# xdspacelab/openvslam

Hardware: NVIDIA H100
Metric: frames/sec extract+match+local-BA @1920x960 4000kp (higher is better)
Workload: dtype u8 (extract, Hamming) + f64 (pose optimiser, local BA)

## Files before the change

openvslam_b200/csrc/ba_math.cuh:

```cuda
#pragma once
#include <math.h>
#include <stdint.h>

#if defined(__CUDACC__)
#define OVS_BA_HD __host__ __device__ __forceinline__
#else
#define OVS_BA_HD static inline
#endif

namespace ovs {

constexpr int kCamPerspective = 0;
constexpr int kCamEquirectangular = 1;
constexpr double kPi = 3.14159265358979323846;

struct CameraD {
    int model;
    double fx, fy, cx, cy, fb, cols, rows;
};

OVS_BA_HD void mat3_vec(const double* R, const double* v, double* o) {
    o[0] = R[0] * v[0] + R[1] * v[1] + R[2] * v[2];
    o[1] = R[3] * v[0] + R[4] * v[1] + R[5] * v[2];
    o[2] = R[6] * v[0] + R[7] * v[1] + R[8] * v[2];
}
OVS_BA_HD void mat3_mat3(const double* A, const double* B, double* C) {
    for (int i = 0; i < 3; ++i)
        for (int j = 0; j < 3; ++j) C[3 * i + j] = A[3 * i] * B[j] + A[3 * i + 1] * B[3 + j] + A[3 * i + 2] * B[6 + j];
}

OVS_BA_HD void pose_oplus(const double* pose, const double* u, double* out) {
    const double wx = u[0], wy = u[1], wz = u[2];
    const double theta = sqrt(wx * wx + wy * wy + wz * wz);
    const double O[9] = {0, -wz, wy, wz, 0, -wx, -wy, wx, 0};
    double O2[9];
    mat3_mat3(O, O, O2);
    double a, b, c;
    if (theta < 0.00001) { a = 1.0; b = 0.5; c = 1.0 / 6.0; }
    else {
        a = sin(theta) / theta;
        b = (1 - cos(theta)) / (theta * theta);
        c = (theta - sin(theta)) / (theta * theta * theta);
    }
    double Rd[9], V[9];
    for (int i = 0; i < 9; ++i) {
        const double I = (i == 0 || i == 4 || i == 8) ? 1.0 : 0.0;
        Rd[i] = I + a * O[i] + b * O2[i];
        V[i] = I + b * O[i] + c * O2[i];
    }
    double td[3], tn[3];
    mat3_vec(V, u + 3, td);
    mat3_mat3(Rd, pose, out);
    mat3_vec(Rd, pose + 9, tn);
    out[9] = tn[0] + td[0]; out[10] = tn[1] + td[1]; out[11] = tn[2] + td[2];
}

OVS_BA_HD int edge_eval(const CameraD& cam, const double* pose, const double* pw, const double* obs, bool stereo,
                        double* e, double* Jp, double* Jl) {
    double pc[3];
    mat3_vec(pose, pw, pc);
    pc[0] += pose[9]; pc[1] += pose[10]; pc[2] += pose[11];
    const double x = pc[0], y = pc[1], z = pc[2];
    const double* R = pose;
    if (cam.model == kCamEquirectangular) {
        const double L = sqrt(x * x + y * y + z * z);
        const double theta = atan2(x, z);
        const double phi = -asin(y / L);
        e[0] = obs[0] - cam.cols * (0.5 + theta / (2 * kPi));
        e[1] = obs[1] - cam.rows * (0.5 - phi / kPi);
        if (Jp || Jl) {
            const double dpc[3][9] = {
                {0, z, -y, 1, 0, 0, R[0], R[1], R[2]},
                {-z, 0, x, 0, 1, 0, R[3], R[4], R[5]},
                {y, -x, 0, 0, 0, 1, R[6], R[7], R[8]}};
            const double xz2 = x * x + z * z;
            const double c0 = -(cam.cols / (2 * kPi)) * (1.0 / xz2);
            const double c1 = -(cam.rows / kPi) * (1.0 / (L * sqrt(xz2)));
            for (int k = 0; k < 9; ++k) {
                const double dL = (1.0 / L) * (x * dpc[0][k] + y * dpc[1][k] + z * dpc[2][k]);
                const double j0 = c0 * (z * dpc[0][k] - x * dpc[2][k]);
                const double j1 = c1 * (L * dpc[1][k] - y * dL);
                if (k < 6) { if (Jp) { Jp[k] = j0; Jp[6 + k] = j1; } }
                else if (Jl) { Jl[k - 6] = j0; Jl[3 + k - 6] = j1; }
            }
        }
        return 2;
    }
    const double fx = cam.fx, fy = cam.fy, fb = cam.fb;
    const double z_sq = z * z;
    const double reproj_x = fx * x / z + cam.cx;
    e[0] = obs[0] - reproj_x;
    e[1] = obs[1] - (fy * y / z + cam.cy);
    if (stereo) e[2] = obs[2] - (reproj_x - fb / z);
    if (Jl) {
        for (int k = 0; k < 3; ++k) {
            Jl[k] = -fx * R[k] / z + fx * x * R[6 + k] / z_sq;
            Jl[3 + k] = -fy * R[3 + k] / z + fy * y * R[6 + k] / z_sq;
            if (stereo) Jl[6 + k] = Jl[k] - fb * R[6 + k] / z_sq;
        }
    }
    if (Jp) {
        Jp[0] = x * y / z_sq * fx; Jp[1] = -(1.0 + (x * x / z_sq)) * fx; Jp[2] = y / z * fx;
        Jp[3] = -1.0 / z * fx; Jp[4] = 0.0; Jp[5] = x / z_sq * fx;
        Jp[6] = (1.0 + y * y / z_sq) * fy; Jp[7] = -x * y / z_sq * fy; Jp[8] = -x / z * fy;
        Jp[9] = 0.0; Jp[10] = -1.0 / z * fy; Jp[11] = y / z_sq * fy;
        if (stereo) {
            Jp[12] = Jp[0] - fb * y / z_sq; Jp[13] = Jp[1] + fb * x / z_sq; Jp[14] = Jp[2];
            Jp[15] = Jp[3]; Jp[16] = 0.0; Jp[17] = Jp[5] - fb / z_sq;
        }
    }
    return stereo ? 3 : 2;
}

OVS_BA_HD void huber(double e2, double delta, double* rho0, double* rho1) {
    const double dsqr = delta * delta;
    if (e2 <= dsqr) { *rho0 = e2; *rho1 = 1.0; }
    else {
        const double sqrte = sqrt(e2);
        *rho0 = 2 * sqrte * delta - dsqr;
        *rho1 = delta / sqrte;
    }
}

OVS_BA_HD bool inv3_sym(const double* D, double* Di) {
    const double a = D[0], b = D[1], c = D[2], d = D[3], e = D[4], f = D[5];
    const double c00 = d * f - e * e, c01 = c * e - b * f, c02 = b * e - c * d;
    const double det = a * c00 + b * c01 + c * c02;
    if (det == 0.0 || !isfinite(det)) return false;
    const double id = 1.0 / det;
    Di[0] = c00 * id; Di[1] = c01 * id; Di[2] = c02 * id;
    Di[3] = (a * f - c * c) * id; Di[4] = (b * c - a * e) * id; Di[5] = (a * d - b * b) * id;
    return true;
}

OVS_BA_HD int sym3(int i, int j) { return i <= j ? (i * 3 - i * (i - 1) / 2 + (j - i)) : (j * 3 - j * (j - 1) / 2 + (i - j)); }
OVS_BA_HD int sym6(int i, int j) { return i <= j ? (i * 6 - i * (i - 1) / 2 + (j - i)) : (j * 6 - j * (j - 1) / 2 + (i - j)); }

}
```

openvslam_b200/csrc/optimize.cu:

```cuda
#include <algorithm>
#include <cfloat>
#include <cmath>
#include <cstdio>
#include <cstdlib>
#include <cstring>
#include <functional>
#include <new>
#include <sched.h>
#include <time.h>
#include <vector>


#include "ba_math.cuh"
#include "block_sum.cuh"
#include "ovs_common.h"
#include "pnp_math.cuh"
#include "sim3_math.cuh"

namespace {

using ovs::CameraD;

constexpr int kMaxReducedDimBig = 6000;
constexpr int kCholMaxDynSmem = 226 * 1024;
constexpr int kNB = 32;
constexpr int kCholThreads = 512;
constexpr int kCholCluster = 8;
constexpr int kPoseThreads = 256;
constexpr int kPoseCluster = 8;

__device__ __forceinline__ double warp_sum(double v) {
#pragma unroll
    for (int o = 16; o > 0; o >>= 1) v += __shfl_xor_sync(0xffffffffu, v, o);
    return v;
}

__device__ double block_sum(double v, double* smem ) {
    const int lane = threadIdx.x & 31, wid = threadIdx.x >> 5, nw = blockDim.x >> 5;
    v = warp_sum(v);
    __syncthreads();
    if (lane == 0) smem[wid] = v;
    __syncthreads();
    double t = 0;
    for (int k = 0; k < nw; ++k) t += smem[k];
    return t;
}

__device__ __forceinline__ void atomic_max_pos(double* addr, double v) {
    atomicMax(reinterpret_cast<unsigned long long*>(addr), (unsigned long long)__double_as_longlong(v));
}

__device__ __forceinline__ void cluster_sync_all() {
    asm volatile("barrier.cluster.arrive.release.aligned;\n" ::);
    asm volatile("barrier.cluster.wait.acquire.aligned;\n" ::);
}
__device__ __forceinline__ unsigned cluster_size() { unsigned r; asm volatile("mov.u32 %0, %%cluster_nctarank;\n" : "=r"(r)); return r; }
__device__ __forceinline__ unsigned cluster_rank() { unsigned r; asm volatile("mov.u32 %0, %%cluster_ctarank;\n" : "=r"(r)); return r; }
__device__ __forceinline__ double ld_dsmem(const double* local_ptr, unsigned rank) {
    const unsigned addr = (unsigned)__cvta_generic_to_shared(local_ptr);
    unsigned remote;
    asm volatile("mapa.shared::cluster.u32 %0, %1, %2;\n" : "=r"(remote) : "r"(addr), "r"(rank));
    double v;
    asm volatile("ld.shared::cluster.f64 %0, [%1];\n" : "=d"(v) : "r"(remote));
    return v;
}
__device__ __forceinline__ void st_dsmem(double* local_ptr, unsigned rank, double v) {
    const unsigned addr = (unsigned)__cvta_generic_to_shared(local_ptr);
    unsigned remote;
    asm volatile("mapa.shared::cluster.u32 %0, %1, %2;\n" : "=r"(remote) : "r"(addr), "r"(rank));
    asm volatile("st.shared::cluster.f64 [%0], %1;\n" :: "r"(remote), "d"(v) : "memory");
}
__device__ __forceinline__ void cluster_sync_mem() {
    asm volatile("barrier.cluster.arrive.release.aligned;\n" ::: "memory");
    asm volatile("barrier.cluster.wait.acquire.aligned;\n" ::: "memory");
}

constexpr int kSpec = 4;
constexpr int kMaxTrials = 10;
struct LmCtl {
    double lambda, ni, currentChi, rho;
    double lam[kSpec], ni_after[kSpec];
    int buf[kSpec];
    int nbatch;
    int cur;
    int err_slot;
    int it;
    int qmax;
    int active;
    int iterations;
    int use_huber;
    int stopped;
    int spec_width;
    int round_live;
    int need_more;
    int pending_nbatch;
    int num_rounds, num_iterations, num_trials, batches, solver_trials;
    int round_iterations[8];
    double lambda_init[8];
    double last_chi2, last_lambda;
};

struct BaDev {
    CameraD cam;
    int K, L, M, nfree, n;
    const double* poses; const double* points;
    const double* poses_ring; const double* points_ring;
    const int* obs_kf; const int* obs_lm; const float2* obs_xy; const float* obs_xr; const float* inv_sigma_sq;
    const unsigned char* level;
    const int* free_idx;
    const int* lm_first;
    int use_huber; double delta;
};

__global__ void __launch_bounds__(128) k_ba_linearize(BaDev P, const LmCtl* __restrict__ ctl, double* __restrict__ Hpl, double* __restrict__ Cpp,
                                                       double* __restrict__ bpo, double* __restrict__ All, double* __restrict__ blo) {
    if (!ctl->active) return;
    __shared__ __align__(16) double sm[128 * 30];
    P.poses = P.poses_ring + (size_t)ctl->cur * 12 * P.K; P.points = P.points_ring + (size_t)ctl->cur * 3 * P.L;
    P.use_huber = ctl->use_huber;
    const int base = blockIdx.x * 128, t = threadIdx.x;
    const int i = base + t;
    const int nedge = min(128, P.M - base);
    const bool live = i < P.M && !P.level[i];
    int dim = 0, fi = -1;
    double e[3] = {0, 0, 0}, Jp[18], Jl[9], ww = 0;
#pragma unroll
    for (int k = 0; k < 18; ++k) Jp[k] = 0;
#pragma unroll
    for (int k = 0; k < 9; ++k) Jl[k] = 0;
    if (live) {
        const int kf = P.obs_kf[i], lm = P.obs_lm[i];
        fi = P.free_idx[kf];
        const float xr = P.obs_xr ? P.obs_xr[i] : -1.0f;
        const bool stereo = xr >= 0.0f;
        const float2 xy = P.obs_xy[i];
        const double obs[3] = {(double)xy.x, (double)xy.y, (double)xr};
        double pose[12], pw[3];
#pragma unroll
        for (int k = 0; k < 12; ++k) pose[k] = P.poses[12 * (size_t)kf + k];
#pragma unroll
        for (int k = 0; k < 3; ++k) pw[k] = P.points[3 * (size_t)lm + k];
        dim = ovs::edge_eval(P.cam, pose, pw, obs, stereo, e, Jp, Jl);
        const double w = (double)P.inv_sigma_sq[i];
        double chi = 0;
        for (int d = 0; d < dim; ++d) chi += w * e[d] * e[d];
        double rho0 = chi, rho1 = 1.0;
        if (P.use_huber) ovs::huber(chi, P.delta, &rho0, &rho1);
        ww = rho1 * w;
    }
    double* sW = sm; double* sbp = sm + 128 * 18; double* sA = sbp + 128 * 6;
    {
        double* A = sA + 6 * t;
        for (int a = 0; a < 3; ++a)
            for (int b = a; b < 3; ++b) {
                double h = 0;
                for (int d = 0; d < dim; ++d) h += Jl[3 * d + a] * ww * Jl[3 * d + b];
                A[ovs::sym3(a, b)] = h;
            }
        double* W = sW + 18 * t; double* bp = sbp + 6 * t;
        const bool fr = fi >= 0;
        for (int a = 0; a < 6; ++a) {
            double g = 0;
            for (int d = 0; d < dim; ++d) g -= Jp[6 * d + a] * ww * e[d];
            bp[a] = fr ? g : 0.0;
            for (int b = 0; b < 3; ++b) {
                double h = 0;
                for (int d = 0; d < dim; ++d) h += Jp[6 * d + a] * ww * Jl[3 * d + b];
                W[3 * a + b] = fr ? h : 0.0;
            }
        }
    }
    __syncthreads();
    {
        const double2* s2 = reinterpret_cast<const double2*>(sW); double2* g2 = reinterpret_cast<double2*>(Hpl + 18 * (size_t)base);
        for (int q = t; q < 9 * nedge; q += 128) g2[q] = s2[q];
        s2 = reinterpret_cast<const double2*>(sbp); g2 = reinterpret_cast<double2*>(bpo + 6 * (size_t)base);
        for (int q = t; q < 3 * nedge; q += 128) g2[q] = s2[q];
        s2 = reinterpret_cast<const double2*>(sA); g2 = reinterpret_cast<double2*>(All + 6 * (size_t)base);
        for (int q = t; q < 3 * nedge; q += 128) g2[q] = s2[q];
    }
    __syncthreads();
    double* sC = sm; double* sbl = sm + 128 * 21;
    {
        double* C = sC + 21 * t; double* bl = sbl + 3 * t;
        const bool fr = fi >= 0;
        for (int a = 0; a < 6; ++a)
            for (int b = a; b < 6; ++b) {
                double h = 0;
                for (int d = 0; d < dim; ++d) h += Jp[6 * d + a] * ww * Jp[6 * d + b];
                C[ovs::sym6(a, b)] = fr ? h : 0.0;
            }
        for (int a = 0; a < 3; ++a) {
            double g = 0;
            for (int d = 0; d < dim; ++d) g -= Jl[3 * d + a] * ww * e[d];
            bl[a] = g;
        }
    }
    __syncthreads();
    {
        const double2* s2 = reinterpret_cast<const double2*>(sC); double2* g2 = reinterpret_cast<double2*>(Cpp + 21 * (size_t)base);
        const int nd = 21 * nedge;
        for (int q = t; q < nd / 2; q += 128) g2[q] = s2[q];
        if ((nd & 1) && t == 0) Cpp[21 * (size_t)base + nd - 1] = sC[nd - 1];
        const int nb = 3 * nedge;
        for (int q = t; q < nb; q += 128) blo[3 * (size_t)base + q] = sbl[q];
    }
}

__global__ void __launch_bounds__(128) k_ba_landmark_accum(BaDev P, const LmCtl* __restrict__ ctl, const double* __restrict__ All, const double* __restrict__ blo,
                                                            double* __restrict__ Hll, double* __restrict__ bl, double* __restrict__ maxdiag) {
    if (!ctl->active) return;
    const int l = blockIdx.x * 128 + threadIdx.x;
    double md = 0;
    if (l < P.L) {
        double H[6] = {0, 0, 0, 0, 0, 0}, b[3] = {0, 0, 0};
        for (int p = P.lm_first[l]; p < P.lm_first[l + 1]; ++p) {
            if (P.level[p]) continue;
#pragma unroll
            for (int k = 0; k < 6; ++k) H[k] += All[6 * (size_t)p + k];
#pragma unroll
            for (int k = 0; k < 3; ++k) b[k] += blo[3 * (size_t)p + k];
        }
#pragma unroll
        for (int k = 0; k < 6; ++k) Hll[6 * (size_t)l + k] = H[k];
#pragma unroll
        for (int k = 0; k < 3; ++k) bl[3 * (size_t)l + k] = b[k];
        md = fmax(fabs(H[0]), fmax(fabs(H[3]), fabs(H[5])));
    }
#pragma unroll
    for (int o = 16; o > 0; o >>= 1) md = fmax(md, __shfl_xor_sync(0xffffffffu, md, o));
    if ((threadIdx.x & 31) == 0 && md > 0) atomic_max_pos(maxdiag, md);
}

__global__ void __launch_bounds__(128) k_ba_pose_accum_chunk(BaDev P, const LmCtl* __restrict__ ctl, const int* __restrict__ nchunks,
                                                              const int4* __restrict__ pair_rec, const int4* __restrict__ chunks,
                                                              const double* __restrict__ Cpp, const double* __restrict__ bpo,
                                                              double* __restrict__ ppart) {
    __shared__ double red[27][4];
    if (!ctl->active || (int)blockIdx.x >= *nchunks) return;
    const int4 ch = chunks[blockIdx.x];
    const int e = ch.y + threadIdx.x;
    double acc[27];
#pragma unroll
    for (int k = 0; k < 27; ++k) acc[k] = 0;
    if (e < ch.z) {
        const int4 rec = pair_rec[e];
        const int o = rec.x;
        if (!rec.w) {
#pragma unroll
            for (int k = 0; k < 21; ++k) acc[k] = Cpp[21 * (size_t)o + k];
#pragma unroll
            for (int k = 0; k < 6; ++k) acc[21 + k] = bpo[6 * (size_t)o + k];
        }
    }
    const int lane = threadIdx.x & 31, wid = threadIdx.x >> 5;
#pragma unroll
    for (int k = 0; k < 27; ++k) {
        const double v = warp_sum(acc[k]);
        if (lane == 0) red[k][wid] = v;
    }
    __syncthreads();
    if (threadIdx.x < 27)
        ppart[27 * (size_t)blockIdx.x + threadIdx.x] = red[threadIdx.x][0] + red[threadIdx.x][1] + red[threadIdx.x][2] + red[threadIdx.x][3];
}

__global__ void k_ba_pose_final_plan(LmCtl* ctl, int nfree, const int* __restrict__ kf_chunk_begin, const double* __restrict__ ppart,
                                     double* __restrict__ Hpp, double* __restrict__ bp, double* maxdiag, int* fail,
                                     const volatile int* stop_word, volatile int* mirror);

__device__ __forceinline__ void dmma_m8n8k4(double& d0, double& d1, double a, double b) {
    asm volatile("mma.sync.aligned.m8n8k4.row.col.f64.f64.f64.f64 {%0, %1}, {%2}, {%3}, {%0, %1};\n" : "+d"(d0), "+d"(d1) : "d"(a), "d"(b));
}

constexpr int kSGY = 76, kSGW = 84;
__global__ void __launch_bounds__(128, 4) k_ba_schur_chunk(BaDev P, const LmCtl* __restrict__ ctl, const int* __restrict__ nchunks,
                                                         const int4* __restrict__ pair_rec, const int4* __restrict__ chunks,
                                                         const int2* __restrict__ pair_ab, const double* __restrict__ Hll,
                                                         const double* __restrict__ Hpl, const double* __restrict__ bl,
                                                         double* __restrict__ spart, size_t spart_stride) {
    __shared__ double s_y[4 * 8 * kSGY];
    __shared__ double s_w[4 * 8 * kSGW];
    double* sYw = s_y + (threadIdx.x >> 5) * 8 * kSGY;
    double* sWw = s_w + (threadIdx.x >> 5) * 8 * kSGW;
    static_assert(4 * 8 * kSGY >= kSpec * 4 * 64, "reduction buffer must fit in the Y region");
    const int nbatch = ctl->nbatch;
    if (nbatch == 0 || (int)blockIdx.x >= *nchunks) return;
    const int4 ch = chunks[blockIdx.x];
    const int2 ab = pair_ab[ch.x];
    const bool diag = ab.x == ab.y;
    const int lane = threadIdx.x & 31, wid = threadIdx.x >> 5;
    const int e = ch.y + threadIdx.x;
    double wa[18], hl[6] = {0, 0, 0, 0, 0, 0};
    int lm = -1;
    {
        double wb[18], gl[3] = {0, 0, 0};
#pragma unroll
        for (int k = 0; k < 18; ++k) { wa[k] = 0; wb[k] = 0; }
        if (e < ch.z) {
            const int4 ob = pair_rec[e];
            if (!ob.w) {
                lm = ob.z;
                const double2* pa = reinterpret_cast<const double2*>(Hpl + 18 * (size_t)ob.x);
                const double2* pb = reinterpret_cast<const double2*>(Hpl + 18 * (size_t)ob.y);
#pragma unroll
                for (int k = 0; k < 9; ++k) { const double2 v = pa[k]; wa[2 * k] = v.x; wa[2 * k + 1] = v.y; }
                if (ob.x == ob.y) {
#pragma unroll
                    for (int k = 0; k < 18; ++k) wb[k] = wa[k];
                } else {
#pragma unroll
                    for (int k = 0; k < 9; ++k) { const double2 v = pb[k]; wb[2 * k] = v.x; wb[2 * k + 1] = v.y; }
                }
                const double2* ph = reinterpret_cast<const double2*>(Hll + 6 * (size_t)lm);
#pragma unroll
                for (int k = 0; k < 3; ++k) { const double2 v = ph[k]; hl[2 * k] = v.x; hl[2 * k + 1] = v.y; }
                if (diag) { gl[0] = bl[3 * (size_t)lm]; gl[1] = bl[3 * (size_t)lm + 1]; gl[2] = bl[3 * (size_t)lm + 2]; }
            }
        }
#pragma unroll
        for (int kc = 0; kc < 3; ++kc) {
            const int kk = 3 * (lane & 3) + kc, base = (lane >> 2) * kSGW + (kk >> 2) * 28 + (kk & 3);
#pragma unroll
            for (int c = 0; c < 6; ++c) sWw[base + 4 * c] = wb[3 * c + kc];
            sWw[base + 24] = gl[kc];
        }
    }
    double lam[kSpec];
#pragma unroll
    for (int bt = 0; bt < kSpec; ++bt) lam[bt] = ctl->lam[bt];
    auto make_dinv = [&](int bt, double (&di)[6]) {
        double D[6] = {hl[0] + lam[bt], hl[1], hl[2], hl[3] + lam[bt], hl[4], hl[5] + lam[bt]};
        if (lm < 0 || !ovs::inv3_sym(D, di)) {
#pragma unroll
            for (int q = 0; q < 6; ++q) di[q] = 0.0;
        }
    };
    const int r = lane >> 2;
    int sbase[3];
#pragma unroll
    for (int kc = 0; kc < 3; ++kc) { const int kk = 3 * (lane & 3) + kc; sbase[kc] = (lane >> 2) * kSGY + (kk >> 2) * 24 + (kk & 3); }
    const bool rowA = r < 6, colB = r < 6 || (r == 6 && diag);
    double acc[kSpec][2];
#pragma unroll
    for (int bt = 0; bt < kSpec; ++bt) { acc[bt][0] = 0; acc[bt][1] = 0; }
    const int nrec_w = min(32, max(0, ch.z - (ch.y + 32 * wid)));
    const bool second_half = nrec_w > 16;
#pragma unroll
    for (int bt = 0; bt < kSpec; ++bt) {
        if (bt < nbatch && nrec_w > 0) {
            double di[6];
            make_dinv(bt, di);
            double ya[18];
#pragma unroll
            for (int a = 0; a < 6; ++a) {
                const double w0 = wa[3 * a], w1 = wa[3 * a + 1], w2 = wa[3 * a + 2];
                ya[3 * a] = w0 * di[0] + w1 * di[1] + w2 * di[2];
                ya[3 * a + 1] = w0 * di[1] + w1 * di[3] + w2 * di[4];
                ya[3 * a + 2] = w0 * di[2] + w1 * di[4] + w2 * di[5];
            }
            __syncwarp();
#pragma unroll
            for (int a = 0; a < 6; ++a) {
                sYw[sbase[0] + 4 * a] = ya[3 * a]; sYw[sbase[1] + 4 * a] = ya[3 * a + 1]; sYw[sbase[2] + 4 * a] = ya[3 * a + 2];
            }
            __syncwarp();
            double c0[2] = {0, 0}, c1[2] = {0, 0}, c2[2] = {0, 0}, c3[2] = {0, 0};
            const double* yb = sYw + lane;
            const double* wb = sWw + lane;
#pragma unroll
            for (int half = 0; half < 2; ++half) {
                if (half == 1 && !second_half) break;
#pragma unroll
                for (int t = 0; t < 3; ++t) {
                    const int oy = (4 * half) * kSGY + t * 24, ow = (4 * half) * kSGW + t * 28;
                    const double a0 = rowA ? yb[oy] : 0.0, b0 = colB ? wb[ow] : 0.0;
                    const double a1 = rowA ? yb[oy + kSGY] : 0.0, b1 = colB ? wb[ow + kSGW] : 0.0;
                    const double a2 = rowA ? yb[oy + 2 * kSGY] : 0.0, b2 = colB ? wb[ow + 2 * kSGW] : 0.0;
                    const double a3 = rowA ? yb[oy + 3 * kSGY] : 0.0, b3 = colB ? wb[ow + 3 * kSGW] : 0.0;
                    dmma_m8n8k4(c0[0], c0[1], a0, b0);
                    dmma_m8n8k4(c1[0], c1[1], a1, b1);
                    dmma_m8n8k4(c2[0], c2[1], a2, b2);
                    dmma_m8n8k4(c3[0], c3[1], a3, b3);
                }
            }
            acc[bt][0] = (c0[0] + c1[0]) + (c2[0] + c3[0]);
            acc[bt][1] = (c0[1] + c1[1]) + (c2[1] + c3[1]);
        }
    }
    __syncthreads();
    double* red = s_y;
#pragma unroll
    for (int bt = 0; bt < kSpec; ++bt)
        if (bt < nbatch) { red[(bt * 4 + wid) * 64 + 2 * lane] = acc[bt][0]; red[(bt * 4 + wid) * 64 + 2 * lane + 1] = acc[bt][1]; }
    __syncthreads();
    for (int idx = threadIdx.x; idx < 42 * nbatch; idx += 128) {
        const int bt = idx / 42, t = idx - 42 * bt;
        const int i = t < 36 ? t / 6 : t - 36;
        const int j = t < 36 ? t % 6 : 6;
        const int src = 2 * (4 * i + (j >> 1)) + (j & 1);
        const double* rb = red + (size_t)bt * 4 * 64;
        double v = rb[src] + rb[64 + src] + rb[128 + src] + rb[192 + src];
        if (j == 6 && !diag) v = 0.0;
        spart[(size_t)bt * spart_stride + 42 * (size_t)blockIdx.x + t] = v;
    }
}

__global__ void __launch_bounds__(256) k_ba_pair_flags(const unsigned char* __restrict__ level, int4* __restrict__ rec, int n) {
    const int i = blockIdx.x * 256 + threadIdx.x;
    if (i >= n) return;
    int4 r = rec[i];
    r.w = (level[r.x] | level[r.y]) ? 1 : 0;
    rec[i] = r;
}

__global__ void __launch_bounds__(64) k_ba_schur_final(int n, const LmCtl* __restrict__ ctl, const int* __restrict__ pair_chunk_begin, const int2* __restrict__ pair_ab,
                                                        const double* __restrict__ spart, size_t spart_stride, const double* __restrict__ Hpp,
                                                        const double* __restrict__ bp, double* __restrict__ S, size_t S_stride) {
    const int pid = blockIdx.x, t = threadIdx.x;
    if ((int)blockIdx.y >= ctl->nbatch) return;
    const double lambda = ctl->lam[blockIdx.y];
    spart += (size_t)blockIdx.y * spart_stride; S += (size_t)blockIdx.y * S_stride;
    double* bS = S + (size_t)n * n;
    if (t >= 42) return;
    const int a = pair_ab[pid].x, b = pair_ab[pid].y;
    const bool diag = a == b;
    if (t >= 36 && !diag) return;
    double s = 0;
    const int c0 = pair_chunk_begin[pid], c1 = pair_chunk_begin[pid + 1];
#pragma unroll 4
    for (int c = c0; c < c1; ++c) s += spart[42 * (size_t)c + t];
    if (t < 36) {
        const int i = t / 6, j = t % 6;
        double v = -s;
        if (diag) v += Hpp[21 * (size_t)a + ovs::sym6(i, j)] + (i == j ? lambda : 0.0);
        S[(size_t)(6 * b + j) * n + 6 * a + i] = v;
    } else {
        bS[6 * a + t - 36] = bp[6 * (size_t)a + t - 36] - s;
    }
}

constexpr int kPP = 36;
__host__ __device__ __forceinline__ size_t chol_fixed_doubles(int n) { return (size_t)32 * 33 + 32 + ((n + 1 + 31) / 32) * 32 + 32 * 33 + 32 * kPP; }
__host__ __device__ __forceinline__ size_t chol_panel_doubles(int n) { return (size_t)(n + 4) * kPP; }
__host__ __device__ __forceinline__ int chol_back_pitch(int n) { return ((n + 3) / 4) * 4 + 4; }
__host__ __device__ __forceinline__ size_t chol_back_doubles(int n) { return (size_t)32 * 33 + (size_t)32 * chol_back_pitch(n); }

__global__ void __launch_bounds__(kCholThreads, 1)
k_ba_cholesky_solve(const LmCtl* __restrict__ ctl, double* __restrict__ A, size_t A_stride, int n, double* __restrict__ x, double* __restrict__ invL, size_t invL_stride,
                    int* __restrict__ fail, long long* __restrict__ dbg_clk, int dbuf) {
    {
        const int bt = blockIdx.x / (int)cluster_size();
        if (bt >= ctl->nbatch) return;
        A += (size_t)bt * A_stride; x += (size_t)bt * n; invL += (size_t)bt * invL_stride; fail += bt;
        if (bt != 0) dbg_clk = nullptr;
    }
    extern __shared__ __align__(16) double sh[];
    const int npad = ((n + 1 + 31) / 32) * 32;
    double* LdT = sh;
    double* invd = LdT + 32 * 33;
    double* vec = invd + 32;
    double* scr = vec + npad;
    double* IL = scr + 32 * 33;
    double* P = IL + 32 * kPP;
    const int tid = threadIdx.x, lane = tid & 31, wid = tid >> 5;
    const int rank = (int)cluster_rank();
    const int ncta = (int)cluster_size();
    const int g = lane >> 2, q = lane & 3;
    __shared__ int s_fail;
    if (tid == 0) s_fail = 0;
    __syncthreads();
    const int nblk = (n + kNB - 1) / kNB;
    auto stamp = [&](int slot) { if (dbg_clk && rank == 0 && tid == 0 && slot < 192) dbg_clk[slot] = clock64(); };
    auto stamp1 = [&](int slot) { if (dbg_clk && rank == 0 && tid == 64 && slot < 192) dbg_clk[slot] = clock64(); };

    auto factor_block = [&](double (&a)[kNB], double* cs) {
        bool bad = false;
        double my_inv = 1.0;
        double ajj = __shfl_sync(0xffffffffu, a[0], 0);
        double inv = rsqrt(ajj);
#pragma unroll
        for (int j = 0; j < kNB; ++j) {
            bad = bad || !(ajj > 0.0) || !isfinite(ajj);
            const double l = (lane >= j) ? a[j] * inv : 0.0;
            if (lane == j) my_inv = inv;
            double* col = cs + j * 32;
            col[lane] = l;
            if (j + 1 < kNB) {
                ajj = __shfl_sync(0xffffffffu, fma(-l, l, a[j + 1]), j + 1);
                inv = rsqrt(ajj);
            }
            __syncwarp();
#pragma unroll
            for (int c = j + 1; c < kNB; ++c) a[c] = fma(-l, col[c], a[c]);
        }
        if (bad && lane == 0) s_fail = 1;
        return my_inv;
    };

    for (int blk = -1; blk < nblk; ++blk) {
        const bool pro = blk < 0;
        const int kb = pro ? 0 : blk * kNB;
        const int nb = pro ? 0 : min(kNB, n - kb);
        const int rem = n - kb - nb;
        const int prow = rem + 1;
        const int nbn = min(kNB, rem);
        if (!pro) stamp(5 * blk);
        if (wid >= 2 && !pro) {
            for (int r = wid - 2; r < prow; r += kCholThreads / 32 - 2) {
                if (lane < nb) {
                    const unsigned dst = (unsigned)__cvta_generic_to_shared(P + r * kPP + lane);
                    const double* src = A + (size_t)(kb + nb + r) * n + kb + lane;
                    asm volatile("cp.async.ca.shared.global [%0], [%1], 8;\n" :: "r"(dst), "l"(src));
                } else {
                    P[r * kPP + lane] = 0.0;
                }
            }
            asm volatile("cp.async.commit_group;\n" ::);
            asm volatile("cp.async.wait_group 0;\n" ::);
        }
        if (!pro) {
            __syncthreads();
            stamp(5 * blk + 1);
            if (s_fail) break;
        }
        const bool worker = wid >= 2 && (wid & 3) != 0;
        const int nw = 11;
        const int wk = wid - 2 - (wid >> 2);
        if (wid == 0) {
            if (rem > 0) {
                for (int r = 0; r < nbn; ++r)
                    if (lane <= r) {
                        const unsigned dst = (unsigned)__cvta_generic_to_shared(scr + r * 33 + lane);
                        asm volatile("cp.async.ca.shared.global [%0], [%1], 8;\n" :: "r"(dst), "l"(A + (size_t)(kb + nb + r) * n + kb + nb + lane));
                    }
                asm volatile("cp.async.commit_group;\n" ::);
            }
            if (lane < prow && !pro) {
                const int r = lane;
                double xr[kNB];
                double* row = P + r * kPP;
#pragma unroll
                for (int c = 0; c < kNB; c += 2) {
                    const double2 v = *reinterpret_cast<const double2*>(row + c);
                    xr[c] = v.x; xr[c + 1] = v.y;
                }
#pragma unroll
                for (int c = 0; c < kNB; ++c) {
                    const double xc = xr[c] * invd[c];
                    xr[c] = xc;
#pragma unroll
                    for (int c2 = c + 1; c2 < kNB; ++c2) xr[c2] = fma(-xc, LdT[c * 32 + c2], xr[c2]);
                }
#pragma unroll
                for (int c = 0; c < kNB; c += 2) *reinterpret_cast<double2*>(row + c) = make_double2(xr[c], xr[c + 1]);
            }
            __syncwarp();
            if (!pro) stamp(5 * blk + 2);
            if (rem == 0) {
                if (rank == 0 && lane < nb) A[(size_t)(kb + nb) * n + kb + lane] = P[lane];
            } else {
                if (!pro) asm volatile("bar.arrive 3, 480;\n" ::: "memory");
            asm volatile("cp.async.wait_group 0;\n" ::: "memory");
            __syncwarp();
            double acc[4][4][2];
#pragma unroll
            for (int ti = 0; ti < 4; ++ti)
#pragma unroll
                for (int tj = 0; tj <= ti; ++tj)
#pragma unroll
                    for (int e = 0; e < 2; ++e) {
                        const int rr = 8 * ti + g, cc = 8 * tj + 2 * q + e;
                        acc[ti][tj][e] = (rr < nbn && cc <= rr) ? scr[rr * 33 + cc] : 0.0;
                    }
            __syncwarp();
#pragma unroll 2
            for (int k4 = pro ? kNB : 0; k4 < kNB; k4 += 4) {
                double pv[4];
#pragma unroll
                for (int ti = 0; ti < 4; ++ti) pv[ti] = P[(8 * ti + g) * kPP + k4 + q];
#pragma unroll
                for (int ti = 0; ti < 4; ++ti)
#pragma unroll
                    for (int tj = 0; tj <= ti; ++tj) dmma_m8n8k4(acc[ti][tj][0], acc[ti][tj][1], -pv[ti], pv[tj]);
            }
#pragma unroll
            for (int ti = 0; ti < 4; ++ti)
#pragma unroll
                for (int tj = 0; tj <= ti; ++tj)
#pragma unroll
                    for (int e = 0; e < 2; ++e) scr[(8 * ti + g) * 33 + 8 * tj + 2 * q + e] = acc[ti][tj][e];
            __syncwarp();
            double a[kNB];
#pragma unroll
            for (int c = 0; c < kNB; ++c) a[c] = (lane < nbn && c <= lane) ? scr[lane * 33 + c] : ((c == lane) ? 1.0 : 0.0);
            if (blk < 12 && !pro) { asm volatile("" :: "d"(a[0]), "d"(a[kNB - 1])); stamp(168 + 2 * blk); }
            __syncwarp();
            const double my_inv = factor_block(a, scr);
            if (blk < 12 && !pro) { asm volatile("" :: "d"(my_inv)); stamp(169 + 2 * blk); }
            if (!pro) asm volatile("bar.sync 2, 64;\n" ::: "memory");
#pragma unroll
            for (int c = 0; c < kNB; ++c) LdT[c * 32 + lane] = scr[c * 32 + lane];
            invd[lane] = my_inv;
            }
        } else if (pro) {
        } else if (wid == 1) {
            double r[kNB];
#pragma unroll
            for (int i = 0; i < kNB; ++i) r[i] = (i == lane) ? 1.0 : 0.0;
#pragma unroll
            for (int i = 0; i < kNB; ++i) {
                const double xi = r[i] * invd[i];
                r[i] = xi;
#pragma unroll
                for (int i2 = i + 1; i2 < kNB; ++i2) r[i2] = fma(-LdT[i * 32 + i2], xi, r[i2]);
            }
#pragma unroll
            for (int i = 0; i < kNB; ++i) IL[i * kPP + lane] = r[i];
            asm volatile("bar.arrive 4, 384;\n" ::: "memory");
            if (rank == 0) {
#pragma unroll
                for (int i = 0; i < kNB; ++i) invL[((size_t)blk * kNB + i) * kNB + lane] = r[i];
            }
            if (rem > 0) asm volatile("bar.arrive 2, 64;\n" ::: "memory");
        } else {
            if (worker) {
                asm volatile("bar.sync 4, 384;\n" ::: "memory");
                double bfr[4][8];
// ... 37 lines not shown
                    const int mj = w - base;
                    const int R0 = mi * 16, C0 = mj * 32;
                    if (w == 0) stamp1(50 + 4 * blk);
                    double acc[2][4][2];
#pragma unroll
                    for (int ti = 0; ti < 2; ++ti)
#pragma unroll
                        for (int tj = 0; tj < 4; ++tj)
#pragma unroll
                            for (int e = 0; e < 2; ++e) {
                                const int rr = R0 + 8 * ti + g, cc = C0 + 8 * tj + 2 * q + e;
                                const bool mine = rr < prow && cc < rem && cc <= rr && !(rr < nbn);
                                acc[ti][tj][e] = mine ? A[(size_t)(kb + nb + rr) * n + kb + nb + cc] : 0.0;
                            }
                    if (w == 0) { asm volatile("" :: "d"(acc[0][0][0]), "d"(acc[1][3][1]), "d"(acc[1][0][0]), "d"(acc[0][3][1])); stamp1(51 + 4 * blk); }
                    const double* pa0 = P + (size_t)min(R0 + g, prow - 1) * kPP + q;
                    const double* pa1 = P + (size_t)min(R0 + 8 + g, prow - 1) * kPP + q;
                    const double* pb[4];
#pragma unroll
                    for (int tj = 0; tj < 4; ++tj) pb[tj] = P + (size_t)min(C0 + 8 * tj + g, prow - 1) * kPP + q;
#pragma unroll 2
                    for (int k4 = 0; k4 < kNB; k4 += 4) {
                        const double af0 = -pa0[k4], af1 = -pa1[k4];
                        double bf[4];
#pragma unroll
                        for (int tj = 0; tj < 4; ++tj) bf[tj] = pb[tj][k4];
#pragma unroll
                        for (int tj = 0; tj < 4; ++tj) {
                            dmma_m8n8k4(acc[0][tj][0], acc[0][tj][1], af0, bf[tj]);
                            dmma_m8n8k4(acc[1][tj][0], acc[1][tj][1], af1, bf[tj]);
                        }
                    }
                    if (w == 0) { asm volatile("" :: "d"(acc[0][0][0]), "d"(acc[1][3][1])); stamp1(52 + 4 * blk); }
#pragma unroll
                    for (int ti = 0; ti < 2; ++ti)
#pragma unroll
                        for (int tj = 0; tj < 4; ++tj)
#pragma unroll
                            for (int e = 0; e < 2; ++e) {
                                const int rr = R0 + 8 * ti + g, cc = C0 + 8 * tj + 2 * q + e;
                                const bool mine = rr < prow && cc < rem && cc <= rr && !(rr < nbn);
                                if (mine) A[(size_t)(kb + nb + rr) * n + kb + nb + cc] = acc[ti][tj][e];
                            }
                    if (w == 0) stamp1(53 + 4 * blk);
                }
            }
        }
        if (rem == 0) break;
        if (pro) continue;
        stamp(5 * blk + 3);
        cluster_sync_all();
        stamp(5 * blk + 4);
    }
    __syncthreads();
    if (s_fail) { if (tid == 0 && rank == 0) *fail = 1; return; }
    if (rank != 0) return;

    for (int i = tid; i < n; i += kCholThreads) vec[i] = A[(size_t)n * n + i];
    const int bp = chol_back_pitch(n);
    double* const R0buf = P;
    double* const L1buf = P + 32 * (size_t)bp;
    double* const R1buf = L1buf + 32 * 33;
    double* const red = scr;
    auto stage = [&](int b, int which) {
        const int kb = b * kNB;
        const int nb = min(kNB, n - kb);
        double* Ldst = which ? L1buf : LdT;
        double* Rdst = which ? R1buf : R0buf;
        for (int i = tid; i < kNB * kNB; i += kCholThreads) {
            const unsigned dst = (unsigned)__cvta_generic_to_shared(Ldst + (i >> 5) * 33 + (i & 31));
            asm volatile("cp.async.ca.shared.global [%0], [%1], 8;\n" :: "r"(dst), "l"(invL + (size_t)b * kNB * kNB + i));
        }
        for (int j = wid; j < nb; j += kCholThreads / 32)
            for (int c = 2 * lane; c < kb; c += 64) {
                const unsigned dst = (unsigned)__cvta_generic_to_shared(Rdst + j * bp + c);
                asm volatile("cp.async.cg.shared.global [%0], [%1], 16;\n" :: "r"(dst), "l"(A + (size_t)(kb + j) * n + c));
            }
        asm volatile("cp.async.commit_group;\n" ::);
    };
    __syncthreads();
    stamp(94);
    stage(nblk - 1, 0);
    for (int blk = nblk - 1; blk >= 0; --blk) {
        const int kb = blk * kNB;
        const int nb = min(kNB, n - kb);
        const int cur = dbuf ? ((nblk - 1 - blk) & 1) : 0;
        if (dbuf && blk > 0) {
            stage(blk - 1, cur ^ 1);
            asm volatile("cp.async.wait_group 1;\n" ::);
        } else {
            asm volatile("cp.async.wait_group 0;\n" ::);
        }
        __syncthreads();
        stamp(96 + 3 * (nblk - 1 - blk));
        const double* Lc = cur ? L1buf : LdT;
        const double* rows = cur ? R1buf : R0buf;
        if (wid == 0) {
            const double t = (lane < nb) ? vec[kb + lane] : 0.0;
            double acc0 = 0, acc1 = 0;
#pragma unroll
            for (int j = 0; j < kNB; j += 2) {
                acc0 = fma(Lc[j * 33 + lane], __shfl_sync(0xffffffffu, t, j), acc0);
                acc1 = fma(Lc[(j + 1) * 33 + lane], __shfl_sync(0xffffffffu, t, j + 1), acc1);
            }
            red[lane] = acc0 + acc1;
            if (lane < nb) vec[kb + lane] = acc0 + acc1;
        }
        __syncthreads();
        stamp(97 + 3 * (nblk - 1 - blk));
        for (int i = tid; i < kb; i += kCholThreads) {
            double s0 = 0, s1 = 0;
#pragma unroll 8
            for (int j = 0; j < kNB; j += 2) {
                if (j < nb) s0 = fma(rows[j * bp + i], red[j], s0);
                if (j + 1 < nb) s1 = fma(rows[(j + 1) * bp + i], red[j + 1], s1);
            }
            vec[i] -= s0 + s1;
        }
        __syncthreads();
        stamp(98 + 3 * (nblk - 1 - blk));
        if (!dbuf && blk > 0) stage(blk - 1, 0);
    }
    for (int i = tid; i < n; i += kCholThreads) x[i] = vec[i];
    stamp(95);
}

__global__ void __launch_bounds__(64) k_chol_big_diag(const LmCtl* __restrict__ ctl, double* __restrict__ A, size_t A_stride, int n, int kb, int nb,
                                                      double* __restrict__ invL, size_t invL_stride, int* __restrict__ fail) {
    if ((int)blockIdx.y >= ctl->nbatch) return;
    A += (size_t)blockIdx.y * A_stride; invL += (size_t)blockIdx.y * invL_stride + (size_t)(kb / kNB) * kNB * kNB; fail += blockIdx.y;
    __shared__ double cs[kNB * kNB];
    __shared__ double sinv[kNB];
    const int lane = threadIdx.x & 31, wid = threadIdx.x >> 5;
    if (wid == 0) {
        double a[kNB];
#pragma unroll
        for (int c = 0; c < kNB; ++c) {
            double v = (c == lane) ? 1.0 : 0.0;
            if (lane < nb && c <= lane) v = A[(size_t)(kb + lane) * n + kb + c];
            a[c] = v;
        }
        bool bad = false;
        double my_inv = 1.0;
        double ajj = __shfl_sync(0xffffffffu, a[0], 0);
        double inv = rsqrt(ajj);
#pragma unroll
        for (int j = 0; j < kNB; ++j) {
            bad = bad || !(ajj > 0.0) || !isfinite(ajj);
            const double l = (lane >= j) ? a[j] * inv : 0.0;
            if (lane == j) my_inv = inv;
            cs[j * 32 + lane] = l;
            if (lane < nb && j <= lane && j < nb) A[(size_t)(kb + lane) * n + kb + j] = l;
            if (j + 1 < kNB) {
                ajj = __shfl_sync(0xffffffffu, fma(-l, l, a[j + 1]), j + 1);
                inv = rsqrt(ajj);
            }
            __syncwarp();
#pragma unroll
            for (int c = j + 1; c < kNB; ++c) a[c] = fma(-l, cs[j * 32 + c], a[c]);
        }
        if (bad && lane == 0) *fail = 1;
        sinv[lane] = my_inv;
    }
    __syncthreads();
    if (wid == 1) {
        double r[kNB];
#pragma unroll
        for (int i = 0; i < kNB; ++i) r[i] = (i == lane) ? 1.0 : 0.0;
#pragma unroll
        for (int i = 0; i < kNB; ++i) {
            const double xi = r[i] * sinv[i];
            r[i] = xi;
#pragma unroll
            for (int i2 = i + 1; i2 < kNB; ++i2) r[i2] = fma(-cs[i * 32 + i2], xi, r[i2]);
        }
#pragma unroll
        for (int i = 0; i < kNB; ++i) invL[i * kNB + lane] = r[i];
    }
}

__global__ void __launch_bounds__(128) k_chol_big_panel(const LmCtl* __restrict__ ctl, double* __restrict__ A, size_t A_stride, int n, int kb, int nb,
                                                        const double* __restrict__ invL, size_t invL_stride) {
    if ((int)blockIdx.y >= ctl->nbatch) return;
    A += (size_t)blockIdx.y * A_stride; invL += (size_t)blockIdx.y * invL_stride + (size_t)(kb / kNB) * kNB * kNB;
    __shared__ double IL[kNB][kNB + 1];
    for (int i = threadIdx.x; i < kNB * kNB; i += 128) IL[i >> 5][i & 31] = invL[i];
    __syncthreads();
    const int prow = n - kb - nb + 1;
    const int r = blockIdx.x * 128 + threadIdx.x;
    if (r >= prow) return;
    double* row = A + (size_t)(kb + nb + r) * n + kb;
    double xr[kNB];
#pragma unroll
    for (int c = 0; c < kNB; ++c) xr[c] = (c < nb) ? row[c] : 0.0;
#pragma unroll
    for (int j = 0; j < kNB; ++j) {
        double acc = 0.0;
#pragma unroll
        for (int k = 0; k <= j; ++k) acc = fma(xr[k], IL[j][k], acc);
        if (j < nb) row[j] = acc;
    }
}

__global__ void __launch_bounds__(128) k_chol_big_trailing(const LmCtl* __restrict__ ctl, double* __restrict__ A, size_t A_stride, int n, int kb, int nb) {
    if ((int)blockIdx.y >= ctl->nbatch) return;
    A += (size_t)blockIdx.y * A_stride;
    const int lane = threadIdx.x & 31, wid = threadIdx.x >> 5, g = lane >> 2, q = lane & 3;
    const int rem = n - kb - nb, prow = rem + 1;
    const int nmr = (prow + 15) / 16, nmc = (rem + 31) / 32;
    const int w = blockIdx.x * 4 + wid;
    int mi = 0, base = 0;
    for (;; ++mi) {
        if (mi >= nmr) return;
        const int cnt = min(nmc, (16 * mi + 15) / 32 + 1);
        if (w < base + cnt) break;
        base += cnt;
    }
    const int mj = w - base;
    const int R0 = mi * 16, C0 = mj * 32;
    const double* P = A + (size_t)(kb + nb) * n + kb;
    double* T = A + (size_t)(kb + nb) * n + kb + nb;
    double acc[2][4][2];
#pragma unroll
    for (int ti = 0; ti < 2; ++ti)
#pragma unroll
        for (int tj = 0; tj < 4; ++tj)
#pragma unroll
            for (int e = 0; e < 2; ++e) {
                const int rr = R0 + 8 * ti + g, cc = C0 + 8 * tj + 2 * q + e;
                acc[ti][tj][e] = (rr < prow && cc < rem && cc <= rr) ? T[(size_t)rr * n + cc] : 0.0;
            }
    const double* pa0 = P + (size_t)min(R0 + g, prow - 1) * n;
    const double* pa1 = P + (size_t)min(R0 + 8 + g, prow - 1) * n;
    const double* pb[4];
#pragma unroll
    for (int tj = 0; tj < 4; ++tj) pb[tj] = P + (size_t)min(C0 + 8 * tj + g, prow - 1) * n;
#pragma unroll 2
    for (int k4 = 0; k4 < kNB; k4 += 4) {
        const bool kin = k4 + q < nb;
        const double af0 = kin ? -pa0[k4 + q] : 0.0, af1 = kin ? -pa1[k4 + q] : 0.0;
        double bf[4];
#pragma unroll
        for (int tj = 0; tj < 4; ++tj) bf[tj] = kin ? pb[tj][k4 + q] : 0.0;
#pragma unroll
        for (int tj = 0; tj < 4; ++tj) {
            dmma_m8n8k4(acc[0][tj][0], acc[0][tj][1], af0, bf[tj]);
            dmma_m8n8k4(acc[1][tj][0], acc[1][tj][1], af1, bf[tj]);
        }
    }
#pragma unroll
    for (int ti = 0; ti < 2; ++ti)
#pragma unroll
        for (int tj = 0; tj < 4; ++tj)
#pragma unroll
            for (int e = 0; e < 2; ++e) {
                const int rr = R0 + 8 * ti + g, cc = C0 + 8 * tj + 2 * q + e;
                if (rr < prow && cc < rem && cc <= rr) T[(size_t)rr * n + cc] = acc[ti][tj][e];
            }
}

__global__ void __launch_bounds__(512) k_chol_big_backsolve(const LmCtl* __restrict__ ctl, const double* __restrict__ A, size_t A_stride, int n, const double* __restrict__ invL,
                                                            size_t invL_stride, double* __restrict__ x, int* __restrict__ fail) {
    if ((int)blockIdx.x >= ctl->nbatch) return;
    A += (size_t)blockIdx.x * A_stride; invL += (size_t)blockIdx.x * invL_stride; x += (size_t)blockIdx.x * n; fail += blockIdx.x;
    extern __shared__ __align__(16) double sh[];
    double* vec = sh;
    double* IL = sh + ((n + 31) / 32) * 32;
    double* red = IL + 32 * 33;
    const int tid = threadIdx.x, lane = tid & 31, wid = tid >> 5;
    for (int i = tid; i < n; i += 512) vec[i] = A[(size_t)n * n + i];
    const int nblk = (n + kNB - 1) / kNB;
    for (int blk = nblk - 1; blk >= 0; --blk) {
        const int kb = blk * kNB, nb = min(kNB, n - kb);
        __syncthreads();
        for (int i = tid; i < kNB * kNB; i += 512) IL[(i >> 5) * 33 + (i & 31)] = invL[(size_t)blk * kNB * kNB + i];
        __syncthreads();
        if (wid == 0) {
            const double t = (lane < nb) ? vec[kb + lane] : 0.0;
            double a0 = 0, a1 = 0;
#pragma unroll
            for (int j = 0; j < kNB; j += 2) {
                a0 = fma(IL[j * 33 + lane], __shfl_sync(0xffffffffu, t, j), a0);
                a1 = fma(IL[(j + 1) * 33 + lane], __shfl_sync(0xffffffffu, t, j + 1), a1);
            }
            red[lane] = a0 + a1;
            if (lane < nb) vec[kb + lane] = a0 + a1;
        }
        __syncthreads();
        for (int i = tid; i < kb; i += 512) {
            double s0 = 0, s1 = 0;
            for (int j = 0; j + 1 < nb; j += 2) {
                s0 = fma(A[(size_t)(kb + j) * n + i], red[j], s0);
                s1 = fma(A[(size_t)(kb + j + 1) * n + i], red[j + 1], s1);
            }
            if (nb & 1) s0 = fma(A[(size_t)(kb + nb - 1) * n + i], red[nb - 1], s0);
            vec[i] -= s0 + s1;
        }
    }
    __syncthreads();
    if (*fail) return;
    for (int i = tid; i < n; i += 512) x[i] = vec[i];
}

__global__ void __launch_bounds__(128) k_ba_update(BaDev P, const LmCtl* __restrict__ ctl, const double* __restrict__ Hpl, const double* __restrict__ Hll,
                                                    const double* __restrict__ bl, const double* __restrict__ bp, const double* __restrict__ x,
                                                    double* poses_ring, double* points_ring,
                                                    double* __restrict__ partial_scale, int* __restrict__ fail) {
    __shared__ double sm[36];
    const int nbatch = ctl->nbatch;
    if (nbatch == 0) return;
    double lambda[kSpec]; int buf[kSpec];
#pragma unroll
    for (int bt = 0; bt < kSpec; ++bt) { lambda[bt] = ctl->lam[bt]; buf[bt] = ctl->buf[bt]; }
    P.poses = P.poses_ring + (size_t)ctl->cur * 12 * P.K; P.points = P.points_ring + (size_t)ctl->cur * 3 * P.L;
    const int t = blockIdx.x * 128 + threadIdx.x;
    double sc[kSpec];
#pragma unroll
    for (int bt = 0; bt < kSpec; ++bt) sc[bt] = 0;
    if (t < P.L) {
        const int l = t;
        const double b0 = bl[3 * (size_t)l], b1 = bl[3 * (size_t)l + 1], b2 = bl[3 * (size_t)l + 2];
        double r[kSpec][3];
#pragma unroll
        for (int bt = 0; bt < kSpec; ++bt) { r[bt][0] = b0; r[bt][1] = b1; r[bt][2] = b2; }
        for (int p = P.lm_first[l]; p < P.lm_first[l + 1]; ++p) {
            const int fi = P.free_idx[P.obs_kf[p]];
            if (P.level[p] || fi < 0) continue;
            double W[18];
            const double2* pw = reinterpret_cast<const double2*>(Hpl + 18 * (size_t)p);
#pragma unroll
            for (int k = 0; k < 9; ++k) { const double2 v = pw[k]; W[2 * k] = v.x; W[2 * k + 1] = v.y; }
#pragma unroll
            for (int bt = 0; bt < kSpec; ++bt) {
                if (bt < nbatch) {
                    const double* xb = x + (size_t)bt * P.n + 6 * fi;
#pragma unroll
                    for (int a = 0; a < 6; ++a) {
                        const double xa = xb[a];
                        r[bt][0] -= W[3 * a] * xa; r[bt][1] -= W[3 * a + 1] * xa; r[bt][2] -= W[3 * a + 2] * xa;
                    }
                }
            }
        }
        const double p0 = P.points[3 * (size_t)l], p1 = P.points[3 * (size_t)l + 1], p2 = P.points[3 * (size_t)l + 2];
#pragma unroll
        for (int bt = 0; bt < kSpec; ++bt) {
            if (bt < nbatch) {
                const double D[6] = {Hll[6 * (size_t)l] + lambda[bt], Hll[6 * (size_t)l + 1], Hll[6 * (size_t)l + 2], Hll[6 * (size_t)l + 3] + lambda[bt],
                                     Hll[6 * (size_t)l + 4], Hll[6 * (size_t)l + 5] + lambda[bt]};
                double Di[6];
                if (!ovs::inv3_sym(D, Di)) {
                    fail[bt] = 1;
#pragma unroll
                    for (int q = 0; q < 6; ++q) Di[q] = 0.0;
                }
                const double d0 = Di[0] * r[bt][0] + Di[1] * r[bt][1] + Di[2] * r[bt][2];
                const double d1 = Di[1] * r[bt][0] + Di[3] * r[bt][1] + Di[4] * r[bt][2];
                const double d2 = Di[2] * r[bt][0] + Di[4] * r[bt][1] + Di[5] * r[bt][2];
                double* cand_points = points_ring + (size_t)buf[bt] * 3 * P.L;
                cand_points[3 * (size_t)l] = p0 + d0;
                cand_points[3 * (size_t)l + 1] = p1 + d1;
                cand_points[3 * (size_t)l + 2] = p2 + d2;
                sc[bt] = d0 * (lambda[bt] * d0 + b0) + d1 * (lambda[bt] * d1 + b1) + d2 * (lambda[bt] * d2 + b2);
            }
        }
    } else if (t < P.L + P.K) {
        const int k = t - P.L;
        const int fi = P.free_idx[k];
        double pose[12];
#pragma unroll
        for (int j = 0; j < 12; ++j) pose[j] = P.poses[12 * (size_t)k + j];
#pragma unroll
        for (int bt = 0; bt < kSpec; ++bt) {
            if (bt < nbatch) {
            double out[12];
            if (fi >= 0) {
                double u[6];
#pragma unroll
                for (int j = 0; j < 6; ++j) { u[j] = x[(size_t)bt * P.n + 6 * fi + j]; sc[bt] += u[j] * (lambda[bt] * u[j] + bp[6 * (size_t)fi + j]); }
                ovs::pose_oplus(pose, u, out);
            } else {
#pragma unroll
                for (int j = 0; j < 12; ++j) out[j] = pose[j];
            }
            double* cand_poses = poses_ring + (size_t)buf[bt] * 12 * P.K;
#pragma unroll
            for (int j = 0; j < 12; ++j) cand_poses[12 * (size_t)k + j] = out[j];
            }
        }
    }
#pragma unroll
    for (int bt = 0; bt < kSpec; ++bt) {
        if (bt < nbatch) {
            const double tot = block_sum(sc[bt], sm);
            if (threadIdx.x == 0) partial_scale[(size_t)bt * gridDim.x + blockIdx.x] = tot;
        }
    }
}

__global__ void __launch_bounds__(128) k_ba_errors(BaDev P, const LmCtl* __restrict__ ctl, int at_current,
                                                    double* __restrict__ err, double* __restrict__ partial_chi) {
    __shared__ double sm[36];
    int slot;
    if (at_current) {
        if (!ctl->active) return;
        slot = ctl->cur;
    } else {
        if ((int)blockIdx.y >= ctl->nbatch) return;
        slot = ctl->buf[blockIdx.y];
    }
    P.use_huber = ctl->use_huber;
    P.poses = P.poses_ring + (size_t)slot * 12 * P.K;
    P.points = P.points_ring + (size_t)slot * 3 * P.L;
    err += (size_t)blockIdx.y * 3 * P.M; partial_chi += (size_t)blockIdx.y * gridDim.x;
    const int i = blockIdx.x * 128 + threadIdx.x;
    double c = 0;
    if (i < P.M && !P.level[i]) {
        const int kf = P.obs_kf[i];
        const float xr = P.obs_xr ? P.obs_xr[i] : -1.0f;
        const bool stereo = xr >= 0.0f;
        const float2 xy = P.obs_xy[i];
        const double obs[3] = {(double)xy.x, (double)xy.y, (double)xr};
        double pose[12], pw[3], e[3] = {0, 0, 0};
#pragma unroll
        for (int k = 0; k < 12; ++k) pose[k] = P.poses[12 * (size_t)kf + k];
        const size_t pi = P.obs_lm ? (size_t)P.obs_lm[i] : (size_t)i;
#pragma unroll
        for (int k = 0; k < 3; ++k) pw[k] = P.points[3 * pi + k];
        ovs::edge_eval(P.cam, pose, pw, obs, stereo, e, nullptr, nullptr);
        err[3 * (size_t)i] = e[0]; err[3 * (size_t)i + 1] = e[1]; err[3 * (size_t)i + 2] = stereo ? e[2] : 0.0;
        const double w = (double)P.inv_sigma_sq[i];
        double chi = w * (e[0] * e[0] + e[1] * e[1]);
        if (stereo) chi += w * e[2] * e[2];
        c = chi;
        if (P.use_huber) { double r1; ovs::huber(chi, P.delta, &c, &r1); }
    }
    const double tot = block_sum(c, sm);
    if (threadIdx.x == 0) partial_chi[blockIdx.x] = tot;
}

__device__ __forceinline__ void mirror_state(const LmCtl& c, volatile int* mirror) {
    if (!mirror) return;
    mirror[0] = c.nbatch; mirror[1] = c.active; mirror[3] = c.need_more; mirror[4] = c.it;
}

__global__ void __launch_bounds__(kSpec * 256) k_ba_reduce(LmCtl* ctl, int mode, const double* __restrict__ partial_chi, int nchi,
                                                           const double* __restrict__ partial_scale, int nscale, int* fail,
                                                           const volatile int* stop_word, int batch_index, int* exec_log, volatile int* mirror,
                                                           int halt_if_undecided, int next_width_cap) {
    __shared__ double sm[kSpec][2][8];
    const int nb = mode == 0 ? (ctl->active ? 1 : 0) : ctl->nbatch;
    if (nb == 0) {
        if (threadIdx.x == 0 && mode == 1 && exec_log && batch_index >= 0) exec_log[batch_index] = 0;
        return;
    }
    const int t = threadIdx.x >> 8, tl = threadIdx.x & 255, lane = tl & 31, w = tl >> 5;
    double a = 0, b = 0;
    if (t < nb) {
        const double* pc = partial_chi + (size_t)t * nchi;
        for (int i = tl; i < nchi; i += 256) a += pc[i];
        if (mode == 1) {
            const double* ps = partial_scale + (size_t)t * nscale;
            for (int i = tl; i < nscale; i += 256) b += ps[i];
        }
    }
    a = warp_sum(a); b = warp_sum(b);
    if (lane == 0) { sm[t][0][w] = a; sm[t][1][w] = b; }
    __syncthreads();
    if (threadIdx.x != 0) return;
    double chi[kSpec], sc[kSpec];
    for (int k = 0; k < nb; ++k) {
        double x = 0, y = 0;
        for (int j = 0; j < 8; ++j) { x += sm[k][0][j]; y += sm[k][1][j]; }
        chi[k] = x; sc[k] = y;
    }
    if (mode == 0) { ctl->currentChi = chi[0]; ctl->err_slot = 0; return; }
    LmCtl c = *ctl;
    const bool stop = stop_word && *stop_word != 0;
    double lambda = c.lambda, ni = c.ni, currentChi = c.currentChi, rho = c.rho;
    int qmax = c.qmax, cur = c.cur, es = c.err_slot, ntr = c.num_trials;
    bool done = false;
#pragma unroll
    for (int k = 0; k < kSpec; ++k) {
        if (k < nb && !done) {
            const bool ok2 = fail[k] == 0;
            const double tempChi = ok2 ? chi[k] : DBL_MAX;
            rho = currentChi - tempChi;
            double scale = ok2 ? sc[k] : 0.0;
            scale += 1e-3;
            rho /= scale;
            es = k;
            ++qmax; ++ntr;
            if (rho > 0 && isfinite(tempChi)) {
                double alpha = 1. - pow(2 * rho - 1, 3.0);
                alpha = fmin(alpha, 2. / 3.);
                lambda = c.lam[k] * fmax(1. / 3., alpha);
                ni = 2;
                currentChi = tempChi;
                cur = c.buf[k];
                done = true;
            } else {
                lambda = c.lam[k] * c.ni_after[k];
                ni = c.ni_after[k] * 2;
                if (!(rho < 0) || qmax >= kMaxTrials || stop) done = true;
            }
        }
    }
    c.lambda = lambda; c.ni = ni; c.currentChi = currentChi; c.rho = rho;
    c.qmax = qmax; c.cur = cur; c.err_slot = es; c.num_trials = ntr;
    c.batches += 1; c.solver_trials += nb;
    if (exec_log && batch_index >= 0) exec_log[batch_index] = nb;
#pragma unroll
    for (int k = 0; k < kSpec; ++k) fail[k] = 0;
    if (done) {
        c.nbatch = 0;
        c.last_chi2 = currentChi; c.last_lambda = lambda;
        const int it = c.it + 1;
        c.it = it;
        if (qmax == kMaxTrials || rho == 0 || it >= c.iterations) c.active = 0;
        if (stop) { c.active = 0; c.stopped = 1; }
    } else {
        int nn = min(kSpec, kMaxTrials - qmax);
        if (next_width_cap > 0) nn = min(nn, next_width_cap);
        double l = lambda, n2 = ni;
#pragma unroll
        for (int k = 0; k < kSpec; ++k)
            if (k < nn) { c.lam[k] = l; c.buf[k] = (cur + 1 + k) % (kSpec + 1); l *= n2; c.ni_after[k] = n2; n2 *= 2; }
        if (halt_if_undecided) {
            c.pending_nbatch = nn; c.nbatch = 0; c.active = 0; c.need_more = 1;
        } else {
            c.nbatch = nn;
        }
    }
    *ctl = c;
    mirror_state(c, mirror);
}

__global__ void k_lm_resume(LmCtl* ctl, volatile int* mirror) {
    LmCtl c = *ctl;
    if (!c.need_more) return;
    c.nbatch = c.pending_nbatch; c.pending_nbatch = 0; c.active = 1; c.need_more = 0;
    *ctl = c;
    mirror_state(c, mirror);
}

__global__ void k_lm_init(LmCtl* ctl, int spec_width, int* fail, volatile int* mirror) {
    LmCtl c;
    memset(&c, 0, sizeof(c));
    c.ni = 2; c.spec_width = spec_width;
    *ctl = c;
    for (int k = 0; k < kSpec; ++k) fail[k] = 0;
    mirror_state(c, mirror);
}

__global__ void k_lm_round_begin(LmCtl* ctl, int iterations, int use_huber, const volatile int* stop_word, double* maxdiag, volatile int* mirror) {
    LmCtl c = *ctl;
    if (stop_word && *stop_word != 0) c.stopped = 1;
    c.iterations = iterations; c.use_huber = use_huber;
    c.it = 0; c.qmax = 0; c.rho = 0; c.lambda = 0; c.ni = 2; c.nbatch = 0;
    c.round_live = c.stopped ? 0 : 1;
    c.active = (iterations > 0 && !c.stopped) ? 1 : 0;
    *ctl = c;
    maxdiag[0] = 0; maxdiag[1] = 0;
    mirror_state(c, mirror);
}

__global__ void k_lm_round_end(LmCtl* ctl, const volatile int* stop_word, volatile int* mirror) {
    LmCtl c = *ctl;
    if (c.round_live || c.num_rounds == 0) {
        const int r = c.num_rounds;
        if (r < 8) c.round_iterations[r] = c.it;
        c.num_iterations += c.it;
        c.num_rounds = r + 1;
    }
    c.active = 0; c.nbatch = 0;
    if (stop_word && *stop_word != 0) c.stopped = 1;
    *ctl = c;
    mirror_state(c, mirror);
}

__device__ void lm_plan_iteration(LmCtl* ctl, double lambda_init, const volatile int* stop_word, int* fail, volatile int* mirror) {
    LmCtl c = *ctl;
    if (c.active && stop_word && *stop_word != 0) { c.active = 0; c.stopped = 1; }
    if (!c.active) {
        c.nbatch = 0;
    } else {
        if (c.it == 0) {
            c.lambda = lambda_init;
            c.ni = 2;
            if (c.num_rounds < 8) c.lambda_init[c.num_rounds] = c.lambda;
        }
        c.qmax = 0; c.rho = 0;
        const int nn = min(max(c.spec_width, 1), kSpec);
        double l = c.lambda, n2 = c.ni;
#pragma unroll
        for (int k = 0; k < kSpec; ++k)
            if (k < nn) { c.lam[k] = l; c.buf[k] = (c.cur + 1 + k) % (kSpec + 1); l *= n2; c.ni_after[k] = n2; n2 *= 2; }
        c.nbatch = nn;
    }
    *ctl = c;
#pragma unroll
    for (int k = 0; k < kSpec; ++k) fail[k] = 0;
    mirror_state(c, mirror);
}

__global__ void __launch_bounds__(1024) k_ba_pose_final_plan(LmCtl* ctl, int nfree, const int* __restrict__ kf_chunk_begin, const double* __restrict__ ppart,
                                                              double* __restrict__ Hpp, double* __restrict__ bp, double* maxdiag, int* fail,
                                                              const volatile int* stop_word, volatile int* mirror) {
    __shared__ double smax[32];
    const bool active = ctl->active != 0, halted = ctl->need_more != 0;
    double md = 0;
    if (active) {
        for (int o = threadIdx.x; o < 27 * nfree; o += 1024) {
            const int a = o / 27, t = o - 27 * a;
            double v = 0;
            const int c0 = kf_chunk_begin[a], c1 = kf_chunk_begin[a + 1];
#pragma unroll 4
            for (int c = c0; c < c1; ++c) v += ppart[27 * (size_t)c + t];
            if (t < 21) {
                Hpp[21 * (size_t)a + t] = v;
                if (t == 0 || t == 6 || t == 11 || t == 15 || t == 18 || t == 20) md = fmax(md, fabs(v));
            } else {
                bp[6 * (size_t)a + t - 21] = v;
            }
        }
    }
#pragma unroll
    for (int o = 16; o > 0; o >>= 1) md = fmax(md, __shfl_xor_sync(0xffffffffu, md, o));
    if ((threadIdx.x & 31) == 0) smax[threadIdx.x >> 5] = md;
    __syncthreads();
    if (threadIdx.x != 0) return;
    if (halted) return;
    for (int w = 0; w < 32; ++w) md = fmax(md, smax[w]);
    md = fmax(md, maxdiag[0]);
    maxdiag[0] = 0; maxdiag[1] = 0;
    lm_plan_iteration(ctl, 1e-5 * md, stop_word, fail, mirror);
}

__global__ void __launch_bounds__(128) k_ba_classify(BaDev P, const LmCtl* __restrict__ ctl, const double* __restrict__ err_slots, double chi2_2d, double chi2_3d, int mode,
                                                      unsigned char* __restrict__ level_out, unsigned char* __restrict__ outlier_out) {
    const int i = blockIdx.x * 128 + threadIdx.x;
    if (i >= P.M || (mode == 0 && ctl->stopped)) return;
    const double* err = err_slots + (size_t)ctl->err_slot * 3 * P.M;
    P.poses = P.poses_ring + (size_t)ctl->cur * 12 * P.K; P.points = P.points_ring + (size_t)ctl->cur * 3 * P.L;
    const bool stereo = P.obs_xr && P.obs_xr[i] >= 0.0f;
    const double w = (double)P.inv_sigma_sq[i];
    const double e0 = err[3 * (size_t)i], e1 = err[3 * (size_t)i + 1], e2 = err[3 * (size_t)i + 2];
    double chi = w * (e0 * e0 + e1 * e1);
    if (stereo) chi += w * e2 * e2;
    bool depth_pos = true;
    if (P.cam.model != ovs::kCamEquirectangular) {
        const double* ps = P.poses + 12 * (size_t)P.obs_kf[i];
        const double* pw = P.points + 3 * (size_t)P.obs_lm[i];
        depth_pos = (ps[6] * pw[0] + ps[7] * pw[1] + ps[8] * pw[2] + ps[11]) > 0;
    }
    const bool outlier = (stereo ? chi2_3d : chi2_2d) < chi || !depth_pos;
    if (mode == 0) { if (outlier) level_out[i] = 1; }
    else outlier_out[i] = outlier ? 1 : 0;
}

__global__ void __launch_bounds__(256) k_ba_replicate_err(const LmCtl* __restrict__ ctl, double* err_slots, size_t n3) {
    if (ctl->stopped) return;
    const size_t i = (size_t)blockIdx.x * 256 + threadIdx.x;
    if (i >= n3) return;
    const int src = ctl->err_slot;
    const double v = err_slots[(size_t)src * n3 + i];
#pragma unroll
    for (int k = 0; k < kSpec; ++k)
        if (k != src) err_slots[(size_t)k * n3 + i] = v;
}

__global__ void __launch_bounds__(1024) k_ba_free_index(int K, const unsigned char* __restrict__ fixed, int* __restrict__ free_idx, long long* counts) {
    __shared__ int wsum[32];
    __shared__ int carry;
    const int tid = threadIdx.x, lane = tid & 31, wid = tid >> 5;
    if (tid == 0) carry = 0;
    __syncthreads();
    for (int base = 0; base < K; base += 1024) {
        const int i = base + tid;
        const int c = (i < K && !fixed[i]) ? 1 : 0;
        int v = c;
#pragma unroll
        for (int o = 1; o < 32; o <<= 1) { const int u = __shfl_up_sync(0xffffffffu, v, o); if (lane >= o) v += u; }
        if (lane == 31) wsum[wid] = v;
        __syncthreads();
        if (wid == 0) {
            int ws = wsum[lane];
#pragma unroll
            for (int o = 1; o < 32; o <<= 1) { const int u = __shfl_up_sync(0xffffffffu, ws, o); if (lane >= o) ws += u; }
            wsum[lane] = ws;
        }
        __syncthreads();
        const int excl = carry + (wid ? wsum[wid - 1] : 0) + v - c;
        if (i < K) free_idx[i] = c ? excl : -1;
        __syncthreads();
        if (tid == 1023) carry = excl + c;
        __syncthreads();
    }
    if (tid == 0) counts[0] = carry;
}

__global__ void __launch_bounds__(256) k_ba_landmark_index(int M, int L, int K, const int* __restrict__ obs_kf, const int* __restrict__ obs_lm,
                                                            int* __restrict__ lm_first, long long* counts) {
    const int i = blockIdx.x * 256 + threadIdx.x;
    if (i >= M) return;
    const int l = obs_lm[i], k = obs_kf[i];
    int err = 0;
    if (l < 0 || l >= L || k < 0 || k >= K) err = 1;
    const int lp = i > 0 ? obs_lm[i - 1] : -1;
    if (!err && i > 0 && l < lp) err = 2;
    if (err) {
        atomicMin(reinterpret_cast<unsigned long long*>(counts + 4), ((unsigned long long)i << 2) | (unsigned)err);
        return;
    }
    if (i == 0 || (lp >= -1 && lp < L && l != lp))
        for (int q = max(lp, -1) + 1; q <= l; ++q) lm_first[q] = i;
    if (i == M - 1)
        for (int q = l + 1; q <= L; ++q) lm_first[q] = M;
}

__global__ void __launch_bounds__(256) k_ba_pair_counts(int L, const int* __restrict__ lm_first, const int* __restrict__ obs_kf,
                                                         const int* __restrict__ free_idx, int* __restrict__ pair_off, const long long* __restrict__ counts) {
    if (counts[4] != 0x7fffffffffffffffll) return;
    const int l = blockIdx.x * 256 + threadIdx.x;
    if (l >= L) return;
    int m = 0;
    for (int p = lm_first[l]; p < lm_first[l + 1]; ++p) m += free_idx[obs_kf[p]] >= 0;
    pair_off[l] = m;
}

__global__ void __launch_bounds__(1024) k_ba_pair_offsets(int L, int* __restrict__ pair_off, long long* counts) {
    __shared__ long long wsum[33];
    __shared__ long long edges;
    const int tid = threadIdx.x, lane = tid & 31, wid = tid >> 5;
    if (counts[4] != 0x7fffffffffffffffll) return;
    if (tid == 0) edges = 0;
    const int run = (L + 1023) / 1024;
    const int b = min(L, tid * run), e = min(L, b + run);
    long long local = 0, my_edges = 0;
    for (int l = b; l < e; ++l) {
        const int m = pair_off[l];
        local += (long long)m * (m + 1) / 2;
        my_edges += m;
    }
    long long v = local;
#pragma unroll
    for (int o = 1; o < 32; o <<= 1) { const long long u = __shfl_up_sync(0xffffffffu, v, o); if (lane >= o) v += u; }
    if (lane == 31) wsum[wid] = v;
    __syncthreads();
    if (wid == 0) {
        const long long x = wsum[lane];
        long long ws = x;
#pragma unroll
        for (int o = 1; o < 32; o <<= 1) { const long long u = __shfl_up_sync(0xffffffffu, ws, o); if (lane >= o) ws += u; }
        wsum[lane] = ws - x;
        if (lane == 31) wsum[32] = ws;
    }
    __syncthreads();
    long long excl = wsum[wid] + v - local;
    for (int l = b; l < e; ++l) {
        const int m = pair_off[l];
        pair_off[l] = (int)min(excl, (long long)0x7fffffff);
        excl += (long long)m * (m + 1) / 2;
    }
    my_edges = (long long)warp_sum((double)my_edges);
    if (lane == 0) atomicAdd(reinterpret_cast<unsigned long long*>(&edges), (unsigned long long)my_edges);
    __syncthreads();
    if (tid == 0) { const long long total = wsum[32]; pair_off[L] = (int)min(total, (long long)0x7fffffff); counts[1] = total; counts[2] = edges; }
}

__global__ void __launch_bounds__(256) k_fill_f32(float* p, size_t n, float v) {
    const size_t i = (size_t)blockIdx.x * 256 + threadIdx.x;
    if (i < n) p[i] = v;
}

__global__ void __launch_bounds__(128) k_ba_emit_pairs(BaDev P, const int* __restrict__ pair_off, unsigned* __restrict__ keys,
                                                        unsigned long long* __restrict__ vals) {
    const int l = blockIdx.x * 128 + threadIdx.x;
    if (l >= P.L) return;
    int pos = pair_off[l];
    const int nf = P.nfree;
    for (int p = P.lm_first[l]; p < P.lm_first[l + 1]; ++p) {
        const int fa = P.free_idx[P.obs_kf[p]];
        if (fa < 0) continue;
        for (int q = p; q < P.lm_first[l + 1]; ++q) {
            const int fb = P.free_idx[P.obs_kf[q]];
            if (fb < 0) continue;
            int a = fa, b = fb, oa = p, ob = q;
            if (a > b) { a = fb; b = fa; oa = q; ob = p; }
            keys[pos] = (unsigned)(a * nf - a * (a - 1) / 2 + (b - a));
            vals[pos] = ((unsigned long long)(unsigned)ob << 32) | (unsigned)oa;
            ++pos;
        }
    }
}

__global__ void __launch_bounds__(256) k_ba_segments(const unsigned* __restrict__ keys, int n, int* __restrict__ seg_begin, int* __restrict__ seg_end) {
    const int i = blockIdx.x * 256 + threadIdx.x;
    if (i >= n) return;
    const unsigned k = keys[i];
    if (i == 0 || keys[i - 1] != k) seg_begin[k] = i;
    if (i == n - 1 || keys[i + 1] != k) seg_end[k] = i + 1;
}

__global__ void __launch_bounds__(256) k_ba_pair_records(const unsigned long long* __restrict__ vals, int n, const int* __restrict__ obs_lm, int4* __restrict__ rec) {
    const int i = blockIdx.x * 256 + threadIdx.x;
    if (i >= n) return;
    const unsigned long long v = vals[i];
    const int oa = (int)(unsigned)(v & 0xffffffffull), ob = (int)(unsigned)(v >> 32);
    rec[i] = make_int4(oa, ob, obs_lm[oa], 0);
}

constexpr int kSortBits = 11, kSortBins = 1 << kSortBits, kSortTile = 2048, kSortThreads = 256, kSortWarps = kSortThreads / 32;
static_assert(kSortTile == kSortWarps * 8 * 32 && kSortBins == kSortThreads * 8, "tile / bin geometry");

__global__ void __launch_bounds__(kSortThreads) k_sort_hist(const unsigned* __restrict__ keys, int n, int shift, int* __restrict__ hist) {
    __shared__ int sh[kSortBins];
    for (int i = threadIdx.x; i < kSortBins; i += kSortThreads) sh[i] = 0;
    __syncthreads();
    const int base = blockIdx.x * kSortTile;
    for (int i = threadIdx.x; i < kSortTile; i += kSortThreads) {
        const int idx = base + i;
        if (idx < n) atomicAdd(&sh[(keys[idx] >> shift) & (kSortBins - 1)], 1);
    }
    __syncthreads();
    int* out = hist + (size_t)blockIdx.x * kSortBins;
    for (int i = threadIdx.x; i < kSortBins; i += kSortThreads) out[i] = sh[i];
}

__global__ void __launch_bounds__(256) k_sort_tile_prefix(int* __restrict__ hist, int ntiles, int* __restrict__ bin_total) {
    const int bin = (int)((blockIdx.x * 256u + threadIdx.x) >> 5), lane = threadIdx.x & 31;
    int run = 0;
    for (int t0 = 0; t0 < ntiles; t0 += 32) {
        const int t = t0 + lane;
        int* p = hist + (size_t)min(t, ntiles - 1) * kSortBins + bin;
        const int v = t < ntiles ? *p : 0;
        int inc = v;
#pragma unroll
        for (int o = 1; o < 32; o <<= 1) { const int u = __shfl_up_sync(0xffffffffu, inc, o); if (lane >= o) inc += u; }
        if (t < ntiles) *p = run + inc - v;
        run += __shfl_sync(0xffffffffu, inc, 31);
    }
    if (lane == 0) bin_total[bin] = run;
}

__global__ void __launch_bounds__(kSortThreads) k_sort_scatter(const unsigned* __restrict__ keys, const unsigned long long* __restrict__ vals, int n, int shift,
                                                               const int* __restrict__ hist, const int* __restrict__ bin_total,
                                                               unsigned* __restrict__ keys_out, unsigned long long* __restrict__ vals_out) {
    __shared__ int s_base[kSortBins];
    __shared__ unsigned short s_cnt[kSortWarps][kSortBins];
    __shared__ int s_warp[kSortWarps];
    const int tid = threadIdx.x, lane = tid & 31, w = tid >> 5;
    for (int i = tid; i < kSortWarps * kSortBins / 2; i += kSortThreads) reinterpret_cast<unsigned*>(&s_cnt[0][0])[i] = 0;
    int tot[8], sum = 0;
#pragma unroll
    for (int k = 0; k < 8; ++k) { tot[k] = bin_total[tid * 8 + k]; sum += tot[k]; }
    int inc = sum;
#pragma unroll
    for (int o = 1; o < 32; o <<= 1) { const int u = __shfl_up_sync(0xffffffffu, inc, o); if (lane >= o) inc += u; }
    if (lane == 31) s_warp[w] = inc;
    const int base = blockIdx.x * kSortTile + w * 256;
    unsigned key[8];
    unsigned long long val[8];
#pragma unroll
    for (int c = 0; c < 8; ++c) {
        const int idx = base + c * 32 + lane;
        key[c] = idx < n ? keys[idx] : 0u;
        val[c] = idx < n ? vals[idx] : 0ull;
    }
    __syncthreads();
    {
        int run = inc - sum;
        for (int ww = 0; ww < w; ++ww) run += s_warp[ww];
        const int* hrow = hist + (size_t)blockIdx.x * kSortBins;
#pragma unroll
        for (int k = 0; k < 8; ++k) { s_base[tid * 8 + k] = run + hrow[tid * 8 + k]; run += tot[k]; }
    }
#pragma unroll
    for (int c = 0; c < 8; ++c) {
        const bool valid = base + c * 32 + lane < n;
        const unsigned d = valid ? (key[c] >> shift) & (kSortBins - 1) : (unsigned)kSortBins;
        const unsigned m = __match_any_sync(0xffffffffu, d);
        if (valid && lane == __ffs(m) - 1) s_cnt[w][d] = (unsigned short)(s_cnt[w][d] + __popc(m));
        __syncwarp();
    }
    __syncthreads();
    for (int bin = tid; bin < kSortBins; bin += kSortThreads) {
        unsigned r = 0;
#pragma unroll
        for (int ww = 0; ww < kSortWarps; ++ww) { const unsigned t = s_cnt[ww][bin]; s_cnt[ww][bin] = (unsigned short)r; r += t; }
    }
    __syncthreads();
#pragma unroll
    for (int c = 0; c < 8; ++c) {
        const bool valid = base + c * 32 + lane < n;
        const unsigned d = valid ? (key[c] >> shift) & (kSortBins - 1) : (unsigned)kSortBins;
        const unsigned m = __match_any_sync(0xffffffffu, d);
        if (valid) {
            const int pos = s_base[d] + (int)s_cnt[w][d] + __popc(m & ((1u << lane) - 1u));
            keys_out[pos] = key[c];
            vals_out[pos] = val[c];
        }
        __syncwarp();
        if (valid && lane == __ffs(m) - 1) s_cnt[w][d] = (unsigned short)(s_cnt[w][d] + __popc(m));
        __syncwarp();
    }
}

size_t sort_scratch_ints(long long n) { return (size_t)((n + kSortTile - 1) / kSortTile) * kSortBins + kSortBins; }
int sort_pairs(cudaStream_t st, unsigned* k0, unsigned* k1, unsigned long long* v0, unsigned long long* v1, int n, int end_bit, int* scratch,
               unsigned** keys_sorted, unsigned long long** vals_sorted) {
    const int ntiles = (n + kSortTile - 1) / kSortTile;
    int* hist = scratch;
    int* bin_total = scratch + (size_t)ntiles * kSortBins;
    unsigned *kin = k0, *kout = k1;
    unsigned long long *vin = v0, *vout = v1;
    for (int shift = 0; shift < end_bit; shift += kSortBits) {
        k_sort_hist<<<ntiles, kSortThreads, 0, st>>>(kin, n, shift, hist);
        OVS_LAUNCH_CHECK();
        k_sort_tile_prefix<<<kSortBins / 8, 256, 0, st>>>(hist, ntiles, bin_total);
        OVS_LAUNCH_CHECK();
        k_sort_scatter<<<ntiles, kSortThreads, 0, st>>>(kin, vin, n, shift, hist, bin_total, kout, vout);
        OVS_LAUNCH_CHECK();
        std::swap(kin, kout); std::swap(vin, vout);
    }
    *keys_sorted = kin; *vals_sorted = vin;
    return OVS_OK;
}

__global__ void __launch_bounds__(128) k_ba_pair_table(int nfree, int2* __restrict__ pair_ab, int* __restrict__ diag) {
    const int a = blockIdx.x;
    const int base = a * nfree - a * (a - 1) / 2;
    for (int b = a + threadIdx.x; b < nfree; b += 128) pair_ab[base + (b - a)] = make_int2(a, b);
    if (threadIdx.x == 0) diag[a] = base;
}

__global__ void __launch_bounds__(1024) k_ba_chunk_scan(const int* __restrict__ ids, int count, const int* __restrict__ seg_begin,
                                                         const int* __restrict__ seg_end, int* __restrict__ chunk_begin, int* __restrict__ total) {
    __shared__ int wsum[32];
    __shared__ int carry;
    const int tid = threadIdx.x, lane = tid & 31, wid = tid >> 5;
    if (tid == 0) carry = 0;
    __syncthreads();
    for (int base = 0; base < count; base += 1024) {
        const int i = base + tid;
        int c = 0;
        if (i < count) { const int id = ids ? ids[i] : i; c = (seg_end[id] - seg_begin[id] + 127) / 128; }
        int v = c;
#pragma unroll
        for (int o = 1; o < 32; o <<= 1) { const int u = __shfl_up_sync(0xffffffffu, v, o); if (lane >= o) v += u; }
        if (lane == 31) wsum[wid] = v;
        __syncthreads();
        if (wid == 0) {
            int ws = wsum[lane];
#pragma unroll
            for (int o = 1; o < 32; o <<= 1) { const int u = __shfl_up_sync(0xffffffffu, ws, o); if (lane >= o) ws += u; }
            wsum[lane] = ws;
        }
        __syncthreads();
        const int excl = carry + (wid ? wsum[wid - 1] : 0) + v - c;
        if (i < count) chunk_begin[i] = excl;
        __syncthreads();
        if (tid == 1023) carry = excl + c;
        __syncthreads();
    }
    if (tid == 0) { chunk_begin[count] = carry; *total = carry; }
}

__global__ void __launch_bounds__(128) k_ba_chunk_fill(const int* __restrict__ ids, int count, const int* __restrict__ seg_begin,
                                                        const int* __restrict__ seg_end, const int* __restrict__ chunk_begin, int4* __restrict__ chunks) {
    const int i = blockIdx.x * 128 + threadIdx.x;
    if (i >= count) return;
    const int id = ids ? ids[i] : i;
    const int e1 = seg_end[id];
    int c = chunk_begin[i];
    for (int e0 = seg_begin[id]; e0 < e1; e0 += 128, ++c) chunks[c] = make_int4(i, e0, min(e0 + 128, e1), 0);
}

struct PoseOptArgs {
    CameraD cam;
    int n;
    const double* pts_w; const float2* obs_xy; const float* obs_xr; const float* inv_sigma_sq;
    double* pose;
    unsigned char* outlier;
    int num_trials, num_each_iter;
    double delta, chi2_2d, chi2_3d;
    double* stats;
};

__device__ bool solve6(const double* Hs , double lambda, const double* b, double* x) {
    double Lm[6][6];
    for (int i = 0; i < 6; ++i)
        for (int j = 0; j <= i; ++j) {
            double s = Hs[ovs::sym6(j, i)] + (i == j ? lambda : 0.0);
            for (int k = 0; k < j; ++k) s -= Lm[i][k] * Lm[j][k];
            if (i == j) {
                if (!(s > 0.0) || !isfinite(s)) return false;
                Lm[i][i] = sqrt(s);
            } else Lm[i][j] = s / Lm[j][j];
        }
    double y[6];
    for (int i = 0; i < 6; ++i) {
        double s = b[i];
        for (int k = 0; k < i; ++k) s -= Lm[i][k] * y[k];
        y[i] = s / Lm[i][i];
    }
    for (int i = 5; i >= 0; --i) {
        double s = y[i];
        for (int k = i + 1; k < 6; ++k) s -= Lm[k][i] * x[k];
        x[i] = s / Lm[i][i];
    }
    return true;
}


__global__ void __cluster_dims__(kPoseCluster, 1, 1) __launch_bounds__(kPoseThreads, 1)
k_pose_optimize(PoseOptArgs A, double* __restrict__ err, unsigned char* __restrict__ level) {
    constexpr int NW = kPoseThreads / 32;
    __shared__ double sm_red[28][NW];
    __shared__ double s_slots[2][kPoseCluster][28];
    __shared__ double s_sys[28], s_pose[12], s_cand[12], s_x[6];
// ... 729 lines not shown
    }
    if (threadIdx.x < 13) A.sim3[13 * (size_t)b + threadIdx.x] = S12[threadIdx.x];
    if (threadIdx.x == 0) {
        A.num_inliers[b] = (int)cnt;
        A.best_iter[b] = best;
        A.valid[b] = (runs && (int)cnt >= A.min_num_inliers) ? 1 : 0;
    }
}

}

extern "C" int ovs_sim3_solve_ransac_host(ovs_optimizer* h, int B, const int32_t* pair_offsets, const ovs_camera* cam_1,
                                          const double* pose_1w, const ovs_camera* cam_2, const double* pose_2w, const double* pos_w_1,
                                          const float* sigma_sq_1, const double* pos_w_2, const float* sigma_sq_2, int fix_scale,
                                          int min_num_inliers, int max_num_iter, const uint64_t* seeds, double* sim3_12, uint8_t* valid,
                                          int32_t* num_inliers, int32_t* best_iter, uint8_t* inlier_out) {
    OVS_REQUIRE(h && B >= 0 && B <= 65535, OVS_ERR_INVALID_ARG, "bad argument (B must be in 0 .. 65535)");
    OVS_REQUIRE(min_num_inliers >= 0 && max_num_iter >= 0, OVS_ERR_INVALID_ARG, "min_num_inliers and max_num_iter must not be negative");
    if (B == 0) return OVS_OK;
    OVS_REQUIRE(pair_offsets && cam_1 && pose_1w && cam_2 && pose_2w && seeds && sim3_12 && valid && num_inliers && best_iter,
                OVS_ERR_INVALID_ARG, "null argument");
    OVS_REQUIRE(pair_offsets[0] == 0, OVS_ERR_INVALID_ARG, "pair_offsets[0] must be 0");
    for (int b = 0; b < B; ++b) {
        OVS_REQUIRE(pair_offsets[b + 1] >= pair_offsets[b], OVS_ERR_INVALID_ARG, "pair_offsets must be non-decreasing (problem %d)", b);
        OVS_REQUIRE((cam_1[b].model == ovs::kCamPerspective || cam_1[b].model == ovs::kCamEquirectangular) &&
                    (cam_2[b].model == ovs::kCamPerspective || cam_2[b].model == ovs::kCamEquirectangular),
                    OVS_ERR_INVALID_ARG, "unknown camera model (problem %d)", b);
    }
    const int n_all = pair_offsets[B];
    OVS_REQUIRE(n_all == 0 || (pos_w_1 && sigma_sq_1 && pos_w_2 && sigma_sq_2 && inlier_out), OVS_ERR_INVALID_ARG, "null argument");
    for (int i = 0; i < n_all; ++i)
        OVS_REQUIRE(sigma_sq_1[i] > 0.0f && std::isfinite(sigma_sq_1[i]) && sigma_sq_2[i] > 0.0f && std::isfinite(sigma_sq_2[i]),
                    OVS_ERR_INVALID_ARG, "sigma_sq of pair %d must be positive and finite", i);
    if (n_all == 0) {
        for (int b = 0; b < B; ++b) {
            for (int m = 0; m < 13; ++m) sim3_12[13 * (size_t)b + m] = (m == 0 || m == 4 || m == 8 || m == 12) ? 1.0 : 0.0;
            valid[b] = 0; num_inliers[b] = 0; best_iter[b] = -1;
        }
        return OVS_OK;
    }
    OVS_CUDA_CHECK(cudaSetDevice(h->device));
    invalidate_plan(h);
    if (h->pending) { OVS_CUDA_CHECK(ovs::sync_stream(h->stream)); h->pending = false; }
    const size_t N = (size_t)n_all, NB = (size_t)B;
    const size_t in_bytes_max = 256 * 12 + (NB + 1) * 4 + NB * 2 * sizeof(CameraD) + NB * 2 * 96 + N * 2 * (24 + 4) + NB * (8 + 8 + 4);
    const size_t out_bytes_max = 256 * 5 + NB * (13 * 8 + 4 + 4 + 1) + N;
    const size_t hbytes = in_bytes_max + out_bytes_max;
    const size_t dbytes = hbytes + 256 * 6 + N * 2 * (24 + 16 + 4) + 4096;
    int rc = ensure_arenas(h, dbytes, hbytes);
    if (rc != OVS_OK) return rc;
    Arena H{h->h_arena, 0, h->h_cap}, D{h->d_arena, 0, h->d_cap};
    int* hoff = H.take<int>(NB + 1); CameraD* hc1 = H.take<CameraD>(NB); CameraD* hc2 = H.take<CameraD>(NB);
    double* hp1 = H.take<double>(12 * NB); double* hp2 = H.take<double>(12 * NB);
    double* hw1 = H.take<double>(3 * N); float* hs1 = H.take<float>(N); double* hw2 = H.take<double>(3 * N); float* hs2 = H.take<float>(N);
    uint64_t* hseed = H.take<uint64_t>(NB); unsigned long long* hkey = H.take<unsigned long long>(NB); unsigned* hdone = H.take<unsigned>(NB);
    const size_t in_bytes = H.off;
    double* hS = H.take<double>(13 * NB);
    const size_t out_begin = (size_t)((uint8_t*)hS - h->h_arena);
    int* hnum = H.take<int>(NB); int* hbest = H.take<int>(NB); uint8_t* hvalid = H.take<uint8_t>(NB); uint8_t* hflags = H.take<uint8_t>(N);
    const size_t out_end = H.off;
    RansacArgs A;
    A.B = B; A.N = n_all; A.fix_scale = fix_scale ? 1 : 0; A.min_num_inliers = min_num_inliers; A.max_num_iter = max_num_iter;
    A.off = D.take<int>(NB + 1); A.cam1 = D.take<CameraD>(NB); A.cam2 = D.take<CameraD>(NB);
    A.pose1 = D.take<double>(12 * NB); A.pose2 = D.take<double>(12 * NB);
    A.pw1 = D.take<double>(3 * N); A.sig1 = D.take<float>(N); A.pw2 = D.take<double>(3 * N); A.sig2 = D.take<float>(N);
    A.seed = D.take<uint64_t>(NB); A.key = D.take<unsigned long long>(NB); A.done = D.take<unsigned>(NB);
    A.sim3 = D.take<double>(13 * NB); A.num_inliers = D.take<int>(NB); A.best_iter = D.take<int>(NB); A.valid = D.take<uint8_t>(NB);
    A.inlier = D.take<uint8_t>(N);
    A.pc1 = D.take<double>(3 * N); A.pc2 = D.take<double>(3 * N); A.rp1 = D.take<double>(2 * N); A.rp2 = D.take<double>(2 * N);
    A.bd1 = D.take<float>(N); A.bd2 = D.take<float>(N);
    memcpy(hoff, pair_offsets, 4 * (NB + 1));
    for (int b = 0; b < B; ++b) { hc1[b] = to_cam(&cam_1[b]); hc2[b] = to_cam(&cam_2[b]); }
    memcpy(hp1, pose_1w, 96 * NB); memcpy(hp2, pose_2w, 96 * NB);
    memcpy(hw1, pos_w_1, 24 * N); memcpy(hs1, sigma_sq_1, 4 * N); memcpy(hw2, pos_w_2, 24 * N); memcpy(hs2, sigma_sq_2, 4 * N);
    memcpy(hseed, seeds, 8 * NB); memset(hkey, 0, 8 * NB); memset(hdone, 0, 4 * NB);
    cudaStream_t st = h->stream;
    OVS_CUDA_CHECK(cudaMemcpyAsync(h->d_arena, h->h_arena, in_bytes, cudaMemcpyHostToDevice, st));
    k_sim3_ransac_prep<<<(n_all + kRansacPrepThreads - 1) / kRansacPrepThreads, kRansacPrepThreads, 0, st>>>(A);
    OVS_LAUNCH_CHECK();
    const int hyp_blocks = max_num_iter > 0 ? (max_num_iter + kRansacWarps - 1) / kRansacWarps : 1;
    k_sim3_ransac<<<dim3(hyp_blocks, B), kRansacThreads, 0, st>>>(A);
    OVS_LAUNCH_CHECK();
    OVS_CUDA_CHECK(cudaMemcpyAsync(h->h_arena + out_begin, h->d_arena + out_begin, out_end - out_begin, cudaMemcpyDeviceToHost, st));
    OVS_CUDA_CHECK(ovs::sync_stream(st));
    memcpy(sim3_12, hS, 13 * 8 * NB);
    memcpy(num_inliers, hnum, 4 * NB); memcpy(best_iter, hbest, 4 * NB); memcpy(valid, hvalid, NB);
    memcpy(inlier_out, hflags, N);
    return OVS_OK;
}

namespace {

constexpr int kPnpHypThreads = 64;
constexpr int kPnpWarps = 4;
constexpr int kPnpThreads = 32 * kPnpWarps;
constexpr int kPnpRefineThreads = ovs::kBlockSumThreads;
constexpr int kPnpChunk = ovs::kBlockSumChunk;

struct PnpArgs {
    int B, N, H, min_num_inliers, recompute;
    const int* off;
    const double* bear; const double* pw; const float* sf;
    const uint64_t* seed;
    unsigned long long* key;
    double* bound;
    double* hyp;
    int* cidx;
    double* pose; int* num_inliers; int* best_iter; uint8_t* valid; uint8_t* inlier;
};

__device__ __forceinline__ bool pnp_runs(const PnpArgs& A, int n) { return n >= ovs::kPnpMinSet && n >= A.min_num_inliers; }

__device__ __forceinline__ bool pnp_corr(const PnpArgs& A, const double* pose, size_t i) {
    const double pw[3] = {A.pw[3 * i], A.pw[3 * i + 1], A.pw[3 * i + 2]};
    const double b[3] = {A.bear[3 * i], A.bear[3 * i + 1], A.bear[3 * i + 2]};
    return ovs::pnp_is_inlier(pose, pw, b, A.bound[i]);
}

__global__ void __launch_bounds__(kPnpHypThreads) k_pnp_hypotheses(PnpArgs A) {
    const size_t g = (size_t)blockIdx.x * kPnpHypThreads + threadIdx.x;
    if (g < (size_t)A.N) A.bound[g] = ovs::pnp_max_cos(A.sf[g]);
    if (A.H == 0 || g >= (size_t)A.B * (size_t)A.H) return;
    const int b = (int)(g / (size_t)A.H), k = (int)(g % (size_t)A.H);
    const int o = A.off[b], n = A.off[b + 1] - o;
    if (!pnp_runs(A, n)) return;
    int idx[ovs::kPnpMinSet];
    ovs::ransac_sample<ovs::kPnpMinSet>(A.seed[b], k, n, idx);
    const ovs::PnpPoints P{A.pw + 3 * (size_t)o, A.bear + 3 * (size_t)o, idx, ovs::kPnpMinSet};
    ovs::epnp_pose(P, ovs::PnpSeqSum{ovs::kPnpMinSet}, A.hyp + 12 * g);
}

__global__ void __launch_bounds__(kPnpThreads) k_pnp_ransac(PnpArgs A) {
    const int b = blockIdx.y, lane = threadIdx.x & 31, warp = threadIdx.x >> 5;
    const int o = A.off[b], n = A.off[b + 1] - o;
    const int k = blockIdx.x * kPnpWarps + warp;
    if (!pnp_runs(A, n) || k >= A.H) return;
    const double* hp = A.hyp + 12 * ((size_t)b * A.H + k);
    double pose[12];
    for (int m = 0; m < 12; ++m) pose[m] = hp[m];
    unsigned cnt = 0;
    for (int base = 0; base < n; base += 32) {
        const int i = base + lane;
        const bool in = i < n && pnp_corr(A, pose, (size_t)(o + i));
        cnt += __popc(__ballot_sync(0xffffffffu, in));
    }
    if (lane == 0 && cnt > 0) atomicMax(&A.key[b], ((unsigned long long)cnt << 32) | (unsigned long long)(~(unsigned)k));
}

using ovs::PnpBlockSum;

__global__ void __launch_bounds__(kPnpRefineThreads) k_pnp_refine(PnpArgs A) {
    __shared__ double s_red[kPnpChunk * kPnpRefineThreads];
    __shared__ double s_res[78];
    __shared__ int s_warp[kPnpRefineThreads / 32];
    const int b = blockIdx.x, t = threadIdx.x, lane = t & 31, warp = t >> 5;
    const int o = A.off[b], n = A.off[b + 1] - o;
    const bool runs = pnp_runs(A, n);
    const unsigned long long key = A.key[b];
    const unsigned cnt = (unsigned)(key >> 32);
    const int best = cnt > 0 ? (int)(~(unsigned)(key & 0xffffffffull)) : -1;
    double pose[12];
    if (best >= 0) {
        const double* hp = A.hyp + 12 * ((size_t)b * A.H + best);
        for (int m = 0; m < 12; ++m) pose[m] = hp[m];
    } else {
        ovs::pnp_identity(pose);
    }
    for (int i = t; i < n; i += kPnpRefineThreads) A.inlier[o + i] = (best >= 0 && pnp_corr(A, pose, (size_t)(o + i))) ? 1 : 0;
    const bool valid = runs && (int)cnt >= A.min_num_inliers;
    int num = (int)cnt;
    if (valid && A.recompute && best >= 0 && (int)cnt >= ovs::kPnpMinSet) {
        int running = 0;
        for (int base = 0; base < n; base += kPnpRefineThreads) {
            const int i = base + t;
            const bool f = i < n && pnp_corr(A, pose, (size_t)(o + i));
            const unsigned bal = __ballot_sync(0xffffffffu, f);
            if (lane == 0) s_warp[warp] = __popc(bal);
            __syncthreads();
            int before = running;
            for (int w = 0; w < warp; ++w) before += s_warp[w];
            if (f) A.cidx[o + before + __popc(bal & ((1u << lane) - 1u))] = i;
            for (int w = 0; w < kPnpRefineThreads / 32; ++w) running += s_warp[w];
            __syncthreads();
        }
        __syncthreads();
        const ovs::PnpPoints P{A.pw + 3 * (size_t)o, A.bear + 3 * (size_t)o, A.cidx + o, (int)cnt};
        double np[12];
        ovs::epnp_pose(P, PnpBlockSum{(int)cnt, s_red, s_res}, np);
        for (int m = 0; m < 12; ++m) pose[m] = np[m];
        int c2 = 0;
        for (int base = 0; base < n; base += kPnpRefineThreads) {
            const int i = base + t;
            const bool f = i < n && pnp_corr(A, pose, (size_t)(o + i));
            if (i < n) A.inlier[o + i] = f ? 1 : 0;
            c2 += __syncthreads_count(f);
        }
        num = c2;
    }
    if (t < 12) A.pose[12 * (size_t)b + t] = pose[t];
    if (t == 0) {
        A.num_inliers[b] = num;
        A.best_iter[b] = best;
        A.valid[b] = valid ? 1 : 0;
    }
}

}

extern "C" int ovs_pnp_solve_ransac_host(ovs_optimizer* h, int B, const int32_t* corr_offsets, const double* bearings,
                                         const double* pos_w, const float* scale_factor, int min_num_inliers, int max_num_iter,
                                         int recompute, const uint64_t* seeds, double* pose_cw, uint8_t* valid, int32_t* num_inliers,
                                         int32_t* best_iter, uint8_t* inlier_out) {
    OVS_REQUIRE(h && B >= 0 && B <= 65535, OVS_ERR_INVALID_ARG, "bad argument (B must be in 0 .. 65535)");
    OVS_REQUIRE(min_num_inliers >= 0 && max_num_iter >= 0, OVS_ERR_INVALID_ARG, "min_num_inliers and max_num_iter must not be negative");
    if (B == 0) return OVS_OK;
    OVS_REQUIRE(corr_offsets && seeds && pose_cw && valid && num_inliers && best_iter, OVS_ERR_INVALID_ARG, "null argument");
    OVS_REQUIRE(corr_offsets[0] == 0, OVS_ERR_INVALID_ARG, "corr_offsets[0] must be 0");
    for (int b = 0; b < B; ++b)
        OVS_REQUIRE(corr_offsets[b + 1] >= corr_offsets[b], OVS_ERR_INVALID_ARG, "corr_offsets must be non-decreasing (problem %d)", b);
    const int n_all = corr_offsets[B];
    OVS_REQUIRE(n_all == 0 || (bearings && pos_w && scale_factor && inlier_out), OVS_ERR_INVALID_ARG, "null argument");
    for (int i = 0; i < n_all; ++i) {
        const double* p = pos_w + 3 * (size_t)i;
        const double* v = bearings + 3 * (size_t)i;
        OVS_REQUIRE(std::isfinite(p[0]) && std::isfinite(p[1]) && std::isfinite(p[2]), OVS_ERR_INVALID_ARG,
                    "pos_w of correspondence %d is not finite", i);
        OVS_REQUIRE(std::isfinite(v[0]) && std::isfinite(v[1]) && std::isfinite(v[2]) &&
                    std::fabs(v[0] * v[0] + v[1] * v[1] + v[2] * v[2] - 1.0) <= 1e-6,
                    OVS_ERR_INVALID_ARG, "bearing of correspondence %d is not a finite unit vector", i);
        OVS_REQUIRE(scale_factor[i] > 0.0f && scale_factor[i] <= 90.0f, OVS_ERR_INVALID_ARG,
                    "scale_factor of correspondence %d must be in (0, 90]", i);
    }
    if (n_all == 0) {
        for (int b = 0; b < B; ++b) {
            ovs::pnp_identity(pose_cw + 12 * (size_t)b);
            valid[b] = 0; num_inliers[b] = 0; best_iter[b] = -1;
        }
        return OVS_OK;
    }
    OVS_CUDA_CHECK(cudaSetDevice(h->device));
    invalidate_plan(h);
    if (h->pending) { OVS_CUDA_CHECK(ovs::sync_stream(h->stream)); h->pending = false; }
    const size_t N = (size_t)n_all, NB = (size_t)B, H = (size_t)max_num_iter;
    const size_t in_bytes_max = 256 * 7 + (NB + 1) * 4 + N * (24 + 24 + 4) + NB * (8 + 8);
    const size_t out_bytes_max = 256 * 5 + NB * (12 * 8 + 4 + 4 + 1) + N;
    const size_t hbytes = in_bytes_max + out_bytes_max;
    const size_t dbytes = hbytes + 256 * 3 + N * (8 + 4) + NB * H * 96 + 4096;
    int rc = ensure_arenas(h, dbytes, hbytes);
    if (rc != OVS_OK) return rc;
    Arena Hh{h->h_arena, 0, h->h_cap}, D{h->d_arena, 0, h->d_cap};
    int* hoff = Hh.take<int>(NB + 1);
    double* hbear = Hh.take<double>(3 * N); double* hpw = Hh.take<double>(3 * N); float* hsf = Hh.take<float>(N);
    uint64_t* hseed = Hh.take<uint64_t>(NB); unsigned long long* hkey = Hh.take<unsigned long long>(NB);
    const size_t in_bytes = Hh.off;
    double* hpose = Hh.take<double>(12 * NB);
    const size_t out_begin = (size_t)((uint8_t*)hpose - h->h_arena);
    int* hnum = Hh.take<int>(NB); int* hbest = Hh.take<int>(NB); uint8_t* hvalid = Hh.take<uint8_t>(NB); uint8_t* hflags = Hh.take<uint8_t>(N);
    const size_t out_end = Hh.off;
    PnpArgs A;
    A.B = B; A.N = n_all; A.H = max_num_iter; A.min_num_inliers = min_num_inliers; A.recompute = recompute ? 1 : 0;
    A.off = D.take<int>(NB + 1);
    A.bear = D.take<double>(3 * N); A.pw = D.take<double>(3 * N); A.sf = D.take<float>(N);
    A.seed = D.take<uint64_t>(NB); A.key = D.take<unsigned long long>(NB);
    A.pose = D.take<double>(12 * NB); A.num_inliers = D.take<int>(NB); A.best_iter = D.take<int>(NB); A.valid = D.take<uint8_t>(NB);
    A.inlier = D.take<uint8_t>(N);
    A.bound = D.take<double>(N); A.cidx = D.take<int>(N); A.hyp = D.take<double>(12 * NB * H);
    memcpy(hoff, corr_offsets, 4 * (NB + 1));
    memcpy(hbear, bearings, 24 * N); memcpy(hpw, pos_w, 24 * N); memcpy(hsf, scale_factor, 4 * N);
    memcpy(hseed, seeds, 8 * NB); memset(hkey, 0, 8 * NB);
    cudaStream_t st = h->stream;
    OVS_CUDA_CHECK(cudaMemcpyAsync(h->d_arena, h->h_arena, in_bytes, cudaMemcpyHostToDevice, st));
    const size_t hyp_threads = std::max(N, NB * H);
    k_pnp_hypotheses<<<(unsigned)((hyp_threads + kPnpHypThreads - 1) / kPnpHypThreads), kPnpHypThreads, 0, st>>>(A);
    OVS_LAUNCH_CHECK();
    if (max_num_iter > 0) {
        k_pnp_ransac<<<dim3((max_num_iter + kPnpWarps - 1) / kPnpWarps, B), kPnpThreads, 0, st>>>(A);
        OVS_LAUNCH_CHECK();
    }
    k_pnp_refine<<<B, kPnpRefineThreads, 0, st>>>(A);
    OVS_LAUNCH_CHECK();
    OVS_CUDA_CHECK(cudaMemcpyAsync(h->h_arena + out_begin, h->d_arena + out_begin, out_end - out_begin, cudaMemcpyDeviceToHost, st));
    OVS_CUDA_CHECK(ovs::sync_stream(st));
    memcpy(pose_cw, hpose, 12 * 8 * NB);
    memcpy(num_inliers, hnum, 4 * NB); memcpy(best_iter, hbest, 4 * NB); memcpy(valid, hvalid, NB);
    memcpy(inlier_out, hflags, N);
    return OVS_OK;
}

struct ovs_ba_plan {
    bool valid = false;
    BaDev P{};
    int K = 0, L = 0, M = 0, nfree = 0, n = 0, npairs = 0, nb_obs = 0, nb_upd = 0;
    long long npair_entries = 0;
    size_t chol_smem = 0;
    int chol_dbuf = 0, chol_big = 0;
    double* hposes = nullptr; double* hpoints = nullptr; uint8_t* hout = nullptr;
    LmCtl* hctl = nullptr; int* hexec = nullptr; int exec_cap = 0;
    double *dposes_in = nullptr, *dpoints_in = nullptr;
    double *dposes_ring = nullptr, *dpoints_ring = nullptr;
    uint8_t* dlevel = nullptr; double* derr = nullptr;
    uint8_t* dout = nullptr;
    LmCtl* dctl = nullptr; int* dexec = nullptr;
    size_t spart_stride = 0, S_stride = 0, invL_stride = 0;
    double *dHpl = nullptr, *dCpp = nullptr, *dbpo = nullptr, *dAll = nullptr, *dblo = nullptr;
    double *dHll = nullptr, *dbl = nullptr, *dHpp = nullptr, *dbp = nullptr;
    double *dS = nullptr, *dbS = nullptr, *dx = nullptr, *dinvL = nullptr;
    int4* d_pair_rec = nullptr; int *dsegb = nullptr, *dsege = nullptr; int2* dpab = nullptr; int* ddiag = nullptr;
    int4 *dchunks = nullptr, *ddchunks = nullptr; int *dpair_chunk_begin = nullptr, *dkf_chunk_begin = nullptr;
    int* dnchunks = nullptr;
    double *dspart = nullptr, *dppart = nullptr; int max_chunks = 0, max_dchunks = 0;
    double *dpchi = nullptr, *dpscale = nullptr; int* dfail = nullptr; double* dmaxdiag = nullptr; long long* dclk = nullptr;
    int cur = 0;
};

namespace {

struct DenseSolve {
    double* S; size_t S_stride; int n; double* x; double* invL; size_t invL_stride; int* fail; long long* clk;
    int chol_big, chol_dbuf; size_t chol_smem;
};

void dense_solve_config(int n, DenseSolve& ds) {
    const size_t fixed = chol_fixed_doubles(n), panel = chol_panel_doubles(n), back = chol_back_doubles(n) - 32 * 33;
    const size_t one = (fixed + std::max(panel, back)) * sizeof(double);
    const size_t two = (fixed + std::max(panel, back + chol_back_doubles(n))) * sizeof(double);
    ds.chol_big = one > (size_t)kCholMaxDynSmem ? 1 : 0;
    ds.chol_dbuf = two <= (size_t)kCholMaxDynSmem ? 1 : 0;
    ds.chol_smem = ds.chol_big ? 0 : (ds.chol_dbuf ? two : one);
}

struct BaInputs {
    const double* poses; const uint8_t* fixed; const double* points; const int32_t* obs_kf; const int32_t* obs_lm;
    const float* obs_xy; const float* obs_x_right; const float* inv_sigma_sq;
};

int ensure_work(ovs_optimizer* h, size_t bytes) {
    if (bytes > h->w_cap) {
        cudaFree(h->d_work); h->d_work = nullptr; h->w_cap = 0;
        bytes += bytes / 4;
        OVS_CUDA_CHECK(cudaMalloc(&h->d_work, bytes));
        h->w_cap = bytes;
    }
    return OVS_OK;
}

int prepare_impl(ovs_optimizer* h, const ovs_camera* cam, int setup_is_mono, int K, int L, int M, const BaInputs& in, bool on_device) {
    OVS_REQUIRE(h && cam && K > 0 && L > 0 && M > 0, OVS_ERR_INVALID_ARG, "bad argument");
    OVS_REQUIRE(in.poses && in.fixed && in.points && in.obs_kf && in.obs_lm && in.obs_xy && in.inv_sigma_sq, OVS_ERR_INVALID_ARG, "null argument");
    OVS_REQUIRE(cam->model == ovs::kCamPerspective || cam->model == ovs::kCamEquirectangular, OVS_ERR_INVALID_ARG, "unknown camera model");
    OVS_CUDA_CHECK(cudaSetDevice(h->device));
    ovs_ba_plan& pl = *h->plan;
    pl.valid = false;
    cudaStream_t st = h->stream;
    if (h->pending) { OVS_CUDA_CHECK(ovs::sync_stream(st)); h->pending = false; }

    const size_t sM = (size_t)M, sL = (size_t)L, sK = (size_t)K;
    const int nb_obs = (M + 127) / 128, nb_upd = (L + K + 127) / 128;
    const int exec_cap = 1024;
    double* hposes; double* hpoints; int *hkf, *hlm; float *hxy, *hxr, *hw; uint8_t* hfixed; uint8_t* hout; long long* hcounts;
    double* dposes_in; double* dpoints_in; int *dkf, *dlm; float *dxy, *dxr, *dw; uint8_t* dfixed;
    int *dfree, *dlmf, *dpoff; long long* dcounts;
    size_t in_bytes = 0;
    auto carve1 = [&](Arena& H, Arena& D) {
        hposes = H.take<double>(12 * sK); hpoints = H.take<double>(3 * sL);
        hkf = H.take<int>(sM); hlm = H.take<int>(sM); hxy = H.take<float>(2 * sM); hxr = H.take<float>(sM); hw = H.take<float>(sM);
        hfixed = H.take<uint8_t>(sK);
        in_bytes = H.off;
        hout = H.take<uint8_t>(sM); pl.hctl = H.take<LmCtl>(1); pl.hexec = H.take<int>(exec_cap); hcounts = H.take<long long>(8);
        dposes_in = D.take<double>(12 * sK); dpoints_in = D.take<double>(3 * sL);
        dkf = D.take<int>(sM); dlm = D.take<int>(sM); dxy = D.take<float>(2 * sM); dxr = D.take<float>(sM); dw = D.take<float>(sM);
        dfixed = D.take<uint8_t>(sK);
        dfree = D.take<int>(sK); dlmf = D.take<int>(sL + 1); dpoff = D.take<int>(sL + 1); dcounts = D.take<long long>(8);
        pl.dout = D.take<uint8_t>(sM); pl.dctl = D.take<LmCtl>(1); pl.dexec = D.take<int>(exec_cap);
        pl.dposes_ring = D.take<double>((kSpec + 1) * 12 * sK); pl.dpoints_ring = D.take<double>((kSpec + 1) * 3 * sL);
        pl.dlevel = D.take<uint8_t>(sM); pl.derr = D.take<double>(kSpec * 3 * sM);
        pl.dHpl = D.take<double>(18 * sM); pl.dCpp = D.take<double>(21 * sM); pl.dbpo = D.take<double>(6 * sM);
        pl.dAll = D.take<double>(6 * sM); pl.dblo = D.take<double>(3 * sM);
        pl.dHll = D.take<double>(6 * sL); pl.dbl = D.take<double>(3 * sL);
        pl.dpchi = D.take<double>(kSpec * (size_t)nb_obs); pl.dpscale = D.take<double>(kSpec * (size_t)nb_upd);
        pl.dfail = D.take<int>(kSpec); pl.dmaxdiag = D.take<double>(2); pl.dclk = D.take<long long>(192); pl.dnchunks = D.take<int>(2);
    };
    {
        Arena H0{nullptr, 0, 0}, D0{nullptr, 0, 0};
        carve1(H0, D0);
        const int rc = ensure_arenas(h, D0.off + 256, H0.off + 256);
        if (rc != OVS_OK) return rc;
    }
    Arena H{h->h_arena, 0, h->h_cap}, D{h->d_arena, 0, h->d_cap};
    carve1(H, D);
    pl.exec_cap = exec_cap;
    h->pending = true;
    if (!on_device) {
        memcpy(hposes, in.poses, 96 * sK); memcpy(hpoints, in.points, 24 * sL);
        memcpy(hkf, in.obs_kf, 4 * sM); memcpy(hlm, in.obs_lm, 4 * sM); memcpy(hxy, in.obs_xy, 8 * sM); memcpy(hw, in.inv_sigma_sq, 4 * sM);
        if (in.obs_x_right) memcpy(hxr, in.obs_x_right, 4 * sM); else for (size_t i = 0; i < sM; ++i) hxr[i] = -1.0f;
        memcpy(hfixed, in.fixed, sK);
        OVS_CUDA_CHECK(cudaMemcpyAsync(h->d_arena, h->h_arena, in_bytes, cudaMemcpyHostToDevice, st));
    } else {
        const cudaMemcpyKind dd = cudaMemcpyDeviceToDevice;
        OVS_CUDA_CHECK(cudaMemcpyAsync(dposes_in, in.poses, 96 * sK, dd, st)); OVS_CUDA_CHECK(cudaMemcpyAsync(dpoints_in, in.points, 24 * sL, dd, st));
        OVS_CUDA_CHECK(cudaMemcpyAsync(dkf, in.obs_kf, 4 * sM, dd, st)); OVS_CUDA_CHECK(cudaMemcpyAsync(dlm, in.obs_lm, 4 * sM, dd, st));
        OVS_CUDA_CHECK(cudaMemcpyAsync(dxy, in.obs_xy, 8 * sM, dd, st)); OVS_CUDA_CHECK(cudaMemcpyAsync(dw, in.inv_sigma_sq, 4 * sM, dd, st));
        if (in.obs_x_right) OVS_CUDA_CHECK(cudaMemcpyAsync(dxr, in.obs_x_right, 4 * sM, dd, st));
        else { k_fill_f32<<<(unsigned)((sM + 255) / 256), 256, 0, st>>>(dxr, sM, -1.0f); OVS_LAUNCH_CHECK(); }
        OVS_CUDA_CHECK(cudaMemcpyAsync(dfixed, in.fixed, sK, dd, st));
    }
    hcounts[0] = 0; hcounts[1] = 0; hcounts[2] = 0; hcounts[3] = 0; hcounts[4] = 0x7fffffffffffffffll;
    OVS_CUDA_CHECK(cudaMemcpyAsync(dcounts, hcounts, 5 * sizeof(long long), cudaMemcpyHostToDevice, st));
    k_ba_free_index<<<1, 1024, 0, st>>>(K, dfixed, dfree, dcounts);
    OVS_LAUNCH_CHECK();
    k_ba_landmark_index<<<(M + 255) / 256, 256, 0, st>>>(M, L, K, dkf, dlm, dlmf, dcounts);
    OVS_LAUNCH_CHECK();
    k_ba_pair_counts<<<(L + 255) / 256, 256, 0, st>>>(L, dlmf, dkf, dfree, dpoff, dcounts);
    OVS_LAUNCH_CHECK();
    k_ba_pair_offsets<<<1, 1024, 0, st>>>(L, dpoff, dcounts);
    OVS_LAUNCH_CHECK();
    OVS_CUDA_CHECK(cudaMemcpyAsync(hcounts, dcounts, 5 * sizeof(long long), cudaMemcpyDeviceToHost, st));
    OVS_CUDA_CHECK(ovs::sync_stream(st));
    if (hcounts[4] != 0x7fffffffffffffffll) {
        const long long i = hcounts[4] >> 2;
        const int code = (int)(hcounts[4] & 3);
        h->pending = false;
        if (code == 2) { ovs::set_error("observations must be grouped by landmark (obs_lm non-decreasing; first violation at observation %lld)", i); return OVS_ERR_INVALID_ARG; }
        if (!on_device) ovs::set_error("observation %lld references keyframe %d / landmark %d out of range", i, in.obs_kf[i], in.obs_lm[i]);
        else ovs::set_error("observation %lld references a keyframe / landmark out of range", i);
        return OVS_ERR_INVALID_ARG;
    }
    const int nfree = (int)hcounts[0];
    const long long npair_entries = hcounts[1], nfree_edges = hcounts[2];
    const int n = 6 * nfree;
    OVS_REQUIRE(nfree >= 1, OVS_ERR_INVALID_ARG, "no free keyframe");
    OVS_REQUIRE(n <= kMaxReducedDimBig, OVS_ERR_UNSUPPORTED, "more than %d free keyframes", kMaxReducedDimBig / 6);
    OVS_REQUIRE(npair_entries < (1ll << 30), OVS_ERR_UNSUPPORTED, "too many co-observations");
    const int npairs = nfree * (nfree + 1) / 2;

    const size_t sE = (size_t)std::max<long long>(npair_entries, 1);
    const size_t max_chunks = sE / 128 + (size_t)npairs + 8;
    const size_t max_dchunks = (size_t)nfree_edges / 128 + (size_t)nfree + 8;
    unsigned *dkeys, *dkeys2; unsigned long long *dvals, *dvals2; int4* dprec; int* dsort;
    auto carve2 = [&](Arena& W) {
        pl.dpab = W.take<int2>(npairs); pl.ddiag = W.take<int>(nfree);
        pl.dHpp = W.take<double>(21 * (size_t)nfree); pl.dbp = W.take<double>(6 * (size_t)nfree);
        pl.S_stride = ((size_t)(n + 1) * n + 31) / 32 * 32; pl.invL_stride = (size_t)((n + kNB - 1) / kNB) * kNB * kNB;
        pl.dS = W.take<double>(kSpec * pl.S_stride); pl.dbS = pl.dS + (size_t)n * n; pl.dx = W.take<double>(kSpec * (size_t)n);
        pl.dinvL = W.take<double>(kSpec * pl.invL_stride);
        dkeys = W.take<unsigned>(sE); dkeys2 = W.take<unsigned>(sE);
        dvals = W.take<unsigned long long>(sE); dvals2 = W.take<unsigned long long>(sE); dprec = W.take<int4>(sE);
        dsort = W.take<int>(sort_scratch_ints((long long)sE));
        pl.dsegb = W.take<int>(npairs); pl.dsege = W.take<int>(npairs);
        pl.dchunks = W.take<int4>(max_chunks); pl.ddchunks = W.take<int4>(max_dchunks);
        pl.dpair_chunk_begin = W.take<int>(npairs + 1); pl.dkf_chunk_begin = W.take<int>(nfree + 1);
        pl.spart_stride = 42 * max_chunks;
        pl.dspart = W.take<double>(kSpec * pl.spart_stride); pl.dppart = W.take<double>(27 * max_dchunks);
    };
    {
        Arena W0{nullptr, 0, 0};
        carve2(W0);
        const int rc = ensure_work(h, W0.off + 256);
        if (rc != OVS_OK) return rc;
    }
    Arena W{h->d_work, 0, h->w_cap};
    carve2(W);
    pl.max_chunks = (int)max_chunks; pl.max_dchunks = (int)max_dchunks;
    OVS_CUDA_CHECK(cudaMemsetAsync(pl.dsegb, 0, 4 * (size_t)npairs, st));
    OVS_CUDA_CHECK(cudaMemsetAsync(pl.dsege, 0, 4 * (size_t)npairs, st));
    OVS_CUDA_CHECK(cudaMemsetAsync(pl.dS, 0, 8 * kSpec * pl.S_stride, st));

    BaDev& P = pl.P;
    P.cam = to_cam(cam); P.K = K; P.L = L; P.M = M; P.nfree = nfree; P.n = n;
    P.poses = dposes_in; P.points = dpoints_in; P.poses_ring = pl.dposes_ring; P.points_ring = pl.dpoints_ring;
    P.obs_kf = dkf; P.obs_lm = dlm; P.obs_xy = (const float2*)dxy; P.obs_xr = dxr; P.inv_sigma_sq = dw;
    P.level = pl.dlevel; P.free_idx = dfree; P.lm_first = dlmf;
    const float chi_sq_2D = 5.99146f, chi_sq_3D = 7.81473f;
    P.use_huber = 1; P.delta = (double)(setup_is_mono ? sqrtf(chi_sq_2D) : sqrtf(chi_sq_3D));

    k_ba_pair_table<<<nfree, 128, 0, st>>>(nfree, pl.dpab, pl.ddiag);
    OVS_LAUNCH_CHECK();
    pl.d_pair_rec = dprec;
    if (npair_entries > 0) {
        k_ba_emit_pairs<<<(L + 127) / 128, 128, 0, st>>>(P, dpoff, dkeys, dvals);
        OVS_LAUNCH_CHECK();
        int end_bit = 1;
        while ((1 << end_bit) < npairs) ++end_bit;
        unsigned* ksorted = nullptr; unsigned long long* vsorted = nullptr;
        const int src = sort_pairs(st, dkeys, dkeys2, dvals, dvals2, (int)npair_entries, end_bit, dsort, &ksorted, &vsorted);
        if (src != OVS_OK) return src;
        k_ba_segments<<<((int)npair_entries + 255) / 256, 256, 0, st>>>(ksorted, (int)npair_entries, pl.dsegb, pl.dsege);
        OVS_LAUNCH_CHECK();
        k_ba_pair_records<<<((int)npair_entries + 255) / 256, 256, 0, st>>>(vsorted, (int)npair_entries, dlm, dprec);
        OVS_LAUNCH_CHECK();
    }
    k_ba_chunk_scan<<<1, 1024, 0, st>>>(nullptr, npairs, pl.dsegb, pl.dsege, pl.dpair_chunk_begin, pl.dnchunks);
    OVS_LAUNCH_CHECK();
    k_ba_chunk_fill<<<(npairs + 127) / 128, 128, 0, st>>>(nullptr, npairs, pl.dsegb, pl.dsege, pl.dpair_chunk_begin, pl.dchunks);
    OVS_LAUNCH_CHECK();
    k_ba_chunk_scan<<<1, 1024, 0, st>>>(pl.ddiag, nfree, pl.dsegb, pl.dsege, pl.dkf_chunk_begin, pl.dnchunks + 1);
    OVS_LAUNCH_CHECK();
    k_ba_chunk_fill<<<(nfree + 127) / 128, 128, 0, st>>>(pl.ddiag, nfree, pl.dsegb, pl.dsege, pl.dkf_chunk_begin, pl.ddchunks);
    OVS_LAUNCH_CHECK();

    pl.K = K; pl.L = L; pl.M = M; pl.nfree = nfree; pl.n = n; pl.npairs = npairs; pl.nb_obs = nb_obs; pl.nb_upd = nb_upd;
    pl.npair_entries = npair_entries;
    {
        DenseSolve ds{};
        dense_solve_config(n, ds);
        pl.chol_big = ds.chol_big; pl.chol_dbuf = ds.chol_dbuf; pl.chol_smem = ds.chol_smem;
    }
    pl.hposes = hposes; pl.hpoints = hpoints; pl.hout = hout;
    pl.dposes_in = dposes_in; pl.dpoints_in = dpoints_in;
    pl.cur = 0;
    pl.valid = true;
    return OVS_OK;
}

}

extern "C" int ovs_local_ba_prepare(ovs_optimizer* h, const ovs_camera* cam, int setup_is_mono, int K, const double* poses,
                                    const uint8_t* fixed, int L, const double* points, int M, const int32_t* obs_kf,
                                    const int32_t* obs_lm, const float* obs_xy, const float* obs_x_right, const float* inv_sigma_sq) {
    const BaInputs in{poses, fixed, points, obs_kf, obs_lm, obs_xy, obs_x_right, inv_sigma_sq};
    return prepare_impl(h, cam, setup_is_mono, K, L, M, in, false);
}

extern "C" int ovs_local_ba_prepare_device(ovs_optimizer* h, const ovs_camera* cam, int setup_is_mono, int K, const double* d_poses,
                                           const uint8_t* d_fixed, int L, const double* d_points, int M, const int32_t* d_obs_kf,
                                           const int32_t* d_obs_lm, const float* d_obs_xy, const float* d_obs_x_right, const float* d_inv_sigma_sq) {
    const BaInputs in{d_poses, d_fixed, d_points, d_obs_kf, d_obs_lm, d_obs_xy, d_obs_x_right, d_inv_sigma_sq};
    return prepare_impl(h, cam, setup_is_mono, K, L, M, in, true);
}

extern "C" int ovs_local_ba_fetch_device(ovs_optimizer* h, double* d_poses, double* d_points, uint8_t* d_outlier_out) {
    OVS_REQUIRE(h && h->plan->valid, OVS_ERR_INVALID_ARG, "no prepared bundle-adjustment problem");
    OVS_CUDA_CHECK(cudaSetDevice(h->device));
    ovs_ba_plan& pl = *h->plan;
    cudaStream_t st = h->stream;
    const size_t sK = (size_t)pl.K, sL = (size_t)pl.L, sM = (size_t)pl.M;
    if (d_poses) OVS_CUDA_CHECK(cudaMemcpyAsync(d_poses, pl.dposes_ring + (size_t)pl.cur * 12 * sK, 96 * sK, cudaMemcpyDeviceToDevice, st));
    if (d_points) OVS_CUDA_CHECK(cudaMemcpyAsync(d_points, pl.dpoints_ring + (size_t)pl.cur * 3 * sL, 24 * sL, cudaMemcpyDeviceToDevice, st));
    if (d_outlier_out) OVS_CUDA_CHECK(cudaMemcpyAsync(d_outlier_out, pl.dout, sM, cudaMemcpyDeviceToDevice, st));
    OVS_CUDA_CHECK(ovs::sync_stream(st));
    h->pending = false;
    return OVS_OK;
}

static void invalidate_plan(ovs_optimizer* h) { h->plan->valid = false; }

namespace {

int wait_for_run(ovs_optimizer* h, cudaEvent_t done, const volatile uint8_t* force_stop_flag) {
    if (!force_stop_flag) { OVS_CUDA_CHECK(ovs::sync_event(done)); return OVS_OK; }
    const bool blocking = ovs::blocking_waits();
    for (;;) {
        const cudaError_t q = cudaEventQuery(done);
        if (q == cudaSuccess) break;
        if (q != cudaErrorNotReady) OVS_CUDA_CHECK(q);
        if (*force_stop_flag) *(volatile int*)(h->h_mirror + 2) = 1;
        if (blocking) { struct timespec ts = {0, 50000}; nanosleep(&ts, nullptr); } else sched_yield();
    }
    return OVS_OK;
}

int launch_dense_solve(ovs_optimizer* h, cudaStream_t st, LmCtl* ctl, const DenseSolve& ds) {
    const int n = ds.n;
    if (!ds.chol_big) {
        cudaLaunchConfig_t cfg = {};
        cfg.gridDim = dim3((unsigned)(h->chol_cluster * kSpec));
        cfg.blockDim = dim3(kCholThreads);
        cfg.dynamicSmemBytes = ds.chol_smem;
        cfg.stream = st;
        cudaLaunchAttribute at[1];
        at[0].id = cudaLaunchAttributeClusterDimension;
        at[0].val.clusterDim.x = (unsigned)h->chol_cluster; at[0].val.clusterDim.y = 1; at[0].val.clusterDim.z = 1;
        cfg.attrs = at; cfg.numAttrs = 1;
        OVS_CUDA_CHECK(cudaLaunchKernelEx(&cfg, k_ba_cholesky_solve, (const LmCtl*)ctl, ds.S, ds.S_stride, n, ds.x, ds.invL, ds.invL_stride, ds.fail, ds.clk, ds.chol_dbuf));
        ovs::count_launch();
    } else {
        for (int kb = 0; kb < n; kb += kNB) {
            const int nb = std::min(kNB, n - kb), rem = n - kb - nb, prow = rem + 1;
            k_chol_big_diag<<<dim3(1, kSpec), 64, 0, st>>>(ctl, ds.S, ds.S_stride, n, kb, nb, ds.invL, ds.invL_stride, ds.fail);
            OVS_LAUNCH_CHECK();
            k_chol_big_panel<<<dim3((prow + 127) / 128, kSpec), 128, 0, st>>>(ctl, ds.S, ds.S_stride, n, kb, nb, ds.invL, ds.invL_stride);
            OVS_LAUNCH_CHECK();
            if (rem > 0) {
                int tiles = 0;
                for (int mi = 0; mi < (prow + 15) / 16; ++mi) tiles += std::min((rem + 31) / 32, (16 * mi + 15) / 32 + 1);
                k_chol_big_trailing<<<dim3((tiles + 3) / 4, kSpec), 128, 0, st>>>(ctl, ds.S, ds.S_stride, n, kb, nb);
                OVS_LAUNCH_CHECK();
            }
        }
        const size_t bsm = (size_t)(((n + 31) / 32) * 32 + 32 * 33 + 32) * sizeof(double);
        k_chol_big_backsolve<<<kSpec, 512, bsm, st>>>(ctl, ds.S, ds.S_stride, n, ds.invL, ds.invL_stride, ds.x, ds.fail);
        OVS_LAUNCH_CHECK();
    }
    return OVS_OK;
}

struct LmDriver {
    ovs_optimizer* h = nullptr; cudaStream_t st = nullptr; LmCtl* ctl = nullptr;
    const volatile int* stop_word = nullptr; double* maxdiag = nullptr; volatile int* mirror = nullptr; volatile int* hm = nullptr;
    bool host_sync = false, use_graph = false;
    std::function<int()> errors_at_current;
    std::function<int(bool in_graph, bool halt_if_undecided)> iteration_head;
    std::function<int(bool in_graph, bool halt_if_undecided, int next_width_cap)> trial_batch;
    std::function<int()> wait_device;
};

int lm_round(LmDriver& D, int iterations, int use_huber) {
    ovs_optimizer* const h = D.h;
    const cudaStream_t st = D.st;
    LmCtl* const ctl = D.ctl;
    volatile int* const hm = D.hm;
    auto finish_iteration = [&]() -> int {
        for (;;) {
            int rc = D.wait_device();
            if (rc != OVS_OK) return rc;
            if (hm[0] == 0) return OVS_OK;
            rc = D.trial_batch(false, false, 0);
            if (rc != OVS_OK) return rc;
        }
    };
    k_lm_round_begin<<<1, 1, 0, st>>>(ctl, iterations, use_huber, D.stop_word, D.maxdiag, D.mirror);
    OVS_LAUNCH_CHECK();
    if (iterations > 0) {
        const int rc = D.errors_at_current();
        if (rc != OVS_OK) return rc;
    }
    bool captured = false;
    int it0 = 0;
    while (it0 < iterations) {
        if (D.host_sync) {
            int rc = D.iteration_head(false, false);
            if (rc != OVS_OK) return rc;
            rc = finish_iteration();
            if (rc != OVS_OK) return rc;
            if (hm[1] == 0) break;
            it0 = hm[4];
            continue;
        }
        for (int it = it0; it < iterations; ++it) {
            if (D.use_graph) {
                if (!captured) {
                    OVS_CUDA_CHECK(cudaStreamBeginCapture(st, cudaStreamCaptureModeThreadLocal));
                    const int rc_body = D.iteration_head(true, true);
                    cudaGraph_t g = nullptr;
                    const cudaError_t ce = cudaStreamEndCapture(st, &g);
                    if (rc_body != OVS_OK) { if (g) cudaGraphDestroy(g); return rc_body; }
                    OVS_CUDA_CHECK(ce);
                    if (h->gx_iter) {
                        cudaGraphExecUpdateResultInfo info;
                        if (cudaGraphExecUpdate(h->gx_iter, g, &info) != cudaSuccess) { cudaGetLastError(); cudaGraphExecDestroy(h->gx_iter); h->gx_iter = nullptr; }
                    }
                    if (!h->gx_iter) {
                        const cudaError_t ie = cudaGraphInstantiate(&h->gx_iter, g, 0);
                        if (ie != cudaSuccess) { cudaGraphDestroy(g); OVS_CUDA_CHECK(ie); }
                    }
                    cudaGraphDestroy(g);
                    captured = true;
                }
                OVS_CUDA_CHECK(cudaGraphLaunch(h->gx_iter, st));
            } else {
                const int rc = D.iteration_head(false, true);
                if (rc != OVS_OK) return rc;
            }
        }
        int rc = D.wait_device();
        if (rc != OVS_OK) return rc;
        if (hm[3] == 0) break;
        k_lm_resume<<<1, 1, 0, st>>>(ctl, D.mirror);
        OVS_LAUNCH_CHECK();
        rc = D.trial_batch(false, false, 0);
        if (rc != OVS_OK) return rc;
        rc = finish_iteration();
        if (rc != OVS_OK) return rc;
        if (hm[1] == 0) break;
        it0 = hm[4];
    }
    k_lm_round_end<<<1, 1, 0, st>>>(ctl, D.stop_word, D.mirror);
    OVS_LAUNCH_CHECK();
    return OVS_OK;
}

}

namespace {
int run_impl(ovs_optimizer* h, int rounds, int huber_first, int num_first_iter, int num_second_iter, const volatile uint8_t* force_stop_flag,
             ovs_ba_stats* stats) {
    OVS_REQUIRE(h && h->plan->valid, OVS_ERR_INVALID_ARG, "no prepared bundle-adjustment problem");
    OVS_REQUIRE(num_first_iter >= 0 && num_second_iter >= 0, OVS_ERR_INVALID_ARG, "bad iteration counts");
    OVS_CUDA_CHECK(cudaSetDevice(h->device));
    if (stats) memset(stats, 0, sizeof(*stats));
    ovs_ba_plan& pl = *h->plan;
    cudaStream_t st = h->stream;
    const int L = pl.L, K = pl.K, M = pl.M, n = pl.n, nfree = pl.nfree, npairs = pl.npairs, nb_obs = pl.nb_obs, nb_upd = pl.nb_upd;
    const size_t sM = (size_t)M, pose_sz = 12 * (size_t)K, point_sz = 3 * (size_t)L;
    const BaDev P = pl.P;
    const float chi_sq_2D = 5.99146f, chi_sq_3D = 7.81473f;
    LmCtl* const ctl = pl.dctl;
    volatile int* const stop_word = h->d_mirror + 2;
    h->h_mirror[0] = 0; h->h_mirror[1] = 0; h->h_mirror[2] = 0;
    h->pending = true;
    OVS_CUDA_CHECK(cudaEventRecord(h->ev[0], st));
    OVS_CUDA_CHECK(cudaMemcpyAsync(pl.dposes_ring, pl.dposes_in, 8 * pose_sz, cudaMemcpyDeviceToDevice, st));
    OVS_CUDA_CHECK(cudaMemcpyAsync(pl.dpoints_ring, pl.dpoints_in, 8 * point_sz, cudaMemcpyDeviceToDevice, st));
    OVS_CUDA_CHECK(cudaMemsetAsync(pl.dlevel, 0, sM, st));
    OVS_CUDA_CHECK(cudaMemsetAsync(pl.derr, 0, 24 * sM, st));
    OVS_CUDA_CHECK(cudaMemsetAsync(pl.dout, 0, sM, st));
    if (pl.npair_entries > 0) {
        k_ba_pair_flags<<<((int)pl.npair_entries + 255) / 256, 256, 0, st>>>(pl.dlevel, pl.d_pair_rec, (int)pl.npair_entries);
        OVS_LAUNCH_CHECK();
    }
    pl.cur = 0;
    if (force_stop_flag && *force_stop_flag) { OVS_CUDA_CHECK(ovs::sync_stream(st)); h->pending = false; return OVS_OK; }

    const bool host_sync = h->lm_host_sync >= 0 ? h->lm_host_sync != 0 : pl.chol_big != 0;
    const bool use_graph = h->use_graphs && !host_sync;
    volatile int* const mirror = (volatile int*)h->d_mirror;
    volatile int* const hm = (volatile int*)h->h_mirror;
    const int sw = std::min(std::max(h->spec_width, 1), kSpec);
    const int sw2 = std::min(std::max(h->spec_width2, 0), kSpec);
    const bool time_solver = stats != nullptr;
    int solver_slots = 0;

    k_lm_init<<<1, 1, 0, st>>>(ctl, sw, pl.dfail, mirror);
    OVS_LAUNCH_CHECK();

    auto wait_device = [&]() -> int {
        if (!force_stop_flag) { OVS_CUDA_CHECK(ovs::sync_stream(st)); return OVS_OK; }
        OVS_CUDA_CHECK(cudaEventRecord(h->ev[1], st));
        return wait_for_run(h, h->ev[1], force_stop_flag);
    };

    auto trial_batch = [&](bool in_graph, bool halt_if_undecided, int next_width_cap) -> int {
        const int slot = solver_slots;
        const bool ev = time_solver && !in_graph && slot < pl.exec_cap;
        if (ev) {
            while (h->solver_ev.size() < 4 * (size_t)(slot + 1)) {
                cudaEvent_t e0;
                OVS_CUDA_CHECK(cudaEventCreateWithFlags(&e0, cudaEventDefault));
                h->solver_ev.push_back(e0);
            }
            OVS_CUDA_CHECK(cudaEventRecord(h->solver_ev[4 * slot], st));
        }
        k_ba_schur_chunk<<<pl.max_chunks, 128, 0, st>>>(P, ctl, pl.dnchunks, pl.d_pair_rec, pl.dchunks, pl.dpab, pl.dHll, pl.dHpl, pl.dbl, pl.dspart, pl.spart_stride);
        OVS_LAUNCH_CHECK();
        k_ba_schur_final<<<dim3(npairs, kSpec), 64, 0, st>>>(n, ctl, pl.dpair_chunk_begin, pl.dpab, pl.dspart, pl.spart_stride, pl.dHpp, pl.dbp, pl.dS, pl.S_stride);
        OVS_LAUNCH_CHECK();
        if (ev) OVS_CUDA_CHECK(cudaEventRecord(h->solver_ev[4 * slot + 1], st));
        const DenseSolve ds{pl.dS, pl.S_stride, n, pl.dx, pl.dinvL, pl.invL_stride, pl.dfail, pl.dclk, pl.chol_big, pl.chol_dbuf, pl.chol_smem};
        const int rc_solve = launch_dense_solve(h, st, ctl, ds);
        if (rc_solve != OVS_OK) return rc_solve;
        if (ev) OVS_CUDA_CHECK(cudaEventRecord(h->solver_ev[4 * slot + 3], st));
        k_ba_update<<<nb_upd, 128, 0, st>>>(P, ctl, pl.dHpl, pl.dHll, pl.dbl, pl.dbp, pl.dx, pl.dposes_ring, pl.dpoints_ring, pl.dpscale, pl.dfail);
        OVS_LAUNCH_CHECK();
        k_ba_errors<<<dim3(nb_obs, kSpec), 128, 0, st>>>(P, ctl, 0, pl.derr, pl.dpchi);
        OVS_LAUNCH_CHECK();
        k_ba_reduce<<<1, kSpec * 256, 0, st>>>(ctl, 1, pl.dpchi, nb_obs, pl.dpscale, nb_upd, pl.dfail, stop_word, ev ? slot : -1, pl.dexec, mirror,
                                               halt_if_undecided ? 1 : 0, next_width_cap);
        OVS_LAUNCH_CHECK();
        if (!in_graph) ++solver_slots;
        return OVS_OK;
    };

    auto iteration_head = [&](bool in_graph, bool halt_if_undecided) -> int {
        k_ba_linearize<<<nb_obs, 128, 0, st>>>(P, ctl, pl.dHpl, pl.dCpp, pl.dbpo, pl.dAll, pl.dblo);
        OVS_LAUNCH_CHECK();
        k_ba_landmark_accum<<<(L + 127) / 128, 128, 0, st>>>(P, ctl, pl.dAll, pl.dblo, pl.dHll, pl.dbl, pl.dmaxdiag);
        OVS_LAUNCH_CHECK();
        k_ba_pose_accum_chunk<<<pl.max_dchunks, 128, 0, st>>>(P, ctl, pl.dnchunks + 1, pl.d_pair_rec, pl.ddchunks, pl.dCpp, pl.dbpo, pl.dppart);
        OVS_LAUNCH_CHECK();
        k_ba_pose_final_plan<<<1, 1024, 0, st>>>(ctl, nfree, pl.dkf_chunk_begin, pl.dppart, pl.dHpp, pl.dbp, pl.dmaxdiag, pl.dfail, stop_word, mirror);
        OVS_LAUNCH_CHECK();
        if (sw2 > 0 && halt_if_undecided) {
            const int rc = trial_batch(in_graph, false, sw2);
            if (rc != OVS_OK) return rc;
        }
        return trial_batch(in_graph, halt_if_undecided, 0);
    };

    LmDriver drv;
    drv.h = h; drv.st = st; drv.ctl = ctl; drv.stop_word = stop_word; drv.maxdiag = pl.dmaxdiag; drv.mirror = mirror; drv.hm = hm;
    drv.host_sync = host_sync; drv.use_graph = use_graph;
    drv.errors_at_current = [&]() -> int {
        k_ba_errors<<<dim3(nb_obs, 1), 128, 0, st>>>(P, ctl, 1, pl.derr, pl.dpchi);
        OVS_LAUNCH_CHECK();
        k_ba_reduce<<<1, kSpec * 256, 0, st>>>(ctl, 0, pl.dpchi, nb_obs, pl.dpscale, 0, pl.dfail, stop_word, -1, nullptr, nullptr, 0, 0);
        OVS_LAUNCH_CHECK();
        return OVS_OK;
    };
    drv.iteration_head = iteration_head;
    drv.trial_batch = trial_batch;
    drv.wait_device = wait_device;
    auto lm_optimize = [&](int iterations, int use_huber) -> int { return lm_round(drv, iterations, use_huber); };

    int rc = lm_optimize(num_first_iter, huber_first);
    if (rc != OVS_OK) return rc;
    if (rounds == 2) {
        k_ba_classify<<<nb_obs, 128, 0, st>>>(P, ctl, pl.derr, (double)chi_sq_2D, (double)chi_sq_3D, 0, pl.dlevel, pl.dout);
        OVS_LAUNCH_CHECK();
        k_ba_replicate_err<<<(unsigned)((3 * sM + 255) / 256), 256, 0, st>>>(ctl, pl.derr, 3 * sM);
        OVS_LAUNCH_CHECK();
        if (pl.npair_entries > 0) {
            k_ba_pair_flags<<<((int)pl.npair_entries + 255) / 256, 256, 0, st>>>(pl.dlevel, pl.d_pair_rec, (int)pl.npair_entries);
            OVS_LAUNCH_CHECK();
        }
        rc = lm_optimize(num_second_iter, 0);
        if (rc != OVS_OK) return rc;
        k_ba_classify<<<nb_obs, 128, 0, st>>>(P, ctl, pl.derr, (double)chi_sq_2D, (double)chi_sq_3D, 1, pl.dlevel, pl.dout);
        OVS_LAUNCH_CHECK();
    }
    OVS_CUDA_CHECK(cudaMemcpyAsync(pl.hctl, ctl, sizeof(LmCtl), cudaMemcpyDeviceToHost, st));
    const int nslots = std::min(solver_slots, pl.exec_cap);
    if (time_solver && nslots > 0) OVS_CUDA_CHECK(cudaMemcpyAsync(pl.hexec, pl.dexec, sizeof(int) * (size_t)nslots, cudaMemcpyDeviceToHost, st));
    OVS_CUDA_CHECK(cudaEventRecord(h->ev[1], st));
    if (force_stop_flag) rc = wait_for_run(h, h->ev[1], force_stop_flag);
    else { OVS_CUDA_CHECK(ovs::sync_event(h->ev[1])); rc = OVS_OK; }
    if (rc != OVS_OK) return rc;
    h->pending = false;
    const LmCtl& c = *pl.hctl;
    pl.cur = c.cur;
    if (stats) {
        stats->num_rounds = c.num_rounds;
        stats->num_iterations = c.num_iterations; stats->num_trials = c.num_trials;
        for (int r = 0; r < 8; ++r) { stats->round_iterations[r] = c.round_iterations[r]; stats->lambda_init[r] = c.lambda_init[r]; }
        stats->last_lambda = c.last_lambda; stats->last_chi2 = c.last_chi2; stats->final_chi2 = c.last_chi2;
        float ms = 0; cudaEventElapsedTime(&ms, h->ev[0], h->ev[1]);
        stats->device_us = ms * 1000.f;
        float sum = 0, sum_schur = 0;
        if (time_solver)
            for (int i = 0; i < nslots; ++i)
                if (pl.hexec[i] > 0) {
                    float m = 0;
                    cudaEventElapsedTime(&m, h->solver_ev[4 * i + 1], h->solver_ev[4 * i + 3]); sum += m;
                    cudaEventElapsedTime(&m, h->solver_ev[4 * i], h->solver_ev[4 * i + 1]); sum_schur += m;
                }
        stats->solver_us = sum * 1000.f;
        stats->schur_us = sum_schur * 1000.f;
        stats->co_observations = (int32_t)pl.npair_entries;
        stats->solver_launches = c.batches;
        stats->solver_trials = c.solver_trials;
        stats->reduced_dim = n;
    }
    return OVS_OK;
}
}

extern "C" int ovs_local_ba_run(ovs_optimizer* h, int num_first_iter, int num_second_iter, const volatile uint8_t* force_stop_flag,
                                ovs_ba_stats* stats) {
    return run_impl(h, 2, 1, num_first_iter, num_second_iter, force_stop_flag, stats);
}

extern "C" int ovs_global_ba_host(ovs_optimizer* h, const ovs_camera* cam, int setup_is_mono, int K, double* poses, const uint8_t* fixed,
                                  int L, double* points, int M, const int32_t* obs_kf, const int32_t* obs_lm, const float* obs_xy,
                                  const float* obs_x_right, const float* inv_sigma_sq, int num_iter, int use_huber_kernel,
                                  const volatile uint8_t* force_stop_flag, ovs_ba_stats* stats) {
    OVS_REQUIRE(h && cam && K > 0 && L >= 0 && M >= 0 && num_iter >= 0, OVS_ERR_INVALID_ARG, "bad argument");
    OVS_REQUIRE(poses && fixed && (L == 0 || points) && (M == 0 || (obs_kf && obs_lm && obs_xy && inv_sigma_sq)), OVS_ERR_INVALID_ARG, "null argument");
    if (stats) memset(stats, 0, sizeof(*stats));
    if (force_stop_flag && *force_stop_flag) return OVS_OK;
    if (M == 0 || L == 0) return OVS_OK;
    int rc = ovs_local_ba_prepare(h, cam, setup_is_mono, K, poses, fixed, L, points, M, obs_kf, obs_lm, obs_xy, obs_x_right, inv_sigma_sq);
    if (rc != OVS_OK) return rc;
    rc = run_impl(h, 1, use_huber_kernel ? 1 : 0, num_iter, 0, force_stop_flag, stats);
    if (rc != OVS_OK) return rc;
    return ovs_local_ba_fetch(h, poses, points, nullptr);
}

extern "C" int ovs_optimizer_cluster_width(const ovs_optimizer* h) { return h ? h->chol_cluster : 0; }

extern "C" int ovs_optimizer_set_cluster_width(ovs_optimizer* h, int width) {
    OVS_REQUIRE(h && (width == 1 || width == 2 || width == 4 || width == 8), OVS_ERR_INVALID_ARG, "cluster width must be 1, 2, 4 or 8");
    h->chol_cluster = width;
    return OVS_OK;
}

extern "C" int ovs_optimizer_set_speculation(ovs_optimizer* h, int width) {
    OVS_REQUIRE(h && width >= 1 && width <= kSpec, OVS_ERR_INVALID_ARG, "speculation width must be 1..%d", kSpec);
    h->spec_width = width;
    return OVS_OK;
}

extern "C" int ovs_optimizer_set_second_batch(ovs_optimizer* h, int width) {
    OVS_REQUIRE(h && width >= 0 && width <= kSpec, OVS_ERR_INVALID_ARG, "second-batch width must be 0..%d", kSpec);
    h->spec_width2 = width;
    return OVS_OK;
}

extern "C" int ovs_optimizer_set_graphs(ovs_optimizer* h, int enable) {
    OVS_REQUIRE(h, OVS_ERR_INVALID_ARG, "null handle");
    h->use_graphs = enable ? 1 : 0;
    return OVS_OK;
}

extern "C" int ovs_optimizer_set_host_sync(ovs_optimizer* h, int mode) {
    OVS_REQUIRE(h && mode >= -1 && mode <= 1, OVS_ERR_INVALID_ARG, "host-sync mode must be -1 (auto), 0 or 1");
    h->lm_host_sync = mode;
    return OVS_OK;
}

extern "C" int ovs_optimizer_debug_clocks(ovs_optimizer* h, long long* out192) {
    OVS_REQUIRE(h && out192 && h->plan->valid, OVS_ERR_INVALID_ARG, "no prepared bundle-adjustment problem");
    OVS_CUDA_CHECK(cudaSetDevice(h->device));
    OVS_CUDA_CHECK(cudaMemcpy(out192, h->plan->dclk, 192 * sizeof(long long), cudaMemcpyDeviceToHost));
    return OVS_OK;
}

extern "C" int ovs_debug_sort_pairs(int device, const uint32_t* keys, const uint64_t* vals, int n, int end_bit, uint32_t* keys_out, uint64_t* vals_out) {
    OVS_REQUIRE(keys && vals && keys_out && vals_out && n >= 0 && end_bit >= 1 && end_bit <= 32, OVS_ERR_INVALID_ARG, "bad argument");
    if (n == 0) return OVS_OK;
    OVS_CUDA_CHECK(cudaSetDevice(device));
    const size_t sn = (size_t)n;
    unsigned *k0 = nullptr, *k1 = nullptr; unsigned long long *v0 = nullptr, *v1 = nullptr; int* scratch = nullptr;
    auto release = [&]() { cudaFree(k0); cudaFree(k1); cudaFree(v0); cudaFree(v1); cudaFree(scratch); };
    int rc = OVS_OK;
    do {
        if (cudaMalloc(&k0, 4 * sn) != cudaSuccess || cudaMalloc(&k1, 4 * sn) != cudaSuccess || cudaMalloc(&v0, 8 * sn) != cudaSuccess ||
            cudaMalloc(&v1, 8 * sn) != cudaSuccess || cudaMalloc(&scratch, 4 * sort_scratch_ints(n)) != cudaSuccess) {
            cudaGetLastError(); ovs::set_error("ovs_debug_sort_pairs: out of device memory"); rc = OVS_ERR_CUDA; break;
        }
        if (cudaMemcpy(k0, keys, 4 * sn, cudaMemcpyHostToDevice) != cudaSuccess || cudaMemcpy(v0, vals, 8 * sn, cudaMemcpyHostToDevice) != cudaSuccess) {
            ovs::set_error("ovs_debug_sort_pairs: upload failed"); rc = OVS_ERR_CUDA; break;
        }
        unsigned* ks = nullptr; unsigned long long* vs = nullptr;
        rc = sort_pairs(nullptr, k0, k1, v0, v1, n, end_bit, scratch, &ks, &vs);
        if (rc != OVS_OK) break;
        if (cudaDeviceSynchronize() != cudaSuccess || cudaMemcpy(keys_out, ks, 4 * sn, cudaMemcpyDeviceToHost) != cudaSuccess ||
            cudaMemcpy(vals_out, vs, 8 * sn, cudaMemcpyDeviceToHost) != cudaSuccess) {
            ovs::set_error("ovs_debug_sort_pairs: %s", cudaGetErrorString(cudaGetLastError())); rc = OVS_ERR_CUDA; break;
        }
    } while (0);
    release();
    return rc;
}

extern "C" int ovs_local_ba_fetch(ovs_optimizer* h, double* poses, double* points, uint8_t* outlier_out) {
    OVS_REQUIRE(h && h->plan->valid, OVS_ERR_INVALID_ARG, "no prepared bundle-adjustment problem");
    OVS_CUDA_CHECK(cudaSetDevice(h->device));
    ovs_ba_plan& pl = *h->plan;
    cudaStream_t st = h->stream;
    const size_t sK = (size_t)pl.K, sL = (size_t)pl.L, sM = (size_t)pl.M;
    OVS_CUDA_CHECK(cudaMemcpyAsync(pl.hposes, pl.dposes_ring + (size_t)pl.cur * 12 * sK, 96 * sK, cudaMemcpyDeviceToHost, st));
    OVS_CUDA_CHECK(cudaMemcpyAsync(pl.hpoints, pl.dpoints_ring + (size_t)pl.cur * 3 * sL, 24 * sL, cudaMemcpyDeviceToHost, st));
    OVS_CUDA_CHECK(cudaMemcpyAsync(pl.hout, pl.dout, sM, cudaMemcpyDeviceToHost, st));
    OVS_CUDA_CHECK(ovs::sync_stream(st));
    h->pending = false;
    if (poses) memcpy(poses, pl.hposes, 96 * sK);
    if (points) memcpy(points, pl.hpoints, 24 * sL);
    if (outlier_out) memcpy(outlier_out, pl.hout, sM);
    return OVS_OK;
}

extern "C" int ovs_local_ba_host(ovs_optimizer* h, const ovs_camera* cam, int setup_is_mono, int K, double* poses, const uint8_t* fixed,
                                 int L, double* points, int M, const int32_t* obs_kf, const int32_t* obs_lm, const float* obs_xy,
                                 const float* obs_x_right, const float* inv_sigma_sq, int num_first_iter, int num_second_iter,
                                 const volatile uint8_t* force_stop_flag, uint8_t* outlier_out, ovs_ba_stats* stats) {
    OVS_REQUIRE(h && cam && K > 0 && L >= 0 && M >= 0, OVS_ERR_INVALID_ARG, "bad argument");
    OVS_REQUIRE(poses && fixed && (L == 0 || points) && (M == 0 || (obs_kf && obs_lm && obs_xy && inv_sigma_sq && outlier_out)),
                OVS_ERR_INVALID_ARG, "null argument");
    if (stats) memset(stats, 0, sizeof(*stats));
    for (int i = 0; i < M; ++i) outlier_out[i] = 0;
    if (force_stop_flag && *force_stop_flag) return OVS_OK;
    if (M == 0 || L == 0) return OVS_OK;
    int rc = ovs_local_ba_prepare(h, cam, setup_is_mono, K, poses, fixed, L, points, M, obs_kf, obs_lm, obs_xy, obs_x_right, inv_sigma_sq);
    if (rc != OVS_OK) return rc;
    rc = ovs_local_ba_run(h, num_first_iter, num_second_iter, force_stop_flag, stats);
    if (rc != OVS_OK) return rc;
    return ovs_local_ba_fetch(h, poses, points, outlier_out);
}

extern "C" int ovs_optimizer_create(int device, ovs_optimizer** out) {
    OVS_REQUIRE(out, OVS_ERR_INVALID_ARG, "null argument");
    int rc = ovs::select_device(device);
    if (rc != OVS_OK) return rc;
    ovs_optimizer* h = new (std::nothrow) ovs_optimizer();
    OVS_REQUIRE(h, OVS_ERR_CUDA, "out of host memory");
    h->device = device;
    h->plan = new (std::nothrow) ovs_ba_plan();
    OVS_REQUIRE(h->plan, OVS_ERR_CUDA, "out of host memory");
    bool ok = cudaStreamCreateWithFlags(&h->stream, cudaStreamNonBlocking) == cudaSuccess
              && cudaEventCreateWithFlags(&h->ev[0], ovs::event_flags()) == cudaSuccess && cudaEventCreateWithFlags(&h->ev[1], ovs::event_flags()) == cudaSuccess
              && cudaHostAlloc(&h->h_mirror, 16 * sizeof(int), cudaHostAllocMapped) == cudaSuccess
              && cudaHostGetDevicePointer(&h->d_mirror, h->h_mirror, 0) == cudaSuccess
              && cudaFuncSetAttribute(k_ba_cholesky_solve, cudaFuncAttributeMaxDynamicSharedMemorySize, kCholMaxDynSmem) == cudaSuccess
              && cudaFuncSetAttribute(k_chol_big_backsolve, cudaFuncAttributeMaxDynamicSharedMemorySize, 60 * 1024) == cudaSuccess;
    if (!ok) {
        ovs::set_error("optimizer handle setup failed: %s", cudaGetErrorString(cudaGetLastError()));
        ovs_optimizer_destroy(h);
        return OVS_ERR_CUDA;
    }
    {
        if (const char* e = getenv("OVS_B200_GRAPHS")) h->use_graphs = atoi(e);
        if (const char* e = getenv("OVS_B200_LM_HOST_SYNC")) h->lm_host_sync = atoi(e) ? 1 : 0;
        if (const char* e = getenv("OVS_B200_SPEC2")) h->spec_width2 = std::min(kSpec, std::max(0, atoi(e)));
        if (const char* e = getenv("OVS_B200_SPEC")) h->spec_width = std::min(kSpec, std::max(1, atoi(e)));
        int want = kCholCluster;
        if (const char* e = getenv("OVS_B200_CHOL_CLUSTER")) want = atoi(e);
        if (want > kCholCluster && cudaFuncSetAttribute(k_ba_cholesky_solve, cudaFuncAttributeNonPortableClusterSizeAllowed, 1) == cudaSuccess) {
            cudaLaunchConfig_t cfg = {};
            cfg.gridDim = dim3((unsigned)(want * kSpec));
            cfg.blockDim = dim3(kCholThreads);
            cfg.dynamicSmemBytes = kCholMaxDynSmem;
            cudaLaunchAttribute at[1];
            at[0].id = cudaLaunchAttributeClusterDimension;
            at[0].val.clusterDim.x = (unsigned)want; at[0].val.clusterDim.y = 1; at[0].val.clusterDim.z = 1;
            cfg.attrs = at; cfg.numAttrs = 1;
            int nclusters = 0;
            const cudaError_t qe = cudaOccupancyMaxActiveClusters(&nclusters, k_ba_cholesky_solve, &cfg);
            if (qe == cudaSuccess && nclusters >= kSpec) h->chol_cluster = want;
            if (getenv("OVS_B200_DEBUG")) fprintf(stderr, "ovs_b200: %d-CTA clusters: query %s, %d co-resident (need %d) -> using %d\n", want, cudaGetErrorString(qe), nclusters, kSpec, h->chol_cluster);
        } else if (want >= 1 && want <= kCholCluster) {
            h->chol_cluster = want;
        }
        cudaGetLastError();
    }
    *out = h;
    return OVS_OK;
}

extern "C" void ovs_optimizer_destroy(ovs_optimizer* h) {
    if (!h) return;
    cudaSetDevice(h->device);
    if (h->stream) ovs::sync_stream(h->stream);
    cudaFree(h->d_arena); cudaFree(h->d_work); cudaFreeHost(h->h_arena); cudaFreeHost(h->h_mirror);
    for (auto& e : h->ev) if (e) cudaEventDestroy(e);
    for (auto& e : h->solver_ev) cudaEventDestroy(e);
    if (h->gx_iter) cudaGraphExecDestroy(h->gx_iter);
    if (h->stream) cudaStreamDestroy(h->stream);
    delete h->plan;
    delete h;
}


namespace {

constexpr int kPgBlk = 161;

struct PgDev {
    int K, E, nfree, n, fix_scale;
    double* ring;
    const int* free_idx;
    const int* ei; const int* ej; const double* meas;
};

__host__ __device__ __forceinline__ int pg_pair_id(int r, int c) { return r * (r + 1) / 2 + c; }

__global__ void __launch_bounds__(256) k_pg_emit(PgDev P, unsigned sentinel, unsigned* __restrict__ keys, unsigned long long* __restrict__ vals) {
    const int e = blockIdx.x * 256 + threadIdx.x;
    if (e >= P.E) return;
    const int a = P.free_idx[P.ei[e]], b = P.free_idx[P.ej[e]];
    const unsigned long long v = (unsigned long long)e << 2;
    keys[3 * (size_t)e] = a >= 0 ? (unsigned)pg_pair_id(a, a) : sentinel;
    vals[3 * (size_t)e] = v;
    keys[3 * (size_t)e + 1] = b >= 0 ? (unsigned)pg_pair_id(b, b) : sentinel;
    vals[3 * (size_t)e + 1] = v | 1;
    unsigned k2 = sentinel;
    unsigned long long v2 = v | 2;
    if (a >= 0 && b >= 0) {
        if (a > b) k2 = (unsigned)pg_pair_id(a, b);
        else { k2 = (unsigned)pg_pair_id(b, a); v2 = v | 3; }
    }
    keys[3 * (size_t)e + 2] = k2;
    vals[3 * (size_t)e + 2] = v2;
}

__device__ __forceinline__ void pg_load13(const double* src, double* dst) {
#pragma unroll
    for (int k = 0; k < 13; ++k) dst[k] = src[k];
}

__global__ void __launch_bounds__(128) k_pg_linearize(PgDev P, const LmCtl* __restrict__ ctl, double* __restrict__ blk) {
    if (!ctl->active) return;
    const int e = blockIdx.x * 128 + threadIdx.x;
// ... 392 lines not shown
```

Measured before the change: 397.7.

## Store compact per-edge Jacobian records and fuse landmark accumulation into linearize

The linearize kernel now writes a compact per-edge record (Jp, Jl, weight, residual) instead of precomputed Hpl/Cpp/bpo/All/blo blocks. Downstream kernels (pose accumulation, Schur chunk, update) recompute their products from this record, templated on 2 or 3 residual rows. Landmark Hll/bl accumulation is folded into linearize through precomputed landmark-aligned edge blocks. The goal is less global memory traffic and one fewer launch, paid for with extra recomputation in several kernels and an explicit round-to-nearest arithmetic path that keeps results identical.

```diff
diff --git a/openvslam_b200/csrc/ba_math.cuh b/openvslam_b200/csrc/ba_math.cuh
--- a/openvslam_b200/csrc/ba_math.cuh
+++ b/openvslam_b200/csrc/ba_math.cuh
@@ -136,4 +136,79 @@
 OVS_BA_HD int sym3(int i, int j) { return i <= j ? (i * 3 - i * (i - 1) / 2 + (j - i)) : (j * 3 - j * (j - 1) / 2 + (i - j)); }
 OVS_BA_HD int sym6(int i, int j) { return i <= j ? (i * 6 - i * (i - 1) / 2 + (j - i)) : (j * 6 - j * (j - 1) / 2 + (i - j)); }
 
-}
+OVS_BA_HD double rn_mul(double a, double b) {
+#if defined(__CUDA_ARCH__)
+    return __dmul_rn(a, b);
+#else
+    return a * b;
+#endif
+}
+OVS_BA_HD double rn_add(double a, double b) {
+#if defined(__CUDA_ARCH__)
+    return __dadd_rn(a, b);
+#else
+    return a + b;
+#endif
+}
+OVS_BA_HD double rn_sub(double a, double b) {
+#if defined(__CUDA_ARCH__)
+    return __dsub_rn(a, b);
+#else
+    return a - b;
+#endif
+}
+
+template <int R, class Out>
+OVS_BA_HD void edge_hpl_each(const double* Jp, const double* Jl, double ww, int dim, Out&& out) {
+    for (int a = 0; a < 6; ++a)
+        for (int b = 0; b < 3; ++b) {
+            double h = 0;
+            for (int d = 0; d < R; ++d)
+                if (d < dim) h = rn_add(h, rn_mul(rn_mul(Jp[6 * d + a], ww), Jl[3 * d + b]));
+            out(a, b, h);
+        }
+}
+template <int R>
+OVS_BA_HD void edge_hpl(const double* Jp, const double* Jl, double ww, int dim, double* W) {
+    edge_hpl_each<R>(Jp, Jl, ww, dim, [W](int a, int b, double h) { W[3 * a + b] = h; });
+}
+template <int R>
+OVS_BA_HD void edge_hll(const double* Jl, double ww, int dim, double* A) {
+    for (int a = 0; a < 3; ++a)
+        for (int b = a; b < 3; ++b) {
+            double h = 0;
+            for (int d = 0; d < R; ++d)
+                if (d < dim) h = rn_add(h, rn_mul(rn_mul(Jl[3 * d + a], ww), Jl[3 * d + b]));
+            A[sym3(a, b)] = h;
+        }
+}
+template <int R>
+OVS_BA_HD void edge_hpp(const double* Jp, double ww, int dim, double* C) {
+    for (int a = 0; a < 6; ++a)
+        for (int b = a; b < 6; ++b) {
+            double h = 0;
+            for (int d = 0; d < R; ++d)
+                if (d < dim) h = rn_add(h, rn_mul(rn_mul(Jp[6 * d + a], ww), Jp[6 * d + b]));
+            C[sym6(a, b)] = h;
+        }
+}
+template <int R>
+OVS_BA_HD void edge_bp(const double* Jp, double ww, const double* e, int dim, double* bp) {
+    for (int a = 0; a < 6; ++a) {
+        double g = 0;
+        for (int d = 0; d < R; ++d)
+            if (d < dim) g = rn_sub(g, rn_mul(rn_mul(Jp[6 * d + a], ww), e[d]));
+        bp[a] = g;
+    }
+}
+template <int R>
+OVS_BA_HD void edge_bl(const double* Jl, double ww, const double* e, int dim, double* bl) {
+    for (int a = 0; a < 3; ++a) {
+        double g = 0;
+        for (int d = 0; d < R; ++d)
+            if (d < dim) g = rn_sub(g, rn_mul(rn_mul(Jl[3 * d + a], ww), e[d]));
+        bl[a] = g;
+    }
+}
+
+}
diff --git a/openvslam_b200/csrc/optimize.cu b/openvslam_b200/csrc/optimize.cu
--- a/openvslam_b200/csrc/optimize.cu
+++ b/openvslam_b200/csrc/optimize.cu
@@ -112,130 +112,116 @@
     int use_huber; double delta;
 };
 
-__global__ void __launch_bounds__(128) k_ba_linearize(BaDev P, const LmCtl* __restrict__ ctl, double* __restrict__ Hpl, double* __restrict__ Cpp,
-                                                       double* __restrict__ bpo, double* __restrict__ All, double* __restrict__ blo) {
-    if (!ctl->active) return;
-    __shared__ __align__(16) double sm[128 * 30];
+template <int R> struct EdgeRec {
+    static constexpr int kJl = 6 * R, kWw = 9 * R, kE = 9 * R + 1;
+    static constexpr int kSize = (10 * R + 2) / 2 * 2;
+    static constexpr int kHpl2 = (9 * R + 2) / 2;
+    static constexpr int kTail0 = 9 * R / 2, kTail1 = (10 * R + 2) / 2;
+};
+constexpr int kLbSegEdges = 2048, kLbSegCap = 2 * (kLbSegEdges / 128) + 2, kLbThreads = 256;
+template <int R> __device__ __forceinline__ int edge_dim(const BaDev& P, size_t i) { return R == 3 && P.obs_xr[i] >= 0.0f ? 3 : 2; }
+
+template <int R>
+__global__ void __launch_bounds__(128) k_ba_linearize(BaDev P, const LmCtl* __restrict__ ctl, const int* __restrict__ nblocks,
+                                                       const int4* __restrict__ lblocks, double* __restrict__ rec,
+                                                       double* __restrict__ Hll, double* __restrict__ bl, double* __restrict__ maxdiag) {
+    using ER = EdgeRec<R>;
+    constexpr int RS = ER::kSize;
+    __shared__ __align__(16) double s_rec[128 * RS];
+    __shared__ double s_hll[128 * 6], s_bl[128 * 3];
+    __shared__ unsigned char s_live[128];
+    if (!ctl->active || (int)(blockIdx.x % kLbSegCap) >= nblocks[blockIdx.x / kLbSegCap]) return;
     P.poses = P.poses_ring + (size_t)ctl->cur * 12 * P.K; P.points = P.points_ring + (size_t)ctl->cur * 3 * P.L;
     P.use_huber = ctl->use_huber;
-    const int base = blockIdx.x * 128, t = threadIdx.x;
-    const int i = base + t;
-    const int nedge = min(128, P.M - base);
-    const bool live = i < P.M && !P.level[i];
-    int dim = 0, fi = -1;
-    double e[3] = {0, 0, 0}, Jp[18], Jl[9], ww = 0;
-#pragma unroll
-    for (int k = 0; k < 18; ++k) Jp[k] = 0;
-#pragma unroll
-    for (int k = 0; k < 9; ++k) Jl[k] = 0;
-    if (live) {
-        const int kf = P.obs_kf[i], lm = P.obs_lm[i];
-        fi = P.free_idx[kf];
-        const float xr = P.obs_xr ? P.obs_xr[i] : -1.0f;
-        const bool stereo = xr >= 0.0f;
-        const float2 xy = P.obs_xy[i];
-        const double obs[3] = {(double)xy.x, (double)xy.y, (double)xr};
-        double pose[12], pw[3];
-#pragma unroll
-        for (int k = 0; k < 12; ++k) pose[k] = P.poses[12 * (size_t)kf + k];
-#pragma unroll
-        for (int k = 0; k < 3; ++k) pw[k] = P.points[3 * (size_t)lm + k];
-        dim = ovs::edge_eval(P.cam, pose, pw, obs, stereo, e, Jp, Jl);
-        const double w = (double)P.inv_sigma_sq[i];
-        double chi = 0;
-        for (int d = 0; d < dim; ++d) chi += w * e[d] * e[d];
-        double rho0 = chi, rho1 = 1.0;
-        if (P.use_huber) ovs::huber(chi, P.delta, &rho0, &rho1);
-        ww = rho1 * w;
-    }
-    double* sW = sm; double* sbp = sm + 128 * 18; double* sA = sbp + 128 * 6;
-    {
-        double* A = sA + 6 * t;
-        for (int a = 0; a < 3; ++a)
-            for (int b = a; b < 3; ++b) {
-                double h = 0;
-                for (int d = 0; d < dim; ++d) h += Jl[3 * d + a] * ww * Jl[3 * d + b];
-                A[ovs::sym3(a, b)] = h;
-            }
-        double* W = sW + 18 * t; double* bp = sbp + 6 * t;
-        const bool fr = fi >= 0;
-        for (int a = 0; a < 6; ++a) {
-            double g = 0;
-            for (int d = 0; d < dim; ++d) g -= Jp[6 * d + a] * ww * e[d];
-            bp[a] = fr ? g : 0.0;
-            for (int b = 0; b < 3; ++b) {
-                double h = 0;
-                for (int d = 0; d < dim; ++d) h += Jp[6 * d + a] * ww * Jl[3 * d + b];
-                W[3 * a + b] = fr ? h : 0.0;
-            }
-        }
-    }
-    __syncthreads();
-    {
-        const double2* s2 = reinterpret_cast<const double2*>(sW); double2* g2 = reinterpret_cast<double2*>(Hpl + 18 * (size_t)base);
-        for (int q = t; q < 9 * nedge; q += 128) g2[q] = s2[q];
-        s2 = reinterpret_cast<const double2*>(sbp); g2 = reinterpret_cast<double2*>(bpo + 6 * (size_t)base);
-        for (int q = t; q < 3 * nedge; q += 128) g2[q] = s2[q];
-        s2 = reinterpret_cast<const double2*>(sA); g2 = reinterpret_cast<double2*>(All + 6 * (size_t)base);
-        for (int q = t; q < 3 * nedge; q += 128) g2[q] = s2[q];
-    }
-    __syncthreads();
-    double* sC = sm; double* sbl = sm + 128 * 21;
-    {
-        double* C = sC + 21 * t; double* bl = sbl + 3 * t;
-        const bool fr = fi >= 0;
-        for (int a = 0; a < 6; ++a)
-            for (int b = a; b < 6; ++b) {
-                double h = 0;
-                for (int d = 0; d < dim; ++d) h += Jp[6 * d + a] * ww * Jp[6 * d + b];
-                C[ovs::sym6(a, b)] = fr ? h : 0.0;
-            }
-        for (int a = 0; a < 3; ++a) {
-            double g = 0;
-            for (int d = 0; d < dim; ++d) g -= Jl[3 * d + a] * ww * e[d];
-            bl[a] = g;
-        }
-    }
-    __syncthreads();
-    {
-        const double2* s2 = reinterpret_cast<const double2*>(sC); double2* g2 = reinterpret_cast<double2*>(Cpp + 21 * (size_t)base);
-        const int nd = 21 * nedge;
-        for (int q = t; q < nd / 2; q += 128) g2[q] = s2[q];
-        if ((nd & 1) && t == 0) Cpp[21 * (size_t)base + nd - 1] = sC[nd - 1];
-        const int nb = 3 * nedge;
-        for (int q = t; q < nb; q += 128) blo[3 * (size_t)base + q] = sbl[q];
-    }
-}
-
-__global__ void __launch_bounds__(128) k_ba_landmark_accum(BaDev P, const LmCtl* __restrict__ ctl, const double* __restrict__ All, const double* __restrict__ blo,
-                                                            double* __restrict__ Hll, double* __restrict__ bl, double* __restrict__ maxdiag) {
-    if (!ctl->active) return;
-    const int l = blockIdx.x * 128 + threadIdx.x;
-    double md = 0;
-    if (l < P.L) {
-        double H[6] = {0, 0, 0, 0, 0, 0}, b[3] = {0, 0, 0};
-        for (int p = P.lm_first[l]; p < P.lm_first[l + 1]; ++p) {
-            if (P.level[p]) continue;
-#pragma unroll
-            for (int k = 0; k < 6; ++k) H[k] += All[6 * (size_t)p + k];
-#pragma unroll
-            for (int k = 0; k < 3; ++k) b[k] += blo[3 * (size_t)p + k];
-        }
-#pragma unroll
-        for (int k = 0; k < 6; ++k) Hll[6 * (size_t)l + k] = H[k];
-#pragma unroll
-        for (int k = 0; k < 3; ++k) bl[3 * (size_t)l + k] = b[k];
-        md = fmax(fabs(H[0]), fmax(fabs(H[3]), fabs(H[5])));
+    const int4 blk = lblocks[blockIdx.x];
+    const int t = threadIdx.x;
+    double H[6] = {0, 0, 0, 0, 0, 0}, b[3] = {0, 0, 0}, md = 0;
+    for (int base = blk.z; base < blk.w; base += 128) {
+        const int i = base + t;
+        const int nedge = min(128, blk.w - base);
+        const bool live = i < blk.w && !P.level[i];
+        int dim = 0, fi = -1;
+        double e[3] = {0, 0, 0}, Jp[18], Jl[9], ww = 0;
+#pragma unroll
+        for (int k = 0; k < 18; ++k) Jp[k] = 0;
+#pragma unroll
+        for (int k = 0; k < 9; ++k) Jl[k] = 0;
+        if (live) {
+            const int kf = P.obs_kf[i], lm = P.obs_lm[i];
+            fi = P.free_idx[kf];
+            const float xr = P.obs_xr ? P.obs_xr[i] : -1.0f;
+            const bool stereo = xr >= 0.0f;
+            const float2 xy = P.obs_xy[i];
+            const double obs[3] = {(double)xy.x, (double)xy.y, (double)xr};
+            double pose[12], pw[3];
+#pragma unroll
+            for (int k = 0; k < 12; ++k) pose[k] = P.poses[12 * (size_t)kf + k];
+#pragma unroll
+            for (int k = 0; k < 3; ++k) pw[k] = P.points[3 * (size_t)lm + k];
+            dim = ovs::edge_eval(P.cam, pose, pw, obs, stereo, e, Jp, Jl);
+            const double w = (double)P.inv_sigma_sq[i];
+            double chi = 0;
+            for (int d = 0; d < dim; ++d) chi += w * e[d] * e[d];
+            double rho0 = chi, rho1 = 1.0;
+            if (P.use_huber) ovs::huber(chi, P.delta, &rho0, &rho1);
+            ww = rho1 * w;
+        }
+        {
+            double* r = s_rec + RS * t;
+            const bool fr = fi >= 0;
+#pragma unroll
+            for (int k = 0; k < 6 * R; ++k) r[k] = fr ? Jp[k] : 0.0;
+#pragma unroll
+            for (int k = 0; k < 3 * R; ++k) r[ER::kJl + k] = Jl[k];
+            r[ER::kWw] = ww;
+#pragma unroll
+            for (int k = 0; k < R; ++k) r[ER::kE + k] = e[k];
+#pragma unroll
+            for (int k = ER::kE + R; k < RS; ++k) r[k] = 0.0;
+            ovs::edge_hll<R>(Jl, ww, dim, s_hll + 6 * t);
+            ovs::edge_bl<R>(Jl, ww, e, dim, s_bl + 3 * t);
+            s_live[t] = live ? 1 : 0;
+        }
+        __syncthreads();
+        {
+            const double2* s2 = reinterpret_cast<const double2*>(s_rec); double2* g2 = reinterpret_cast<double2*>(rec + RS * (size_t)base);
+            for (int q = t; q < (RS / 2) * nedge; q += 128) g2[q] = s2[q];
+        }
+        for (int l = blk.x + t; l < blk.y; l += 128) {
+            const int p0 = max(P.lm_first[l], base), p1 = min(P.lm_first[l + 1], base + nedge);
+            if (blk.y - blk.x > 1) {
+#pragma unroll
+                for (int k = 0; k < 6; ++k) H[k] = 0;
+#pragma unroll
+                for (int k = 0; k < 3; ++k) b[k] = 0;
+            }
+            for (int p = p0; p < p1; ++p) {
+                if (!s_live[p - base]) continue;
+#pragma unroll
+                for (int k = 0; k < 6; ++k) H[k] += s_hll[6 * (p - base) + k];
+#pragma unroll
+                for (int k = 0; k < 3; ++k) b[k] += s_bl[3 * (p - base) + k];
+            }
+            if (base + 128 >= blk.w) {
+#pragma unroll
+                for (int k = 0; k < 6; ++k) Hll[6 * (size_t)l + k] = H[k];
+#pragma unroll
+                for (int k = 0; k < 3; ++k) bl[3 * (size_t)l + k] = b[k];
+                md = fmax(md, fmax(fabs(H[0]), fmax(fabs(H[3]), fabs(H[5]))));
+            }
+        }
+        __syncthreads();
     }
 #pragma unroll
     for (int o = 16; o > 0; o >>= 1) md = fmax(md, __shfl_xor_sync(0xffffffffu, md, o));
     if ((threadIdx.x & 31) == 0 && md > 0) atomic_max_pos(maxdiag, md);
 }
 
+template <int R>
 __global__ void __launch_bounds__(128) k_ba_pose_accum_chunk(BaDev P, const LmCtl* __restrict__ ctl, const int* __restrict__ nchunks,
                                                               const int4* __restrict__ pair_rec, const int4* __restrict__ chunks,
-                                                              const double* __restrict__ Cpp, const double* __restrict__ bpo,
-                                                              double* __restrict__ ppart) {
+                                                              const double* __restrict__ rec, double* __restrict__ ppart) {
+    using ER = EdgeRec<R>;
     __shared__ double red[27][4];
     if (!ctl->active || (int)blockIdx.x >= *nchunks) return;
     const int4 ch = chunks[blockIdx.x];
@@ -244,13 +230,18 @@
 #pragma unroll
     for (int k = 0; k < 27; ++k) acc[k] = 0;
     if (e < ch.z) {
-        const int4 rec = pair_rec[e];
-        const int o = rec.x;
-        if (!rec.w) {
-#pragma unroll
-            for (int k = 0; k < 21; ++k) acc[k] = Cpp[21 * (size_t)o + k];
-#pragma unroll
-            for (int k = 0; k < 6; ++k) acc[21 + k] = bpo[6 * (size_t)o + k];
+        const int4 pr = pair_rec[e];
+        const int o = pr.x;
+        if (!pr.w) {
+            const double2* r2 = reinterpret_cast<const double2*>(rec + ER::kSize * (size_t)o);
+            double r[2 * ER::kTail1];
+#pragma unroll
+            for (int k = 0; k < 3 * R; ++k) { const double2 v = r2[k]; r[2 * k] = v.x; r[2 * k + 1] = v.y; }
+#pragma unroll
+            for (int k = ER::kTail0; k < ER::kTail1; ++k) { const double2 v = r2[k]; r[2 * k] = v.x; r[2 * k + 1] = v.y; }
+            const int dim = edge_dim<R>(P, o);
+            ovs::edge_hpp<R>(r, r[ER::kWw], dim, acc);
+            ovs::edge_bp<R>(r, r[ER::kWw], r + ER::kE, dim, acc + 21);
         }
     }
     const int lane = threadIdx.x & 31, wid = threadIdx.x >> 5;
@@ -273,11 +264,13 @@
 }
 
 constexpr int kSGY = 76, kSGW = 84;
+template <int R>
 __global__ void __launch_bounds__(128, 4) k_ba_schur_chunk(BaDev P, const LmCtl* __restrict__ ctl, const int* __restrict__ nchunks,
                                                          const int4* __restrict__ pair_rec, const int4* __restrict__ chunks,
                                                          const int2* __restrict__ pair_ab, const double* __restrict__ Hll,
-                                                         const double* __restrict__ Hpl, const double* __restrict__ bl,
+                                                         const double* __restrict__ rec, const double* __restrict__ bl,
                                                          double* __restrict__ spart, size_t spart_stride) {
+    using ER = EdgeRec<R>;
     __shared__ double s_y[4 * 8 * kSGY];
     __shared__ double s_w[4 * 8 * kSGW];
     double* sYw = s_y + (threadIdx.x >> 5) * 8 * kSGY;
@@ -293,36 +286,53 @@
     double wa[18], hl[6] = {0, 0, 0, 0, 0, 0};
     int lm = -1;
     {
-        double wb[18], gl[3] = {0, 0, 0};
-#pragma unroll
-        for (int k = 0; k < 18; ++k) { wa[k] = 0; wb[k] = 0; }
+        constexpr bool kLoadAFirst = R == 2;
+        double gl[3] = {0, 0, 0}, ra[2 * ER::kHpl2], rb2[2 * ER::kHpl2];
+        double (&rb)[2 * ER::kHpl2] = kLoadAFirst ? rb2 : ra;
+        const double2* pa = nullptr;
+        bool live = false, same = true;
+        int da = 2, db = 2;
+        auto load_rec = [](const double2* p, double (&r)[2 * ER::kHpl2]) {
+#pragma unroll
+            for (int k = 0; k < ER::kHpl2; ++k) { const double2 v = p[k]; r[2 * k] = v.x; r[2 * k + 1] = v.y; }
+        };
+#pragma unroll
+        for (int k = 0; k < 18; ++k) wa[k] = 0;
         if (e < ch.z) {
             const int4 ob = pair_rec[e];
             if (!ob.w) {
+                live = true;
                 lm = ob.z;
-                const double2* pa = reinterpret_cast<const double2*>(Hpl + 18 * (size_t)ob.x);
-                const double2* pb = reinterpret_cast<const double2*>(Hpl + 18 * (size_t)ob.y);
-#pragma unroll
-                for (int k = 0; k < 9; ++k) { const double2 v = pa[k]; wa[2 * k] = v.x; wa[2 * k + 1] = v.y; }
-                if (ob.x == ob.y) {
-#pragma unroll
-                    for (int k = 0; k < 18; ++k) wb[k] = wa[k];
-                } else {
-#pragma unroll
-                    for (int k = 0; k < 9; ++k) { const double2 v = pb[k]; wb[2 * k] = v.x; wb[2 * k + 1] = v.y; }
-                }
+                same = ob.x == ob.y;
+                pa = reinterpret_cast<const double2*>(rec + ER::kSize * (size_t)ob.x);
+                if (kLoadAFirst || same) load_rec(pa, ra);
+                if (!same) load_rec(reinterpret_cast<const double2*>(rec + ER::kSize * (size_t)ob.y), rb);
                 const double2* ph = reinterpret_cast<const double2*>(Hll + 6 * (size_t)lm);
 #pragma unroll
                 for (int k = 0; k < 3; ++k) { const double2 v = ph[k]; hl[2 * k] = v.x; hl[2 * k + 1] = v.y; }
                 if (diag) { gl[0] = bl[3 * (size_t)lm]; gl[1] = bl[3 * (size_t)lm + 1]; gl[2] = bl[3 * (size_t)lm + 2]; }
-            }
-        }
-#pragma unroll
-        for (int kc = 0; kc < 3; ++kc) {
-            const int kk = 3 * (lane & 3) + kc, base = (lane >> 2) * kSGW + (kk >> 2) * 28 + (kk & 3);
-#pragma unroll
-            for (int c = 0; c < 6; ++c) sWw[base + 4 * c] = wb[3 * c + kc];
-            sWw[base + 24] = gl[kc];
+                da = edge_dim<R>(P, ob.x); db = edge_dim<R>(P, ob.y);
+            }
+        }
+        int sb[3];
+#pragma unroll
+        for (int kc = 0; kc < 3; ++kc) { const int kk = 3 * (lane & 3) + kc; sb[kc] = (lane >> 2) * kSGW + (kk >> 2) * 28 + (kk & 3); }
+        auto park = [&](int c, int kc, double v) { sWw[sb[kc] + 4 * c] = v; };
+        if (!live) {
+#pragma unroll
+            for (int c = 0; c < 6; ++c)
+#pragma unroll
+                for (int kc = 0; kc < 3; ++kc) park(c, kc, 0.0);
+        } else if (same) {
+            ovs::edge_hpl_each<R>(ra, ra + ER::kJl, ra[ER::kWw], da, park);
+        } else {
+            ovs::edge_hpl_each<R>(rb, rb + ER::kJl, rb[ER::kWw], db, park);
+        }
+#pragma unroll
+        for (int kc = 0; kc < 3; ++kc) sWw[sb[kc] + 24] = gl[kc];
+        if (live) {
+            if (!kLoadAFirst && !same) load_rec(pa, ra);
+            ovs::edge_hpl<R>(ra, ra + ER::kJl, ra[ER::kWw], da, wa);
         }
     }
     double lam[kSpec];
@@ -966,7 +976,8 @@
     for (int i = tid; i < n; i += 512) x[i] = vec[i];
 }
 
-__global__ void __launch_bounds__(128) k_ba_update(BaDev P, const LmCtl* __restrict__ ctl, const double* __restrict__ Hpl, const double* __restrict__ Hll,
+template <int R>
+__global__ void __launch_bounds__(128) k_ba_update(BaDev P, const LmCtl* __restrict__ ctl, const double* __restrict__ rec, const double* __restrict__ Hll,
                                                     const double* __restrict__ bl, const double* __restrict__ bp, const double* __restrict__ x,
                                                     double* poses_ring, double* points_ring,
                                                     double* __restrict__ partial_scale, int* __restrict__ fail) {
@@ -990,10 +1001,12 @@
         for (int p = P.lm_first[l]; p < P.lm_first[l + 1]; ++p) {
             const int fi = P.free_idx[P.obs_kf[p]];
             if (P.level[p] || fi < 0) continue;
-            double W[18];
-            const double2* pw = reinterpret_cast<const double2*>(Hpl + 18 * (size_t)p);
-#pragma unroll
-            for (int k = 0; k < 9; ++k) { const double2 v = pw[k]; W[2 * k] = v.x; W[2 * k + 1] = v.y; }
+            using ER = EdgeRec<R>;
+            double W[18], er[2 * ER::kHpl2];
+            const double2* pw = reinterpret_cast<const double2*>(rec + ER::kSize * (size_t)p);
+#pragma unroll
+            for (int k = 0; k < ER::kHpl2; ++k) { const double2 v = pw[k]; er[2 * k] = v.x; er[2 * k + 1] = v.y; }
+            ovs::edge_hpl<R>(er, er + ER::kJl, er[ER::kWw], edge_dim<R>(P, p), W);
 #pragma unroll
             for (int bt = 0; bt < kSpec; ++bt) {
                 if (bt < nbatch) {
@@ -1365,9 +1378,10 @@
 }
 
 __global__ void __launch_bounds__(256) k_ba_landmark_index(int M, int L, int K, const int* __restrict__ obs_kf, const int* __restrict__ obs_lm,
-                                                            int* __restrict__ lm_first, long long* counts) {
+                                                            const float* __restrict__ obs_xr, int* __restrict__ lm_first, long long* counts) {
     const int i = blockIdx.x * 256 + threadIdx.x;
     if (i >= M) return;
+    if (obs_xr[i] >= 0.0f) counts[5] = 1;
     const int l = obs_lm[i], k = obs_kf[i];
     int err = 0;
     if (l < 0 || l >= L || k < 0 || k >= K) err = 1;
@@ -1381,6 +1395,55 @@
         for (int q = max(lp, -1) + 1; q <= l; ++q) lm_first[q] = i;
     if (i == M - 1)
         for (int q = l + 1; q <= L; ++q) lm_first[q] = M;
+}
+
+__device__ __forceinline__ int lower_bound_first(const int* __restrict__ lm_first, int L, int v) {
+    int lo = 0, hi = L;
+    while (lo < hi) { const int mid = (lo + hi) >> 1; if (lm_first[mid] < v) lo = mid + 1; else hi = mid; }
+    return lo;
+}
+__global__ void __launch_bounds__(kLbThreads) k_ba_landmark_blocks(int L, const int* __restrict__ lm_first, int4* __restrict__ blocks, int* __restrict__ nblocks) {
+    __shared__ int s_first[kLbThreads + 1];
+    __shared__ int s_range[2];
+    const int lane = threadIdx.x & 31, seg = blockIdx.x;
+    if (threadIdx.x < 2) s_range[threadIdx.x] = lower_bound_first(lm_first, L, (seg + (int)threadIdx.x) * kLbSegEdges);
+    __syncthreads();
+    const int l0 = s_range[0], l1 = (seg + 1 == (int)gridDim.x) ? L : s_range[1];
+    blocks += (size_t)seg * kLbSegCap;
+    int start = l0, s = l0 < L ? lm_first[l0] : 0, nb = 0;
+    for (int c0 = l0; c0 < l1; c0 += kLbThreads) {
+        __syncthreads();
+        for (int q = threadIdx.x; q <= kLbThreads; q += kLbThreads)
+            if (c0 + q <= l1) s_first[q] = lm_first[c0 + q];
+        __syncthreads();
+        if (threadIdx.x >= 32) continue;
+        const int cn = min(kLbThreads, l1 - c0);
+        for (int g = 0; g < cn; g += 32) {
+            const int j = g + lane;
+            const bool in = j < cn;
+            const int eb = in ? s_first[j] : 0, ee = in ? s_first[j + 1] : 0;
+            int cur = c0 + g;
+            for (;;) {
+                const unsigned over = __ballot_sync(0xffffffffu, in && c0 + j >= cur && ee - s > 128);
+                if (!over) break;
+                const int f = __ffs(over) - 1, lf = c0 + g + f;
+                const int bf = __shfl_sync(0xffffffffu, eb, f), ef = __shfl_sync(0xffffffffu, ee, f);
+                if (lf == start) {
+                    if (lane == 0) blocks[nb] = make_int4(start, lf + 1, s, ef);
+                    start = lf + 1; s = ef;
+                } else {
+                    if (lane == 0) blocks[nb] = make_int4(start, lf, s, bf);
+                    start = lf; s = bf;
+                }
+                cur = start;
+                ++nb;
+            }
+        }
+    }
+    if (threadIdx.x == 0) {
+        if (start < l1) blocks[nb++] = make_int4(start, l1, s, lm_first[l1]);
+        nblocks[seg] = nb;
+    }
 }
 
 __global__ void __launch_bounds__(256) k_ba_pair_counts(int L, const int* __restrict__ lm_first, const int* __restrict__ obs_kf,
@@ -2716,7 +2779,9 @@
     uint8_t* dout = nullptr;
     LmCtl* dctl = nullptr; int* dexec = nullptr;
     size_t spart_stride = 0, S_stride = 0, invL_stride = 0;
-    double *dHpl = nullptr, *dCpp = nullptr, *dbpo = nullptr, *dAll = nullptr, *dblo = nullptr;
+    int rows = 2;
+    double* drec = nullptr;
+    int4* dlblocks = nullptr; int* dnlblocks = nullptr; int nlseg = 0;
     double *dHll = nullptr, *dbl = nullptr, *dHpp = nullptr, *dbp = nullptr;
     double *dS = nullptr, *dbS = nullptr, *dx = nullptr, *dinvL = nullptr;
     int4* d_pair_rec = nullptr; int *dsegb = nullptr, *dsege = nullptr; int2* dpab = nullptr; int* ddiag = nullptr;
@@ -2771,6 +2836,7 @@
     const size_t sM = (size_t)M, sL = (size_t)L, sK = (size_t)K;
     const int nb_obs = (M + 127) / 128, nb_upd = (L + K + 127) / 128;
     const int exec_cap = 1024;
+    const int nlseg = M / kLbSegEdges + 1;
     double* hposes; double* hpoints; int *hkf, *hlm; float *hxy, *hxr, *hw; uint8_t* hfixed; uint8_t* hout; long long* hcounts;
     double* dposes_in; double* dpoints_in; int *dkf, *dlm; float *dxy, *dxr, *dw; uint8_t* dfixed;
     int *dfree, *dlmf, *dpoff; long long* dcounts;
@@ -2788,8 +2854,7 @@
         pl.dout = D.take<uint8_t>(sM); pl.dctl = D.take<LmCtl>(1); pl.dexec = D.take<int>(exec_cap);
         pl.dposes_ring = D.take<double>((kSpec + 1) * 12 * sK); pl.dpoints_ring = D.take<double>((kSpec + 1) * 3 * sL);
         pl.dlevel = D.take<uint8_t>(sM); pl.derr = D.take<double>(kSpec * 3 * sM);
-        pl.dHpl = D.take<double>(18 * sM); pl.dCpp = D.take<double>(21 * sM); pl.dbpo = D.take<double>(6 * sM);
-        pl.dAll = D.take<double>(6 * sM); pl.dblo = D.take<double>(3 * sM);
+        pl.dlblocks = D.take<int4>((size_t)nlseg * kLbSegCap); pl.dnlblocks = D.take<int>(nlseg);
         pl.dHll = D.take<double>(6 * sL); pl.dbl = D.take<double>(3 * sL);
         pl.dpchi = D.take<double>(kSpec * (size_t)nb_obs); pl.dpscale = D.take<double>(kSpec * (size_t)nb_upd);
         pl.dfail = D.take<int>(kSpec); pl.dmaxdiag = D.take<double>(2); pl.dclk = D.take<long long>(192); pl.dnchunks = D.take<int>(2);
@@ -2819,17 +2884,17 @@
         else { k_fill_f32<<<(unsigned)((sM + 255) / 256), 256, 0, st>>>(dxr, sM, -1.0f); OVS_LAUNCH_CHECK(); }
         OVS_CUDA_CHECK(cudaMemcpyAsync(dfixed, in.fixed, sK, dd, st));
     }
-    hcounts[0] = 0; hcounts[1] = 0; hcounts[2] = 0; hcounts[3] = 0; hcounts[4] = 0x7fffffffffffffffll;
-    OVS_CUDA_CHECK(cudaMemcpyAsync(dcounts, hcounts, 5 * sizeof(long long), cudaMemcpyHostToDevice, st));
+    hcounts[0] = 0; hcounts[1] = 0; hcounts[2] = 0; hcounts[3] = 0; hcounts[4] = 0x7fffffffffffffffll; hcounts[5] = 0;
+    OVS_CUDA_CHECK(cudaMemcpyAsync(dcounts, hcounts, 6 * sizeof(long long), cudaMemcpyHostToDevice, st));
     k_ba_free_index<<<1, 1024, 0, st>>>(K, dfixed, dfree, dcounts);
     OVS_LAUNCH_CHECK();
-    k_ba_landmark_index<<<(M + 255) / 256, 256, 0, st>>>(M, L, K, dkf, dlm, dlmf, dcounts);
+    k_ba_landmark_index<<<(M + 255) / 256, 256, 0, st>>>(M, L, K, dkf, dlm, dxr, dlmf, dcounts);
     OVS_LAUNCH_CHECK();
     k_ba_pair_counts<<<(L + 255) / 256, 256, 0, st>>>(L, dlmf, dkf, dfree, dpoff, dcounts);
     OVS_LAUNCH_CHECK();
     k_ba_pair_offsets<<<1, 1024, 0, st>>>(L, dpoff, dcounts);
     OVS_LAUNCH_CHECK();
-    OVS_CUDA_CHECK(cudaMemcpyAsync(hcounts, dcounts, 5 * sizeof(long long), cudaMemcpyDeviceToHost, st));
+    OVS_CUDA_CHECK(cudaMemcpyAsync(hcounts, dcounts, 6 * sizeof(long long), cudaMemcpyDeviceToHost, st));
     OVS_CUDA_CHECK(ovs::sync_stream(st));
     if (hcounts[4] != 0x7fffffffffffffffll) {
         const long long i = hcounts[4] >> 2;
@@ -2847,12 +2912,15 @@
     OVS_REQUIRE(n <= kMaxReducedDimBig, OVS_ERR_UNSUPPORTED, "more than %d free keyframes", kMaxReducedDimBig / 6);
     OVS_REQUIRE(npair_entries < (1ll << 30), OVS_ERR_UNSUPPORTED, "too many co-observations");
     const int npairs = nfree * (nfree + 1) / 2;
+    const int rows = hcounts[5] ? 3 : 2;
+    const size_t rec_doubles = (size_t)(rows == 3 ? EdgeRec<3>::kSize : EdgeRec<2>::kSize) * sM;
 
     const size_t sE = (size_t)std::max<long long>(npair_entries, 1);
     const size_t max_chunks = sE / 128 + (size_t)npairs + 8;
     const size_t max_dchunks = (size_t)nfree_edges / 128 + (size_t)nfree + 8;
     unsigned *dkeys, *dkeys2; unsigned long long *dvals, *dvals2; int4* dprec; int* dsort;
     auto carve2 = [&](Arena& W) {
+        pl.drec = W.take<double>(rec_doubles);
         pl.dpab = W.take<int2>(npairs); pl.ddiag = W.take<int>(nfree);
         pl.dHpp = W.take<double>(21 * (size_t)nfree); pl.dbp = W.take<double>(6 * (size_t)nfree);
         pl.S_stride = ((size_t)(n + 1) * n + 31) / 32 * 32; pl.invL_stride = (size_t)((n + kNB - 1) / kNB) * kNB * kNB;
@@ -2888,6 +2956,9 @@
     const float chi_sq_2D = 5.99146f, chi_sq_3D = 7.81473f;
     P.use_huber = 1; P.delta = (double)(setup_is_mono ? sqrtf(chi_sq_2D) : sqrtf(chi_sq_3D));
 
+    k_ba_landmark_blocks<<<nlseg, kLbThreads, 0, st>>>(L, dlmf, pl.dlblocks, pl.dnlblocks);
+    OVS_LAUNCH_CHECK();
+
     k_ba_pair_table<<<nfree, 128, 0, st>>>(nfree, pl.dpab, pl.ddiag);
     OVS_LAUNCH_CHECK();
     pl.d_pair_rec = dprec;
@@ -2914,6 +2985,7 @@
     OVS_LAUNCH_CHECK();
 
     pl.K = K; pl.L = L; pl.M = M; pl.nfree = nfree; pl.n = n; pl.npairs = npairs; pl.nb_obs = nb_obs; pl.nb_upd = nb_upd;
+    pl.rows = rows; pl.nlseg = nlseg;
     pl.npair_entries = npair_entries;
     {
         DenseSolve ds{};
@@ -3155,7 +3227,8 @@
             }
             OVS_CUDA_CHECK(cudaEventRecord(h->solver_ev[4 * slot], st));
         }
-        k_ba_schur_chunk<<<pl.max_chunks, 128, 0, st>>>(P, ctl, pl.dnchunks, pl.d_pair_rec, pl.dchunks, pl.dpab, pl.dHll, pl.dHpl, pl.dbl, pl.dspart, pl.spart_stride);
+        if (pl.rows == 3) k_ba_schur_chunk<3><<<pl.max_chunks, 128, 0, st>>>(P, ctl, pl.dnchunks, pl.d_pair_rec, pl.dchunks, pl.dpab, pl.dHll, pl.drec, pl.dbl, pl.dspart, pl.spart_stride);
+        else k_ba_schur_chunk<2><<<pl.max_chunks, 128, 0, st>>>(P, ctl, pl.dnchunks, pl.d_pair_rec, pl.dchunks, pl.dpab, pl.dHll, pl.drec, pl.dbl, pl.dspart, pl.spart_stride);
         OVS_LAUNCH_CHECK();
         k_ba_schur_final<<<dim3(npairs, kSpec), 64, 0, st>>>(n, ctl, pl.dpair_chunk_begin, pl.dpab, pl.dspart, pl.spart_stride, pl.dHpp, pl.dbp, pl.dS, pl.S_stride);
         OVS_LAUNCH_CHECK();
@@ -3164,7 +3237,8 @@
         const int rc_solve = launch_dense_solve(h, st, ctl, ds);
         if (rc_solve != OVS_OK) return rc_solve;
         if (ev) OVS_CUDA_CHECK(cudaEventRecord(h->solver_ev[4 * slot + 3], st));
-        k_ba_update<<<nb_upd, 128, 0, st>>>(P, ctl, pl.dHpl, pl.dHll, pl.dbl, pl.dbp, pl.dx, pl.dposes_ring, pl.dpoints_ring, pl.dpscale, pl.dfail);
+        if (pl.rows == 3) k_ba_update<3><<<nb_upd, 128, 0, st>>>(P, ctl, pl.drec, pl.dHll, pl.dbl, pl.dbp, pl.dx, pl.dposes_ring, pl.dpoints_ring, pl.dpscale, pl.dfail);
+        else k_ba_update<2><<<nb_upd, 128, 0, st>>>(P, ctl, pl.drec, pl.dHll, pl.dbl, pl.dbp, pl.dx, pl.dposes_ring, pl.dpoints_ring, pl.dpscale, pl.dfail);
         OVS_LAUNCH_CHECK();
         k_ba_errors<<<dim3(nb_obs, kSpec), 128, 0, st>>>(P, ctl, 0, pl.derr, pl.dpchi);
         OVS_LAUNCH_CHECK();
@@ -3176,11 +3250,12 @@
     };
 
     auto iteration_head = [&](bool in_graph, bool halt_if_undecided) -> int {
-        k_ba_linearize<<<nb_obs, 128, 0, st>>>(P, ctl, pl.dHpl, pl.dCpp, pl.dbpo, pl.dAll, pl.dblo);
+        const unsigned nb_lin = (unsigned)(pl.nlseg * kLbSegCap);
+        if (pl.rows == 3) k_ba_linearize<3><<<nb_lin, 128, 0, st>>>(P, ctl, pl.dnlblocks, pl.dlblocks, pl.drec, pl.dHll, pl.dbl, pl.dmaxdiag);
+        else k_ba_linearize<2><<<nb_lin, 128, 0, st>>>(P, ctl, pl.dnlblocks, pl.dlblocks, pl.drec, pl.dHll, pl.dbl, pl.dmaxdiag);
         OVS_LAUNCH_CHECK();
-        k_ba_landmark_accum<<<(L + 127) / 128, 128, 0, st>>>(P, ctl, pl.dAll, pl.dblo, pl.dHll, pl.dbl, pl.dmaxdiag);
-        OVS_LAUNCH_CHECK();
-        k_ba_pose_accum_chunk<<<pl.max_dchunks, 128, 0, st>>>(P, ctl, pl.dnchunks + 1, pl.d_pair_rec, pl.ddchunks, pl.dCpp, pl.dbpo, pl.dppart);
+        if (pl.rows == 3) k_ba_pose_accum_chunk<3><<<pl.max_dchunks, 128, 0, st>>>(P, ctl, pl.dnchunks + 1, pl.d_pair_rec, pl.ddchunks, pl.drec, pl.dppart);
+        else k_ba_pose_accum_chunk<2><<<pl.max_dchunks, 128, 0, st>>>(P, ctl, pl.dnchunks + 1, pl.d_pair_rec, pl.ddchunks, pl.drec, pl.dppart);
         OVS_LAUNCH_CHECK();
         k_ba_pose_final_plan<<<1, 1024, 0, st>>>(ctl, nfree, pl.dkf_chunk_begin, pl.dppart, pl.dHpp, pl.dbp, pl.dmaxdiag, pl.dfail, stop_word, mirror);
         OVS_LAUNCH_CHECK();
```

After: 433.8 (median of 6 runs). +9.1%, better.
